# hassony2/homan

Measured on AMD Instinct MI355X. Metric: optimisation iters/sec (30-frame 256^2 clip), higher is better.
Workload: dtype f32

## Files before the change

homan_amd/csrc/adam.hip:

```cpp
#include "hm_common.h"

struct AdamSlot {
    float* p; float* g; float* m; float* v;
    long n;
    float lr;
    int pad;
};

__device__ __forceinline__ void log_total_clip(float* __restrict__ vals, const float* __restrict__ w, int n, int s,
                                               int max_steps, float* __restrict__ log, int c, int nc)
{
    float* v = vals + (long)c * (n + 1);
    float t = 0.f;
    for (int i = 0; i < n; ++i)
        if (w[i] != 0.f) t += w[i] * v[i];
    v[n] = t;
    if (s < max_steps)
        for (int i = 0; i <= n; ++i) log[((long)s * nc + c) * (n + 1) + i] = v[i];
}
__device__ __forceinline__ double adam_pow(double b, int t)
{
    double r = 1.0;
    for (; t > 0; t >>= 1) {
        if (t & 1) r = r * b;
        b = b * b;
    }
    return r;
}
__global__ __launch_bounds__(256) void k_adam(const AdamSlot* __restrict__ slots, int n_tensors, int* __restrict__ step,
                                               float beta1, float beta2, float eps, int zero_grad, float* __restrict__ vals,
                                               const float* __restrict__ log_w, int log_n, int max_steps,
                                               float* __restrict__ log, int nclips)
{
    HM_LATENCY_KERNEL();
    HM_STAMP_START(0);
    const int step_now = __builtin_nontemporal_load(step);
    if ((int)blockIdx.y == n_tensors) {
        if (threadIdx.x == 0) {
            for (int c = blockIdx.x; c < nclips; c += gridDim.x) log_total_clip(vals, log_w, log_n, step_now, max_steps, log, c, nclips);
            const unsigned nblk = gridDim.x * gridDim.y;
            if (atomicAdd(reinterpret_cast<unsigned int*>(step) + 1, 1u) == nblk - 1u) {
                atomicExch(reinterpret_cast<unsigned int*>(step) + 1, 0u);
                atomicExch(step, step_now + 1);
            }
        }
        return;
    }
    const AdamSlot s = slots[blockIdx.y];
    const double bc1 = 1.0 - adam_pow((double)beta1, step_now + 1);
    const double bc2 = 1.0 - adam_pow((double)beta2, step_now + 1);
    const float neg_step = (float)(-((double)s.lr / bc1));
    const float bc2_sqrt = (float)sqrt(bc2);
    const float w1 = (float)(1.0 - (double)beta1), w2 = (float)(1.0 - (double)beta2);
    for (long i = (long)blockIdx.x * blockDim.x + threadIdx.x; i < s.n; i += (long)gridDim.x * blockDim.x) {
        const float g = s.g[i];
        float m = s.m[i], v = s.v[i];
        m = m + w1 * (g - m);
        v = v * beta2;
        v = v + (w2 * g) * g;
        const float denom = sqrtf(v) / bc2_sqrt + eps;
        s.p[i] = s.p[i] + (neg_step * m) / denom;
        s.m[i] = m;
        s.v[i] = v;
        if (zero_grad) s.g[i] = 0.f;
    }
    __syncthreads();
    if (threadIdx.x == 0) {
        const unsigned nblk = gridDim.x * gridDim.y;
        if (atomicAdd(reinterpret_cast<unsigned int*>(step) + 1, 1u) == nblk - 1u) {
            atomicExch(reinterpret_cast<unsigned int*>(step) + 1, 0u);
            atomicExch(step, step_now + 1);
        }
    }
    HM_STAMP_END(0);
}

__global__ void k_log(const float* __restrict__ src, int n, const int* __restrict__ step, int max_steps,
                      float* __restrict__ log)
{
    const int i = blockIdx.x * blockDim.x + threadIdx.x;
    const int t = step[0];
    if (i < n && t < max_steps) log[(long)t * n + i] = src[i];
}

__global__ void k_log_total(float* __restrict__ vals, const float* __restrict__ w, int n, const int* __restrict__ step,
                            int max_steps, float* __restrict__ log)
{
    HM_LATENCY_KERNEL();
    if (threadIdx.x == 0) log_total_clip(vals, w, n, step[0], max_steps, log, blockIdx.x, gridDim.x);
}

extern "C" {
int hm_log_total_clips(float* vals, const float* weights, int n, const int* step, int max_steps, float* log, int nclips,
                       hipStream_t stream)
{
    HM_CHECK_ARG(vals && weights && step && log && n > 0 && nclips > 0);
    hipLaunchKernelGGL(k_log_total, dim3(nclips), dim3(64), 0, stream, vals, weights, n, step, max_steps, log);
    return hm_launch_status();
}
size_t hm_adam_slot_bytes(void) { return sizeof(AdamSlot); }

int hm_adam_step(const void* slots, int n_tensors, int* step, float beta1, float beta2, float eps, int zero_grad,
                 int blocks_per_tensor, hipStream_t stream)
{
    HM_CHECK_ARG(slots && step && n_tensors > 0 && blocks_per_tensor > 0);
    hipLaunchKernelGGL(k_adam, dim3(blocks_per_tensor, n_tensors), dim3(256), 0, stream, (const AdamSlot*)slots, n_tensors,
                       step, beta1, beta2, eps, zero_grad, (float*)nullptr, (const float*)nullptr, 0, 0, (float*)nullptr, 0);
    return hm_launch_status();
}
int hm_adam_step_log(const void* slots, int n_tensors, int* step, float beta1, float beta2, float eps, int zero_grad,
                     int blocks_per_tensor, float* vals, const float* weights, int n, int max_steps, float* log, int nclips,
                     hipStream_t stream)
{
    HM_CHECK_ARG(slots && step && n_tensors > 0 && blocks_per_tensor > 0);
    HM_CHECK_ARG(vals && weights && log && n > 0 && nclips > 0);
    hipLaunchKernelGGL(k_adam, dim3(blocks_per_tensor, n_tensors + 1), dim3(256), 0, stream, (const AdamSlot*)slots, n_tensors,
                       step, beta1, beta2, eps, zero_grad, vals, weights, n, max_steps, log, nclips);
    return hm_launch_status();
}
int hm_log_scalars(const float* src, int n, const int* step, int max_steps, float* log, hipStream_t stream)
{
    HM_CHECK_ARG(src && step && log && n > 0);
    hipLaunchKernelGGL(k_log, dim3(hm_cdiv(n, 64)), dim3(64), 0, stream, src, n, step, max_steps, log);
    return hm_launch_status();
}
#ifdef HM_CHAIN_STAMPS
int hm_debug_chain_adam(unsigned long long* out, int reset)
{
    unsigned long long z[8] = {~0ull, 0, ~0ull, 0, ~0ull, 0, ~0ull, 0};
    (void)hipDeviceSynchronize();
    if (out) (void)hipMemcpyFromSymbol(out, HIP_SYMBOL(g_chain_ts), sizeof(z));
    if (reset) (void)hipMemcpyToSymbol(HIP_SYMBOL(g_chain_ts), z, sizeof(z));
    return HM_OK;
}
#endif
}
```

homan_amd/csrc/geometry.hip:

```cpp
#include "hm_common.h"

__global__ __launch_bounds__(256) void k_rigid_fwd(const float* __restrict__ mesh, const float* __restrict__ rot6d,
                                                   const float* __restrict__ trans, const float* __restrict__ scale,
                                                   int abs_scale, int N, int V, float* __restrict__ rotmat,
                                                   float* __restrict__ verts, int clip_len)
{
    __shared__ float R[9];
    const int n = blockIdx.y;
    if (threadIdx.x == 0) {
        float r[9];
        rot6d_to_mat(rot6d + n * 6, r);
#pragma unroll
        for (int k = 0; k < 9; ++k) R[k] = r[k];
        if (blockIdx.x == 0 && rotmat)
#pragma unroll
            for (int k = 0; k < 9; ++k) rotmat[n * 9 + k] = r[k];
    }
    __syncthreads();
    const int v = blockIdx.x * blockDim.x + threadIdx.x;
    if (v >= V) return;
    float s = scale[n / clip_len];
    if (abs_scale) s = fabsf(s);
    const float* m = mesh + ((long)n * V + v) * 3;
    const float x = s * m[0], y = s * m[1], z = s * m[2];
    float* o = verts + ((long)n * V + v) * 3;
    const float* t = trans + n * 3;
    o[0] = x * R[0] + y * R[3] + z * R[6] + t[0];
    o[1] = x * R[1] + y * R[4] + z * R[7] + t[1];
    o[2] = x * R[2] + y * R[5] + z * R[8] + t[2];
}

struct SilGather {
    const double* parts;
    const int* adj_off;
    const int* adj_items;
    const float* cam_verts;
    const float* K;
    float orig_size;
    int F;
};
template <bool EXACT>
__global__ __launch_bounds__(1024) void k_rigid_bwd(const float* __restrict__ mesh, const float* __restrict__ rot6d,
                                                   const float* __restrict__ scale, int abs_scale, RigidTerms terms,
                                                   SilGather sil,
                                                   const float* __restrict__ g_rigid, const float* __restrict__ g_frame,
                                                   int frame_stride, float frame_scale, int N, int V,
                                                   float* __restrict__ g_mesh,
                                                   float* __restrict__ g_rot6d, float* __restrict__ g_trans,
                                                   float* __restrict__ g_scale_part, float* __restrict__ partials,
                                                   unsigned int* __restrict__ frame_cnt, int clip_len, double magic)
{
    HM_LATENCY_KERNEL();
    HM_STAMP_START(sil.parts ? 1 : 0);
    __shared__ float red13[16 * 13];
    __shared__ double red13d[EXACT ? 16 * 13 : 1];
    __shared__ int s_flag;
    const int n = blockIdx.x;
    float R[9];
    rot6d_to_mat(rot6d + n * 6, R);
    const float sraw = scale[n / clip_len];
    const float s = abs_scale ? fabsf(sraw) : sraw;
    float gfr[3] = {0.f, 0.f, 0.f};
    if (g_frame) {
#pragma unroll
        for (int c = 0; c < 3; ++c) gfr[c] = frame_scale * g_frame[(long)n * frame_stride + c];
    }
    float acc[13];
    double accd[13];
#pragma unroll
    for (int k = 0; k < 13; ++k) { acc[k] = 0.f; accd[k] = 0.0; }
    for (int v = blockIdx.y * blockDim.x + threadIdx.x; v < V; v += gridDim.y * blockDim.x) {
        const long o = ((long)n * V + v) * 3;
        const float m[3] = {mesh[o], mesh[o + 1], mesh[o + 2]};
        float gf[3] = {0.f, 0.f, 0.f}, gt[3];
#pragma unroll
        for (int k = 0; k < 5; ++k)
            if (terms.p[k]) {
                gf[0] += terms.w[k] * terms.p[k][o]; gf[1] += terms.w[k] * terms.p[k][o + 1]; gf[2] += terms.w[k] * terms.p[k][o + 2];
            }
        if (sil.parts) {
            double su = 0.0, sv = 0.0;
            const double2* pf = reinterpret_cast<const double2*>(sil.parts + (long)n * sil.F * 6);
            const int a1 = sil.adj_off[v + 1];
            for (int a = sil.adj_off[v]; a < a1; a += 8) {
                int item[8];
#pragma unroll
                for (int k = 0; k < 8; ++k) item[k] = a + k < a1 ? sil.adj_items[a + k] : -1;
                double2 g2[8];
#pragma unroll
                for (int k = 0; k < 8; ++k) g2[k] = item[k] >= 0 ? pf[item[k]] : make_double2(0.0, 0.0);
#pragma unroll
                for (int k = 0; k < 8; ++k) { su += g2[k].x; sv += g2[k].y; }
            }
            const float gu = (float)su, gv = (float)sv;
            const float* k = sil.K + n * 9;
            const float x = sil.cam_verts[o], y = sil.cam_verts[o + 1], z = sil.cam_verts[o + 2];
            const float zz = z + 1e-9f;
            const float du0 = gu * (2.0f / sil.orig_size), dv0 = -gv * (2.0f / sil.orig_size);
            const float dxn = k[0] * du0 + k[3] * dv0;
            const float dyn = k[1] * du0 + k[4] * dv0;
            gf[0] += dxn / zz;
            gf[1] += dyn / zz;
            gf[2] += -(dxn * x + dyn * y) / (zz * zz);
        }
        gt[0] = gf[0] + gfr[0]; gt[1] = gf[1] + gfr[1]; gt[2] = gf[2] + gfr[2];
        if (g_rigid) { gt[0] += g_rigid[o]; gt[1] += g_rigid[o + 1]; gt[2] += g_rigid[o + 2]; }
        const float dm[3] = {R[0] * gf[0] + R[1] * gf[1] + R[2] * gf[2], R[3] * gf[0] + R[4] * gf[1] + R[5] * gf[2],
                             R[6] * gf[0] + R[7] * gf[1] + R[8] * gf[2]};
        if (EXACT) {
#pragma unroll
            for (int i = 0; i < 3; ++i)
#pragma unroll
                for (int j = 0; j < 3; ++j) accd[3 * i + j] += hm_quant((s * m[i]) * gt[j], magic);
#pragma unroll
            for (int j = 0; j < 3; ++j) accd[9 + j] += hm_quant(gt[j], magic);
            accd[12] += hm_quant(m[0] * dm[0] + m[1] * dm[1] + m[2] * dm[2], magic);
        } else {
#pragma unroll
            for (int i = 0; i < 3; ++i)
#pragma unroll
                for (int j = 0; j < 3; ++j) acc[3 * i + j] += (s * m[i]) * gt[j];
#pragma unroll
            for (int j = 0; j < 3; ++j) acc[9 + j] += gt[j];
            acc[12] += m[0] * dm[0] + m[1] * dm[1] + m[2] * dm[2];
        }
        if (g_mesh) { g_mesh[o] = s * dm[0]; g_mesh[o + 1] = s * dm[1]; g_mesh[o + 2] = s * dm[2]; }
    }
    float tot[13];
    if (EXACT) {
        hm_block_sum_n_f64<13>(accd, red13d);
        if (gridDim.y > 1) {
            double* rec = reinterpret_cast<double*>(partials + ((long)n * gridDim.y + blockIdx.y) * 32);
            if (threadIdx.x == 0) {
#pragma unroll
                for (int k = 0; k < 13; ++k) __hip_atomic_store(rec + k, accd[k], __ATOMIC_RELAXED, __HIP_MEMORY_SCOPE_AGENT);
            }
            if (!hm_last_block(frame_cnt + n, gridDim.y, &s_flag)) return;
            if (threadIdx.x < 13 * gridDim.y)
                red13d[threadIdx.x] = __hip_atomic_load(reinterpret_cast<const double*>(partials + ((long)n * gridDim.y + threadIdx.x / 13) * 32) + threadIdx.x % 13,
                                                        __ATOMIC_RELAXED, __HIP_MEMORY_SCOPE_AGENT);
            __syncthreads();
            if (threadIdx.x == 0) {
#pragma unroll
                for (int k = 0; k < 13; ++k) accd[k] = 0.0;
                for (unsigned c = 0; c < gridDim.y; ++c)
#pragma unroll
                    for (int k = 0; k < 13; ++k) accd[k] += red13d[c * 13 + k];
            }
        }
#pragma unroll
        for (int k = 0; k < 13; ++k) tot[k] = (float)accd[k];
    } else {
#pragma unroll
    for (int k = 0; k < 13; ++k) tot[k] = acc[k];
    hm_block_sum_n<13>(tot, red13);
    if (gridDim.y > 1) {
        float* rec = partials + ((long)n * gridDim.y + blockIdx.y) * 32;
        if (threadIdx.x == 0) {
#pragma unroll
            for (int k = 0; k < 13; ++k) hm_partial_store(rec + k, tot[k]);
        }
        if (!hm_last_block(frame_cnt + n, gridDim.y, &s_flag)) return;
        if (threadIdx.x < 13 * gridDim.y)
            red13[threadIdx.x] = hm_partial_load(partials + ((long)n * gridDim.y + threadIdx.x / 13) * 32 + threadIdx.x % 13);
        __syncthreads();
        if (threadIdx.x == 0) {
#pragma unroll
            for (int k = 0; k < 13; ++k) tot[k] = 0.f;
            for (unsigned c = 0; c < gridDim.y; ++c)
#pragma unroll
                for (int k = 0; k < 13; ++k) tot[k] += red13[c * 13 + k];
        }
    }
    }
    if (threadIdx.x == 0) {
        float dr6[6];
        rot6d_backward(rot6d + n * 6, tot, dr6);
#pragma unroll
        for (int k = 0; k < 6; ++k) g_rot6d[n * 6 + k] = dr6[k];
#pragma unroll
        for (int k = 0; k < 3; ++k) g_trans[n * 3 + k] = tot[9 + k];
        if (g_scale_part) g_scale_part[n] = (abs_scale && sraw < 0.f) ? -tot[12] : tot[12];
    }
    HM_STAMP_END(sil.parts ? 1 : 0);
}

struct SmoothIn { const float* verts; float w; };
template <int NV, int MAXT>
__global__ __launch_bounds__(MAXT) void k_rigid_bwd_x(const float* __restrict__ mesh, const float* __restrict__ rot6d,
                                                     const float* __restrict__ scale, int abs_scale, RigidTerms terms,
                                                     SilGather sil, SmoothIn sm, int N, int V, float* __restrict__ g_rot6d,
                                                     float* __restrict__ g_trans, float* __restrict__ g_scale_part,
                                                     float* __restrict__ partials, unsigned int* __restrict__ frame_cnt,
                                                     int clip_len, double magic)
{
    HM_LATENCY_KERNEL();
    HM_STAMP_START(1);
    __shared__ double red13d[16 * 13];
    __shared__ int s_flag;
    const int n = blockIdx.x;
    float R[9];
    rot6d_to_mat(rot6d + n * 6, R);
    const float sraw = scale[n / clip_len];
    const float s = abs_scale ? fabsf(sraw) : sraw;
    const int fl = n % clip_len;
    const long row = (long)V * 3;
    const long scnt = (long)(clip_len - 1) * row;
    const float inv_cnt = scnt > 0 ? 1.0f / (float)scnt : 0.f;
    int vv[NV];
    bool ok[NV];
    int a0[NV], a1[NV];
    float m[NV][3], cv[NV][3], tv[NV][5][3], nb[NV][2][3];
#pragma unroll
    for (int j = 0; j < NV; ++j) {
        vv[j] = ((int)blockIdx.y * NV + j) * (int)blockDim.x + (int)threadIdx.x;
        ok[j] = vv[j] < V;
        const int v = ok[j] ? vv[j] : 0;
        const long o = ((long)n * V + v) * 3;
        a0[j] = sil.parts ? sil.adj_off[v] : 0;
        a1[j] = sil.parts ? sil.adj_off[v + 1] : 0;
#pragma unroll
        for (int c = 0; c < 3; ++c) {
            m[j][c] = mesh[o + c];
            cv[j][c] = sil.parts ? sil.cam_verts[o + c] : 0.f;
        }
#pragma unroll
        for (int k = 0; k < 5; ++k)
#pragma unroll
            for (int c = 0; c < 3; ++c) tv[j][k][c] = terms.p[k] ? terms.p[k][o + c] : 0.f;
#pragma unroll
        for (int c = 0; c < 3; ++c) {
            nb[j][0][c] = (sm.verts && fl + 1 < clip_len) ? sm.verts[o + row + c] : 0.f;
            nb[j][1][c] = (sm.verts && fl >= 1) ? sm.verts[o - row + c] : 0.f;
        }
    }
    float sv[NV][3];
#pragma unroll
    for (int j = 0; j < NV; ++j)
#pragma unroll
        for (int c = 0; c < 3; ++c) sv[j][c] = sm.verts ? sm.verts[((long)n * V + (ok[j] ? vv[j] : 0)) * 3 + c] : 0.f;
    int item[NV][8];
#pragma unroll
    for (int j = 0; j < NV; ++j)
#pragma unroll
        for (int k = 0; k < 8; ++k) item[j][k] = (ok[j] && a0[j] + k < a1[j]) ? sil.adj_items[a0[j] + k] : -1;
    double su[NV], sw[NV];
    {
        const double2* pf = reinterpret_cast<const double2*>(sil.parts + (long)n * sil.F * 6);
        double2 g2[NV][8];
#pragma unroll
        for (int j = 0; j < NV; ++j)
#pragma unroll
            for (int k = 0; k < 8; ++k) g2[j][k] = item[j][k] >= 0 ? pf[item[j][k]] : make_double2(0.0, 0.0);
#pragma unroll
        for (int j = 0; j < NV; ++j) {
            su[j] = 0.0; sw[j] = 0.0;
#pragma unroll
            for (int k = 0; k < 8; ++k) { su[j] += g2[j][k].x; sw[j] += g2[j][k].y; }
            for (int a = a0[j] + 8; ok[j] && a < a1[j]; ++a) {
                const double2 g = pf[sil.adj_items[a]];
                su[j] += g.x; sw[j] += g.y;
            }
        }
    }
    double accd[13];
#pragma unroll
    for (int k = 0; k < 13; ++k) accd[k] = 0.0;
#pragma unroll
    for (int j = 0; j < NV; ++j) {
        if (!ok[j]) continue;
        float gf[3] = {0.f, 0.f, 0.f}, gt[3];
        if (sm.verts) {
#pragma unroll
            for (int c = 0; c < 3; ++c) {
                float g = 0.f;
                if (fl + 1 < clip_len) { const float d = nb[j][0][c] - sv[j][c]; g -= d; }
                if (fl >= 1) g += sv[j][c] - nb[j][1][c];
                gf[c] += sm.w * (2.0f * g * inv_cnt);
            }
        }
#pragma unroll
        for (int k = 0; k < 5; ++k)
            if (terms.p[k]) {
                gf[0] += terms.w[k] * tv[j][k][0]; gf[1] += terms.w[k] * tv[j][k][1]; gf[2] += terms.w[k] * tv[j][k][2];
            }
        if (sil.parts) {
            const float gu = (float)su[j], gv = (float)sw[j];
            const float* k = sil.K + n * 9;
            const float x = cv[j][0], y = cv[j][1], z = cv[j][2];
            const float zz = z + 1e-9f;
            const float du0 = gu * (2.0f / sil.orig_size), dv0 = -gv * (2.0f / sil.orig_size);
            const float dxn = k[0] * du0 + k[3] * dv0;
            const float dyn = k[1] * du0 + k[4] * dv0;
            gf[0] += dxn / zz;
            gf[1] += dyn / zz;
            gf[2] += -(dxn * x + dyn * y) / (zz * zz);
        }
        gt[0] = gf[0] + 0.f; gt[1] = gf[1] + 0.f; gt[2] = gf[2] + 0.f;
        const float dm[3] = {R[0] * gf[0] + R[1] * gf[1] + R[2] * gf[2], R[3] * gf[0] + R[4] * gf[1] + R[5] * gf[2],
                             R[6] * gf[0] + R[7] * gf[1] + R[8] * gf[2]};
#pragma unroll
        for (int i = 0; i < 3; ++i)
#pragma unroll
            for (int q = 0; q < 3; ++q) accd[3 * i + q] += hm_quant((s * m[j][i]) * gt[q], magic);
#pragma unroll
        for (int q = 0; q < 3; ++q) accd[9 + q] += hm_quant(gt[q], magic);
        accd[12] += hm_quant(m[j][0] * dm[0] + m[j][1] * dm[1] + m[j][2] * dm[2], magic);
    }
    hm_block_sum_n_f64<13>(accd, red13d);
    if (gridDim.y > 1) {
        double* rec = reinterpret_cast<double*>(partials + ((long)n * gridDim.y + blockIdx.y) * 32);
        if (threadIdx.x == 0) {
#pragma unroll
            for (int k = 0; k < 13; ++k) __hip_atomic_store(rec + k, accd[k], __ATOMIC_RELAXED, __HIP_MEMORY_SCOPE_AGENT);
        }
        if (!hm_last_block(frame_cnt + n, gridDim.y, &s_flag)) return;
        if (threadIdx.x < 13 * gridDim.y)
            red13d[threadIdx.x] = __hip_atomic_load(reinterpret_cast<const double*>(partials + ((long)n * gridDim.y + threadIdx.x / 13) * 32) + threadIdx.x % 13,
                                                    __ATOMIC_RELAXED, __HIP_MEMORY_SCOPE_AGENT);
        __syncthreads();
        if (threadIdx.x == 0) {
#pragma unroll
            for (int k = 0; k < 13; ++k) accd[k] = 0.0;
            for (unsigned c = 0; c < gridDim.y; ++c)
#pragma unroll
                for (int k = 0; k < 13; ++k) accd[k] += red13d[c * 13 + k];
        }
    }
    if (threadIdx.x == 0) {
        float tot[13], dr6[6];
#pragma unroll
        for (int k = 0; k < 13; ++k) tot[k] = (float)accd[k];
        rot6d_backward(rot6d + n * 6, tot, dr6);
#pragma unroll
        for (int k = 0; k < 6; ++k) g_rot6d[n * 6 + k] = dr6[k];
#pragma unroll
        for (int k = 0; k < 3; ++k) g_trans[n * 3 + k] = tot[9 + k];
        if (g_scale_part) g_scale_part[n] = (abs_scale && sraw < 0.f) ? -tot[12] : tot[12];
    }
    HM_STAMP_END(1);
}

__global__ void k_scale_by(const float* __restrict__ in, const float* __restrict__ s, long n, float* __restrict__ out)
{
    const long i = (long)blockIdx.x * blockDim.x + threadIdx.x;
    if (i < n) out[i] = s[0] * in[i];
}
__global__ void k_sum_small(const float* __restrict__ parts, int n, float w0, const float* __restrict__ extra, float w1,
                            float* __restrict__ out)
{
    __shared__ float red[16];
    const int c = blockIdx.x;
    float a = 0.f;
    for (int i = threadIdx.x; i < n; i += blockDim.x) a += parts[(long)c * n + i];
    a = hm_block_sum(a, red);
    if (threadIdx.x == 0) out[c] = w0 * a + (extra ? w1 * extra[c] : 0.f);
}

extern "C" {
int hm_sum_small_clips(const float* parts, int n, float w0, const float* extra, float w1, float* out, int nclips,
                       hipStream_t stream)
{
    HM_CHECK_ARG(parts && out && n > 0 && nclips > 0);
    hipLaunchKernelGGL(k_sum_small, dim3(nclips), dim3(64), 0, stream, parts, n, w0, extra, w1, out);
    return hm_launch_status();
}
int hm_rigid_fwd_clips(const float* mesh, const float* rot6d, const float* trans, const float* scale, int abs_scale, int N,
                       int V, float* rotmat, float* verts, int clip_len, hipStream_t stream)
{
    HM_CHECK_ARG(mesh && rot6d && trans && scale && verts && N > 0 && V > 0 && HM_CLIP_LEN_OK(N, clip_len));
    hipLaunchKernelGGL(k_rigid_fwd, dim3(hm_cdiv(V, 256), N), dim3(256), 0, stream, mesh, rot6d, trans, scale,
                       abs_scale, N, V, rotmat, verts, clip_len ? clip_len : N);
    return hm_launch_status();
}
int hm_rigid_fwd(const float* mesh, const float* rot6d, const float* trans, const float* scale, int abs_scale, int N,
                 int V, float* rotmat, float* verts, hipStream_t stream)
{
    return hm_rigid_fwd_clips(mesh, rot6d, trans, scale, abs_scale, N, V, rotmat, verts, 0, stream);
}
#define RIGID_MAX_CHUNKS 16
size_t hm_rigid_workspace_bytes(int N) { return (((size_t)N * 4 + 255) & ~(size_t)255) + (size_t)N * RIGID_MAX_CHUNKS * 32 * 4; }
static int rigid_bwd_launch(const float* mesh, const float* rot6d, const float* scale, int abs_scale,
                            const float* const* g_terms, const float* weights, int n_terms, SilGather sil,
                            const float* g_rigid, const float* g_frame, int frame_stride, float frame_scale, int N, int V,
                            float* g_mesh, float* g_rot6d, float* g_trans, float* g_scale_part, void* workspace,
                            int clip_len, int exact, int sum_log2q, SmoothIn smooth, hipStream_t stream)
{
    HM_CHECK_ARG(sum_log2q <= 0 && sum_log2q >= -60);
    HM_CHECK_ARG(mesh && rot6d && scale && g_rot6d && g_trans && N > 0 && V > 0 && HM_CLIP_LEN_OK(N, clip_len));
    HM_CHECK_ARG(n_terms >= 0 && n_terms <= 5 && (n_terms == 0 || (g_terms && weights)));
    HM_CHECK_ARG(!g_frame || frame_stride >= 3);
    RigidTerms t;
    for (int k = 0; k < 5; ++k) { t.p[k] = k < n_terms ? g_terms[k] : nullptr; t.w[k] = k < n_terms ? weights[k] : 0.f; }
    const int threads = exact ? 256 : (V > 512 ? 1024 : 256);
    const int chunks = workspace ? min(RIGID_MAX_CHUNKS, hm_cdiv(V, exact ? threads : 4 * threads)) : 1;
    unsigned int* cnt = (unsigned int*)workspace;
    float* partials = workspace ? (float*)((char*)workspace + (((size_t)N * 4 + 255) & ~(size_t)255)) : nullptr;
    const bool small = V <= RIGID_MAX_CHUNKS * 256;
    const int nv = small ? 1 : 2;
    const int thr = small ? 256 : 768;
    if (exact && !g_rigid && !g_frame && !g_mesh && (workspace ? V <= RIGID_MAX_CHUNKS * thr * nv : V <= thr * nv)) {
        const int ch = hm_cdiv(V, thr * nv);
        const double magic = hm_sum_magic(sum_log2q);
        if (nv == 2)
            hipLaunchKernelGGL((k_rigid_bwd_x<2, 768>), dim3(N, ch), dim3(thr), 0, stream, mesh, rot6d, scale,
                               abs_scale, t, sil, smooth, N, V, g_rot6d, g_trans, g_scale_part, partials, cnt, clip_len ? clip_len : N, magic);
        else
            hipLaunchKernelGGL((k_rigid_bwd_x<1, 1024>), dim3(N, ch), dim3(thr), 0, stream, mesh, rot6d, scale,
                               abs_scale, t, sil, smooth, N, V, g_rot6d, g_trans, g_scale_part, partials, cnt, clip_len ? clip_len : N, magic);
        return hm_launch_status();
    }
    HM_CHECK_ARG(!smooth.verts);
    if (exact)
        hipLaunchKernelGGL(k_rigid_bwd<true>, dim3(N, chunks), dim3(threads), 0, stream, mesh, rot6d, scale,
                           abs_scale, t, sil, g_rigid, g_frame, frame_stride, frame_scale, N, V, g_mesh, g_rot6d, g_trans,
                           g_scale_part, partials, cnt, clip_len ? clip_len : N, hm_sum_magic(sum_log2q));
    else
        hipLaunchKernelGGL(k_rigid_bwd<false>, dim3(N, chunks), dim3(threads), 0, stream, mesh, rot6d, scale,
                           abs_scale, t, sil, g_rigid, g_frame, frame_stride, frame_scale, N, V, g_mesh, g_rot6d, g_trans,
                           g_scale_part, partials, cnt, clip_len ? clip_len : N, 0.0);
    return hm_launch_status();
}
int hm_rigid_bwd_clips(const float* mesh, const float* rot6d, const float* scale, int abs_scale,
                       const float* const* g_terms, const float* weights, int n_terms, const float* g_rigid,
                       const float* g_frame, int frame_stride, float frame_scale, int N, int V, float* g_mesh,
                       float* g_rot6d, float* g_trans, float* g_scale_part, void* workspace, int clip_len,
                       hipStream_t stream)
{
    SilGather none = {nullptr, nullptr, nullptr, nullptr, nullptr, 1.0f, 0};
    return rigid_bwd_launch(mesh, rot6d, scale, abs_scale, g_terms, weights, n_terms, none, g_rigid, g_frame, frame_stride,
                            frame_scale, N, V, g_mesh, g_rot6d, g_trans, g_scale_part, workspace, clip_len, 0, 0,
                            SmoothIn{nullptr, 0.f}, stream);
}
int hm_rigid_bwd(const float* mesh, const float* rot6d, const float* scale, int abs_scale, const float* const* g_terms,
                 const float* weights, int n_terms, const float* g_rigid, const float* g_frame, int frame_stride,
                 float frame_scale, int N, int V, float* g_mesh, float* g_rot6d, float* g_trans, float* g_scale_part,
                 void* workspace, hipStream_t stream)
{
    return hm_rigid_bwd_clips(mesh, rot6d, scale, abs_scale, g_terms, weights, n_terms, g_rigid, g_frame, frame_stride,
                              frame_scale, N, V, g_mesh, g_rot6d, g_trans, g_scale_part, workspace, 0, stream);
}
int hm_rigid_bwd_sil_clips(const float* mesh, const float* rot6d, const float* scale, int abs_scale,
                           const float* const* g_terms, const float* weights, int n_terms, const double* sil_parts,
                           const int* adj_off, const int* adj_items, const float* cam_verts, const float* K,
                           float orig_size, int F, int N, int V, float* g_rot6d, float* g_trans, float* g_scale_part,
                           void* workspace, int clip_len, int sum_log2q, const float* smooth_verts, float smooth_weight,
                           hipStream_t stream)
{
    HM_CHECK_ARG(sil_parts && adj_off && adj_items && cam_verts && K && F > 0);
    SilGather sil = {sil_parts, adj_off, adj_items, cam_verts, K, orig_size, F};
    return rigid_bwd_launch(mesh, rot6d, scale, abs_scale, g_terms, weights, n_terms, sil, nullptr, nullptr, 0, 0.f, N, V,
                            nullptr, g_rot6d, g_trans, g_scale_part, workspace, clip_len, 1, sum_log2q,
                            SmoothIn{smooth_verts, smooth_weight}, stream);
}
int hm_rigid_bwd_sil(const float* mesh, const float* rot6d, const float* scale, int abs_scale, const float* const* g_terms,
                     const float* weights, int n_terms, const double* sil_parts, const int* adj_off, const int* adj_items,
                     const float* cam_verts, const float* K, float orig_size, int F, int N, int V, float* g_rot6d,
                     float* g_trans, float* g_scale_part, void* workspace, int sum_log2q, hipStream_t stream)
{
    return hm_rigid_bwd_sil_clips(mesh, rot6d, scale, abs_scale, g_terms, weights, n_terms, sil_parts, adj_off, adj_items,
                                  cam_verts, K, orig_size, F, N, V, g_rot6d, g_trans, g_scale_part, workspace, 0, sum_log2q,
                                  nullptr, 0.f, stream);
}
int hm_scale_by(const float* in, const float* s, long n, float* out, hipStream_t stream)
{
    HM_CHECK_ARG(in && s && out && n > 0);
    hipLaunchKernelGGL(k_scale_by, dim3(hm_cdiv(n, 256)), dim3(256), 0, stream, in, s, n, out);
    return hm_launch_status();
}
#ifdef HM_CHAIN_STAMPS
int hm_debug_chain_geometry(unsigned long long* out, int reset)
{
    unsigned long long z[8] = {~0ull, 0, ~0ull, 0, ~0ull, 0, ~0ull, 0};
    (void)hipDeviceSynchronize();
    if (out) (void)hipMemcpyFromSymbol(out, HIP_SYMBOL(g_chain_ts), sizeof(z));
    if (reset) (void)hipMemcpyToSymbol(HIP_SYMBOL(g_chain_ts), z, sizeof(z));
    return HM_OK;
}
#endif
}
```

homan_amd/csrc/hm_common.h:

```cpp
#pragma once
#include <hip/hip_runtime.h>
#include <stdint.h>
#include "homan_amd.h"

#define HM_WAVE 64

#ifndef HM_PRIO
#define HM_PRIO 3
#endif
#define HM_LATENCY_KERNEL() __builtin_amdgcn_s_setprio(HM_PRIO)
#ifdef HM_CHAIN_STAMPS
static __device__ unsigned long long g_chain_ts[8];
#define HM_STAMP_START(k) do { if (threadIdx.x == 0) atomicMin(&g_chain_ts[2 * (k)], (unsigned long long)wall_clock64()); } while (0)
#define HM_STAMP_END(k) do { if (threadIdx.x == 0) atomicMax(&g_chain_ts[2 * (k) + 1], (unsigned long long)wall_clock64()); } while (0)
#else
#define HM_STAMP_START(k)
#define HM_STAMP_END(k)
#endif
#ifndef HM_HAND_PRIO
#define HM_HAND_PRIO HM_PRIO
#endif
#define HM_HAND_KERNEL() __builtin_amdgcn_s_setprio(HM_HAND_PRIO)
#ifdef HM_CHAIN_PRIO
#define HM_CHAIN_KERNEL() __builtin_amdgcn_s_setprio(HM_CHAIN_PRIO)
#else
#define HM_CHAIN_KERNEL()
#endif

#define HM_CHECK_ARG(cond) \
    do {                   \
        if (!(cond)) return HM_ERR_BAD_ARG; \
    } while (0)

#define HM_CLIP_LEN_OK(N, clip_len) ((clip_len) == 0 || ((clip_len) > 0 && (N) % (clip_len) == 0))
#define HM_RED_WS_FLOATS 576

static inline int hm_launch_status()
{
    hipError_t e = hipGetLastError();
    return e == hipSuccess ? HM_OK : HM_ERR_LAUNCH;
}

static inline int hm_cdiv(long a, long b) { return (int)((a + b - 1) / b); }

template <int CTRL, int ROW_MASK>
__device__ __forceinline__ float hm_dpp(float old, float v)
{
    return __builtin_bit_cast(float, __builtin_amdgcn_update_dpp(__builtin_bit_cast(int, old), __builtin_bit_cast(int, v),
                                                                CTRL, ROW_MASK, 0xf, false));
}
__device__ __forceinline__ float hm_wave_sum(float v)
{
    v += hm_dpp<0xb1, 0xf>(0.f, v);
    v += hm_dpp<0x4e, 0xf>(0.f, v);
    v += hm_dpp<0x114, 0xf>(0.f, v);
    v += hm_dpp<0x118, 0xf>(0.f, v);
    v += hm_dpp<0x142, 0xa>(0.f, v);
    v += hm_dpp<0x143, 0xc>(0.f, v);
    return __builtin_bit_cast(float, __builtin_amdgcn_readlane(__builtin_bit_cast(int, v), 63));
}
__device__ __forceinline__ float hm_wave_min(float v)
{
    v = fminf(v, hm_dpp<0xb1, 0xf>(v, v));
    v = fminf(v, hm_dpp<0x4e, 0xf>(v, v));
    v = fminf(v, hm_dpp<0x114, 0xf>(v, v));
    v = fminf(v, hm_dpp<0x118, 0xf>(v, v));
    v = fminf(v, hm_dpp<0x142, 0xa>(v, v));
    v = fminf(v, hm_dpp<0x143, 0xc>(v, v));
    return __builtin_bit_cast(float, __builtin_amdgcn_readlane(__builtin_bit_cast(int, v), 63));
}
__device__ __forceinline__ float hm_wave_max(float v)
{
    v = fmaxf(v, hm_dpp<0xb1, 0xf>(v, v));
    v = fmaxf(v, hm_dpp<0x4e, 0xf>(v, v));
    v = fmaxf(v, hm_dpp<0x114, 0xf>(v, v));
    v = fmaxf(v, hm_dpp<0x118, 0xf>(v, v));
    v = fmaxf(v, hm_dpp<0x142, 0xa>(v, v));
    v = fmaxf(v, hm_dpp<0x143, 0xc>(v, v));
    return __builtin_bit_cast(float, __builtin_amdgcn_readlane(__builtin_bit_cast(int, v), 63));
}

__device__ __forceinline__ float hm_block_sum(float v, float* red)
{
    const int lane = threadIdx.x & 63, w = threadIdx.x >> 6, nw = (blockDim.x + 63) >> 6;
    v = hm_wave_sum(v);
    __syncthreads();
    if (lane == 0) red[w] = v;
    __syncthreads();
    float t = 0.f;
    for (int i = 0; i < nw; ++i) t += red[i];
    return t;
}
template <int N>
__device__ __forceinline__ void hm_block_sum_n(float (&v)[N], float* red)
{
    const int lane = threadIdx.x & 63, w = threadIdx.x >> 6, nw = (blockDim.x + 63) >> 6;
#pragma unroll
    for (int k = 0; k < N; ++k) v[k] = hm_wave_sum(v[k]);
    __syncthreads();
    if (lane == 0) {
#pragma unroll
        for (int k = 0; k < N; ++k) red[k * 16 + w] = v[k];
    }
    __syncthreads();
#pragma unroll
    for (int k = 0; k < N; ++k) {
        float t = 0.f;
        for (int i = 0; i < nw; ++i) t += red[k * 16 + i];
        v[k] = t;
    }
}
__device__ __forceinline__ float hm_block_min(float v, float* red)
{
    const int lane = threadIdx.x & 63, w = threadIdx.x >> 6, nw = (blockDim.x + 63) >> 6;
    v = hm_wave_min(v);
    __syncthreads();
    if (lane == 0) red[w] = v;
    __syncthreads();
    float t = red[0];
    for (int i = 1; i < nw; ++i) t = fminf(t, red[i]);
    return t;
}
__device__ __forceinline__ float hm_block_max(float v, float* red)
{
    const int lane = threadIdx.x & 63, w = threadIdx.x >> 6, nw = (blockDim.x + 63) >> 6;
    v = hm_wave_max(v);
    __syncthreads();
    if (lane == 0) red[w] = v;
    __syncthreads();
    float t = red[0];
    for (int i = 1; i < nw; ++i) t = fmaxf(t, red[i]);
    return t;
}

__device__ __forceinline__ void hm_partial_store(float* p, float v)
{
    __hip_atomic_store(p, v, __ATOMIC_RELAXED, __HIP_MEMORY_SCOPE_AGENT);
}
__device__ __forceinline__ float hm_partial_load(const float* p)
{
    return __hip_atomic_load(p, __ATOMIC_RELAXED, __HIP_MEMORY_SCOPE_AGENT);
}
__device__ __forceinline__ bool hm_last_block(unsigned int* counter, unsigned int nblocks, int* s_flag)
{
    __syncthreads();
    if (threadIdx.x == 0) {
        asm volatile("s_waitcnt vmcnt(0)" ::: "memory");
        const unsigned int ticket = atomicAdd(counter, 1u);
        const int last = (ticket == nblocks - 1u);
        if (last) atomicExch(counter, 0u);
        *s_flag = last;
    }
    __syncthreads();
    return *s_flag != 0;
}


__device__ __forceinline__ float hm_last_block_sum(const float* partials, int n, int stride, float* red)
{
    float a = 0.f;
    for (int i = threadIdx.x; i < n; i += blockDim.x) a += hm_partial_load(partials + (long)i * stride);
    return hm_block_sum(a, red);
}

__host__ __device__ __forceinline__ void hm_sincos(float af, float* sn, float* cs)
{
    const double a = (double)af;
    const double k = __builtin_rint(a * 0.63661977236758138243);
    double r = a - k * 1.57079632673412561417e+00;
    r = r - k * 6.07710050650619224932e-11;
    const double z = r * r;
    double ps = 1.58969099521155010221e-10;
    ps = -2.50507602534068634195e-08 + z * ps;
    ps = 2.75573137070700676789e-06 + z * ps;
    ps = -1.98412698298579493134e-04 + z * ps;
    ps = 8.33333333332248946124e-03 + z * ps;
    ps = -1.66666666666666324348e-01 + z * ps;
    const double s = r + (r * z) * ps;
    double pc = -1.13596475577881948265e-11;
    pc = 2.08757232129817482790e-09 + z * pc;
    pc = -2.75573143513906633035e-07 + z * pc;
    pc = 2.48015872894767294178e-05 + z * pc;
    pc = -1.38888888888741095749e-03 + z * pc;
    pc = 4.16666666666666019037e-02 + z * pc;
    const double c = (1.0 - 0.5 * z) + (z * z) * pc;
    const int q = (int)((long long)k) & 3;
    const double sv = (q == 0) ? s : (q == 1) ? c : (q == 2) ? -s : -c;
    const double cv = (q == 0) ? c : (q == 1) ? -s : (q == 2) ? -c : s;
    *sn = (float)sv;
    *cs = (float)cv;
}

__host__ __device__ __forceinline__ float hm_tanh(float xf)
{
    const double ax = xf < 0.f ? -(double)xf : (double)xf;
    if (ax > 20.0) return xf < 0.f ? -1.0f : 1.0f;
    if (ax < 0.01) {
        const double q = ax * ax;
        const double sm = ax * (1.0 + q * (-3.33333333333333314830e-01 + q * (1.33333333333333331483e-01 + q * -5.39682539682539708542e-02)));
        return (float)(xf < 0.f ? -sm : sm);
    }
    const double t = -2.0 * ax;
    const double k = __builtin_rint(t * 1.44269504088896338700e+00);
    const double r = (t - k * 6.93147180369123816490e-01) - k * 1.90821492927058770002e-10;
    const double z = r * r;
    double p = 4.13813679705723846039e-08;
    p = -1.65339022054652515390e-06 + z * p;
    p = 6.61375632143793436117e-05 + z * p;
    p = -2.77777777770155933842e-03 + z * p;
    p = 1.66666666666666019037e-01 + z * p;
    const double c = r - z * p;
    const double er = 1.0 - ((r * c) / (c - 2.0) - r);
    const double e = __builtin_ldexp(er, (int)k);
    const double th = (1.0 - e) / (1.0 + e);
    return (float)(xf < 0.f ? -th : th);
}

__host__ __device__ __forceinline__ float hm_sigmoid(float xf)
{
    const double t = -(double)xf;
    const double k = __builtin_rint(t * 1.44269504088896338700e+00);
    const double r = (t - k * 6.93147180369123816490e-01) - k * 1.90821492927058770002e-10;
    const double z = r * r;
    double p = 4.13813679705723846039e-08;
    p = -1.65339022054652515390e-06 + z * p;
    p = 6.61375632143793436117e-05 + z * p;
    p = -2.77777777770155933842e-03 + z * p;
    p = 1.66666666666666019037e-01 + z * p;
    const double c = r - z * p;
    const double er = 1.0 - ((r * c) / (c - 2.0) - r);
    const double e = __builtin_ldexp(er, (int)k);
    return (float)(1.0 / (1.0 + e));
}

__device__ __forceinline__ void rot6d_to_mat(const float* r6 , float* R )
{
    const float a1[3] = {r6[0], r6[2], r6[4]}, a2[3] = {r6[1], r6[3], r6[5]};
    const float n1 = fmaxf(sqrtf(a1[0] * a1[0] + a1[1] * a1[1] + a1[2] * a1[2]), 1e-12f);
    const float b1[3] = {a1[0] / n1, a1[1] / n1, a1[2] / n1};
    const float d = b1[0] * a2[0] + b1[1] * a2[1] + b1[2] * a2[2];
    const float u[3] = {a2[0] - d * b1[0], a2[1] - d * b1[1], a2[2] - d * b1[2]};
    const float nu = fmaxf(sqrtf(u[0] * u[0] + u[1] * u[1] + u[2] * u[2]), 1e-12f);
    const float b2[3] = {u[0] / nu, u[1] / nu, u[2] / nu};
    const float b3[3] = {b1[1] * b2[2] - b1[2] * b2[1], b1[2] * b2[0] - b1[0] * b2[2], b1[0] * b2[1] - b1[1] * b2[0]};
#pragma unroll
    for (int i = 0; i < 3; ++i) { R[3 * i] = b1[i]; R[3 * i + 1] = b2[i]; R[3 * i + 2] = b3[i]; }
}

__device__ __forceinline__ void rot6d_backward(const float* r6, const float* dR, float* dr6)
{
    const float a1[3] = {r6[0], r6[2], r6[4]}, a2[3] = {r6[1], r6[3], r6[5]};
    const float n1r = sqrtf(a1[0] * a1[0] + a1[1] * a1[1] + a1[2] * a1[2]);
    const float n1 = fmaxf(n1r, 1e-12f);
    const float b1[3] = {a1[0] / n1, a1[1] / n1, a1[2] / n1};
    const float d = b1[0] * a2[0] + b1[1] * a2[1] + b1[2] * a2[2];
    const float u[3] = {a2[0] - d * b1[0], a2[1] - d * b1[1], a2[2] - d * b1[2]};
    const float nur = sqrtf(u[0] * u[0] + u[1] * u[1] + u[2] * u[2]);
    const float nu = fmaxf(nur, 1e-12f);
    const float b2[3] = {u[0] / nu, u[1] / nu, u[2] / nu};
    float db1[3] = {dR[0], dR[3], dR[6]}, db2[3] = {dR[1], dR[4], dR[7]};
    const float db3[3] = {dR[2], dR[5], dR[8]};
    db1[0] += b2[1] * db3[2] - b2[2] * db3[1];
    db1[1] += b2[2] * db3[0] - b2[0] * db3[2];
    db1[2] += b2[0] * db3[1] - b2[1] * db3[0];
    db2[0] += db3[1] * b1[2] - db3[2] * b1[1];
    db2[1] += db3[2] * b1[0] - db3[0] * b1[2];
    db2[2] += db3[0] * b1[1] - db3[1] * b1[0];
    float du[3];
    if (nur > 1e-12f) {
        const float s = b2[0] * db2[0] + b2[1] * db2[1] + b2[2] * db2[2];
#pragma unroll
        for (int i = 0; i < 3; ++i) du[i] = (db2[i] - b2[i] * s) / nu;
    } else {
#pragma unroll
        for (int i = 0; i < 3; ++i) du[i] = db2[i] / nu;
    }
    float da2[3] = {du[0], du[1], du[2]};
    const float dd = -(du[0] * b1[0] + du[1] * b1[1] + du[2] * b1[2]);
#pragma unroll
    for (int i = 0; i < 3; ++i) { db1[i] += -d * du[i] + dd * a2[i]; da2[i] += dd * b1[i]; }
    float da1[3];
    if (n1r > 1e-12f) {
        const float s = b1[0] * db1[0] + b1[1] * db1[1] + b1[2] * db1[2];
#pragma unroll
        for (int i = 0; i < 3; ++i) da1[i] = (db1[i] - b1[i] * s) / n1;
    } else {
#pragma unroll
        for (int i = 0; i < 3; ++i) da1[i] = db1[i] / n1;
    }
#pragma unroll
    for (int i = 0; i < 3; ++i) { dr6[2 * i] = da1[i]; dr6[2 * i + 1] = da2[i]; }
}

#define HM_SUM_LOG2Q_DEFAULT (-44)
__host__ __device__ __forceinline__ double hm_sum_magic(int log2q)
{
    return 6755399441055744.0  * __builtin_ldexp(1.0, log2q ? log2q : HM_SUM_LOG2Q_DEFAULT);
}
__device__ __forceinline__ double hm_quant(float x, double magic) { return ((double)x + magic) - magic; }

template <int CTRL, int ROW_MASK>
__device__ __forceinline__ double hm_dpp_f64(double v)
{
    const int lo = __builtin_amdgcn_update_dpp(0, __double2loint(v), CTRL, ROW_MASK, 0xf, false);
    const int hi = __builtin_amdgcn_update_dpp(0, __double2hiint(v), CTRL, ROW_MASK, 0xf, false);
    return __hiloint2double(hi, lo);
}
__device__ __forceinline__ double hm_wave_sum_f64(double v)
{
    v += hm_dpp_f64<0xb1, 0xf>(v);
    v += hm_dpp_f64<0x4e, 0xf>(v);
    v += hm_dpp_f64<0x114, 0xf>(v);
    v += hm_dpp_f64<0x118, 0xf>(v);
    v += hm_dpp_f64<0x142, 0xa>(v);
    v += hm_dpp_f64<0x143, 0xc>(v);
    return __hiloint2double(__builtin_amdgcn_readlane(__double2hiint(v), 63), __builtin_amdgcn_readlane(__double2loint(v), 63));
}
template <int N>
__device__ __forceinline__ void hm_block_sum_n_f64(double (&v)[N], double* red)
{
    const int lane = threadIdx.x & 63, w = threadIdx.x >> 6, nw = (blockDim.x + 63) >> 6;
#pragma unroll
    for (int k = 0; k < N; ++k) v[k] = hm_wave_sum_f64(v[k]);
    if (nw == 1) return;
    __syncthreads();
    if (lane == 0) {
#pragma unroll
        for (int k = 0; k < N; ++k) red[k * 16 + w] = v[k];
    }
    __syncthreads();
#pragma unroll
    for (int k = 0; k < N; ++k) {
        double t = 0.0;
        for (int i = 0; i < nw; ++i) t += red[k * 16 + i];
        v[k] = t;
    }
}

struct RigidTerms { const float* p[5]; float w[5]; };
```

homan_amd/csrc/mano.hip:

```cpp
#include "hm_common.h"
#include <string.h>

#define MANO_V 778
#define MANO_J 16
#define MANO_NF 145
#define MANO_CHUNK 256
#define MANO_NCHUNK 4
#define MANO_PART 352
#define MANO_NCH64 13
#define MANO_STATE_SH 832
#define MANO_STATE_DW (MANO_STATE_SH + 3 * MANO_V + 2)

struct ManoModelDev {
    const float* v_template;
    const float* M;
    const float* J_template;
    const float* J_shapedirs;
    const float* weights;
    const float* comps;
    const float* hand_mean;
    const int* parents;
};

__device__ __forceinline__ void rodrigues(const float* r, float* R)
{
    const float e0 = r[0] + 1e-8f, e1 = r[1] + 1e-8f, e2 = r[2] + 1e-8f;
    const float a = sqrtf(e0 * e0 + e1 * e1 + e2 * e2);
    const float nx = r[0] / a, ny = r[1] / a, nz = r[2] / a;
    float s, cs_;
    hm_sincos(a, &s, &cs_);
    const float c1 = 1.0f - cs_;
    const float K[9] = {0.f, -nz, ny, nz, 0.f, -nx, -ny, nx, 0.f};
#pragma unroll
    for (int i = 0; i < 3; ++i)
#pragma unroll
        for (int j = 0; j < 3; ++j) {
            float kk = K[3 * i] * K[j] + K[3 * i + 1] * K[3 + j] + K[3 * i + 2] * K[6 + j];
            R[3 * i + j] = (i == j ? 1.0f : 0.0f) + s * K[3 * i + j] + c1 * kk;
        }
}

__device__ __forceinline__ void rodrigues_backward(const float* r, const float* dR, float* dr)
{
    const float e[3] = {r[0] + 1e-8f, r[1] + 1e-8f, r[2] + 1e-8f};
    const float a = sqrtf(e[0] * e[0] + e[1] * e[1] + e[2] * e[2]);
    const float n[3] = {r[0] / a, r[1] / a, r[2] / a};
    float s, c;
    hm_sincos(a, &s, &c);
    const float c1 = 1.0f - c;
    const float K[9] = {0.f, -n[2], n[1], n[2], 0.f, -n[0], -n[1], n[0], 0.f};
    float KK[9];
#pragma unroll
    for (int i = 0; i < 3; ++i)
#pragma unroll
        for (int j = 0; j < 3; ++j) KK[3 * i + j] = K[3 * i] * K[j] + K[3 * i + 1] * K[3 + j] + K[3 * i + 2] * K[6 + j];
    float dRK = 0.f, dRKK = 0.f;
#pragma unroll
    for (int k = 0; k < 9; ++k) { dRK += dR[k] * K[k]; dRKK += dR[k] * KK[k]; }
    float da = c * dRK + s * dRKK;
    float dK[9];
#pragma unroll
    for (int i = 0; i < 3; ++i)
#pragma unroll
        for (int j = 0; j < 3; ++j) {
            float t1 = dR[3 * i] * K[3 * j] + dR[3 * i + 1] * K[3 * j + 1] + dR[3 * i + 2] * K[3 * j + 2];
            float t2 = K[i] * dR[j] + K[3 + i] * dR[3 + j] + K[6 + i] * dR[6 + j];
            dK[3 * i + j] = s * dR[3 * i + j] + c1 * (t1 + t2);
        }
    const float dn[3] = {dK[7] - dK[5], dK[2] - dK[6], dK[3] - dK[1]};
    da += -(dn[0] * r[0] + dn[1] * r[1] + dn[2] * r[2]) / (a * a);
#pragma unroll
    for (int i = 0; i < 3; ++i) dr[i] = dn[i] / a + da * e[i] / a;
}

struct ManoShared {
    float pose[48];
    float Rl[MANO_J][9];
    float J[MANO_J][3];
    float Rw[MANO_J][9];
    float tw[MANO_J][3];
    float A[MANO_J][12];
    float feat[MANO_NF];
    int parents[MANO_J];
    int depth[MANO_J];
};

__device__ __forceinline__ void mano_prepare(const ManoModelDev& m, const float* pca, int pca_stride, const float* rot,
                                             const float* betas, int b, ManoShared& sh, int t)
{
    if (t < 48) {
        float v;
        if (t < 3) v = rot[b * 3 + t];
        else {
            const int k = t - 3;
            v = 0.f;
            for (int i = 0; i < 16; ++i) v += pca[(long)b * pca_stride + i] * m.comps[i * 45 + k];
            v += m.hand_mean[k];
        }
        sh.pose[t] = v;
    }
    if (t < 10) sh.feat[135 + t] = betas[b * 10 + t];
    if (t < MANO_J) sh.parents[t] = m.parents[t];
    __syncthreads();
    if (t < MANO_J) {
        int d = 0;
        for (int q = sh.parents[t]; q >= 0; q = sh.parents[q]) ++d;
        sh.depth[t] = d;
        float R[9];
        rodrigues(&sh.pose[3 * t], R);
#pragma unroll
        for (int k = 0; k < 9; ++k) sh.Rl[t][k] = R[k];
        if (t >= 1)
#pragma unroll
            for (int k = 0; k < 9; ++k) sh.feat[9 * (t - 1) + k] = R[k] - ((k % 4 == 0) ? 1.0f : 0.0f);
#pragma unroll
        for (int c = 0; c < 3; ++c) {
            float v = m.J_template[t * 3 + c];
            for (int l = 0; l < 10; ++l) v += betas[b * 10 + l] * m.J_shapedirs[(t * 3 + c) * 10 + l];
            sh.J[t][c] = v;
        }
    }
    __syncthreads();
    int depth = 0, par = -1, maxd = 0;
    if (t < MANO_J) { par = sh.parents[t]; depth = sh.depth[t]; }
#pragma unroll
    for (int j = 0; j < MANO_J; ++j) maxd = max(maxd, sh.depth[j]);
    for (int level = 0; level < MANO_J; ++level) {
        if (t < MANO_J && depth == level) {
            const int j = t, p = par;
            if (p < 0) {
#pragma unroll
                for (int k = 0; k < 9; ++k) sh.Rw[j][k] = sh.Rl[j][k];
#pragma unroll
                for (int c = 0; c < 3; ++c) sh.tw[j][c] = sh.J[j][c];
            } else {
                const float rel[3] = {sh.J[j][0] - sh.J[p][0], sh.J[j][1] - sh.J[p][1], sh.J[j][2] - sh.J[p][2]};
#pragma unroll
                for (int i = 0; i < 3; ++i) {
#pragma unroll
                    for (int k = 0; k < 3; ++k)
                        sh.Rw[j][3 * i + k] = sh.Rw[p][3 * i] * sh.Rl[j][k] + sh.Rw[p][3 * i + 1] * sh.Rl[j][3 + k] +
                                              sh.Rw[p][3 * i + 2] * sh.Rl[j][6 + k];
                    sh.tw[j][i] = sh.Rw[p][3 * i] * rel[0] + sh.Rw[p][3 * i + 1] * rel[1] + sh.Rw[p][3 * i + 2] * rel[2] +
                                  sh.tw[p][i];
                }
            }
        }
        __syncthreads();
        if (level >= maxd) break;
    }
    if (t < MANO_J) {
        const int j = t;
#pragma unroll
        for (int i = 0; i < 3; ++i) {
            sh.A[j][4 * i] = sh.Rw[j][3 * i];
            sh.A[j][4 * i + 1] = sh.Rw[j][3 * i + 1];
            sh.A[j][4 * i + 2] = sh.Rw[j][3 * i + 2];
            sh.A[j][4 * i + 3] = sh.tw[j][i] - (sh.Rw[j][3 * i] * sh.J[j][0] + sh.Rw[j][3 * i + 1] * sh.J[j][1] +
                                                sh.Rw[j][3 * i + 2] * sh.J[j][2]);
        }
    }
    __syncthreads();
}

#define MANO_VCH 64
#define MANO_ROWS_PER_WAVE 37
__device__ __forceinline__ void mano_posed_chunk(const ManoModelDev& m, const ManoShared& sh, int v0, float (*s_part)[MANO_VCH][3],
                                                 float (*s_vp)[3])
{
    const int lane = threadIdx.x & 63, wv = threadIdx.x >> 6;
    const int v = min(v0 + lane, MANO_V - 1);
    float a0 = 0.f, a1 = 0.f, a2 = 0.f;
    const int k0 = wv * MANO_ROWS_PER_WAVE, k1 = min(MANO_NF, k0 + MANO_ROWS_PER_WAVE);
    const float* base = m.M + 3 * v;
#pragma unroll 4
    for (int k = k0; k < k1; ++k) {
        const float f = sh.feat[k];
        const float* row = base + (long)k * (3 * MANO_V);
        a0 += f * row[0];
        a1 += f * row[1];
        a2 += f * row[2];
    }
    s_part[wv][lane][0] = a0; s_part[wv][lane][1] = a1; s_part[wv][lane][2] = a2;
    __syncthreads();
    if (wv == 0) {
#pragma unroll
        for (int c = 0; c < 3; ++c)
            s_vp[lane][c] = m.v_template[3 * v + c] + ((s_part[0][lane][c] + s_part[1][lane][c]) + (s_part[2][lane][c] + s_part[3][lane][c]));
    }
    __syncthreads();
}

__device__ __forceinline__ void mano_skin_transform(const ManoModelDev& m, const ManoShared& sh, int v, float* T)
{
#pragma unroll
    for (int k = 0; k < 12; ++k) T[k] = 0.f;
    const float4* wrow = reinterpret_cast<const float4*>(m.weights + v * MANO_J);
#pragma unroll
    for (int q = 0; q < 4; ++q) {
        const float4 w4 = wrow[q];
        const float ws[4] = {w4.x, w4.y, w4.z, w4.w};
#pragma unroll
        for (int u = 0; u < 4; ++u) {
            const int j = 4 * q + u;
#pragma unroll
            for (int k = 0; k < 12; ++k) T[k] += ws[u] * sh.A[j][k];
        }
    }
}

#define MANO_FPW 4
__global__ __launch_bounds__(256) void k_mano_fwd(ManoModelDev m, const float* __restrict__ pca, int pca_stride,
                                                   const float* __restrict__ rot, const float* __restrict__ betas,
                                                   const float* __restrict__ trans, int B, float* __restrict__ verts,
                                                   float* __restrict__ joints, const float* __restrict__ rigid_rot6d,
                                                   const float* __restrict__ rigid_trans,
                                                   const float* __restrict__ rigid_scale, float* __restrict__ verts_world,
                                                   float* __restrict__ state, int clip_len, int row0, int row_stride)
{
    __shared__ ManoShared shs[MANO_FPW];
    __shared__ float s_part[4][MANO_FPW][MANO_VCH][3];
    __shared__ float s_vp[MANO_FPW][MANO_VCH][3];
    __shared__ float s_R[MANO_FPW][9];
    const int lane = threadIdx.x & 63, wv = threadIdx.x >> 6;
    const int b_raw = blockIdx.y * MANO_FPW + wv;
    const bool live = b_raw < B;
    const int b = (min(b_raw, B - 1)) * row_stride + row0;
    ManoShared& sh = shs[wv];
    if (verts_world && lane == 48) rot6d_to_mat(rigid_rot6d + b * 6, s_R[wv]);
    mano_prepare(m, pca, pca_stride, rot, betas, b, sh, lane);
    const float tr[3] = {trans ? trans[b * 3] : 0.f, trans ? trans[b * 3 + 1] : 0.f, trans ? trans[b * 3 + 2] : 0.f};
    if (joints && live && blockIdx.x == 0 && lane < MANO_J * 3)
        joints[b * MANO_J * 3 + lane] = sh.tw[lane / 3][lane % 3] + tr[lane % 3];
    const int v0 = blockIdx.x * MANO_VCH;
    const int v = min(v0 + lane, MANO_V - 1);
    {
        float a[MANO_FPW][3];
#pragma unroll
        for (int f = 0; f < MANO_FPW; ++f) a[f][0] = a[f][1] = a[f][2] = 0.f;
        const int k0 = wv * MANO_ROWS_PER_WAVE, k1 = min(MANO_NF, k0 + MANO_ROWS_PER_WAVE);
        const float* base = m.M + 3 * v;
#pragma unroll 4
        for (int k = k0; k < k1; ++k) {
            const float* row = base + (long)k * (3 * MANO_V);
            const float r0 = row[0], r1 = row[1], r2 = row[2];
#pragma unroll
            for (int f = 0; f < MANO_FPW; ++f) {
                const float ft = shs[f].feat[k];
                a[f][0] += ft * r0;
                a[f][1] += ft * r1;
                a[f][2] += ft * r2;
            }
        }
#pragma unroll
        for (int f = 0; f < MANO_FPW; ++f) {
            s_part[wv][f][lane][0] = a[f][0]; s_part[wv][f][lane][1] = a[f][1]; s_part[wv][f][lane][2] = a[f][2];
        }
    }
    __syncthreads();
#pragma unroll
    for (int c = 0; c < 3; ++c)
        s_vp[wv][lane][c] = m.v_template[3 * v + c] + ((s_part[0][wv][lane][c] + s_part[1][wv][lane][c]) +
                                                       (s_part[2][wv][lane][c] + s_part[3][wv][lane][c]));
    __builtin_amdgcn_wave_barrier();
    if (!live) return;
    if (state) {
        float* st = state + (long)b * MANO_STATE_DW;
        if (blockIdx.x == 0)
            for (int i = lane; i < (int)(sizeof(ManoShared) / 4); i += 64) st[i] = reinterpret_cast<const float*>(&sh)[i];
        const int nv3 = 3 * min(MANO_VCH, MANO_V - v0);
        for (int i = lane; i < nv3; i += 64) st[MANO_STATE_SH + 3 * v0 + i] = (&s_vp[wv][0][0])[i];
    }
    if (v0 + lane >= MANO_V) return;
    float T[12];
    mano_skin_transform(m, sh, v, T);
    const float* vp = s_vp[wv][lane];
    float* o = verts + ((long)b * MANO_V + v) * 3;
    float p[3];
#pragma unroll
    for (int i = 0; i < 3; ++i) { p[i] = T[4 * i] * vp[0] + T[4 * i + 1] * vp[1] + T[4 * i + 2] * vp[2] + T[4 * i + 3] + tr[i]; o[i] = p[i]; }
    if (verts_world) {
        const float s = rigid_scale[b / clip_len];
        const float x = s * p[0], y = s * p[1], z = s * p[2];
        const float* t = rigid_trans + b * 3;
        const float* R = s_R[wv];
        float* ow = verts_world + ((long)b * MANO_V + v) * 3;
        ow[0] = x * R[0] + y * R[3] + z * R[6] + t[0];
        ow[1] = x * R[1] + y * R[4] + z * R[7] + t[1];
        ow[2] = x * R[2] + y * R[5] + z * R[8] + t[2];
    }
}

static_assert(sizeof(ManoShared) / 4 <= MANO_STATE_SH, "MANO_STATE_SH too small");

struct ManoBwd2Shared {
    float tot[MANO_PART];
    float dRw[MANO_J][9], dtw[MANO_J][3], dJ[MANO_J][3], dRl[MANO_J][9], dpose[48];
    float cR[MANO_J][9], ct[MANO_J][3], cJ[MANO_J][3];
};
__device__ __forceinline__ void mano_bwd2_body(const ManoModelDev& m, const ManoShared& sh, ManoBwd2Shared& w,
                                               const float* __restrict__ partials, int nchunk, int lb, int b, int pca_dim,
                                               const float* __restrict__ g_pca_extra, float w_extra,
                                               float* __restrict__ g_pca, float* __restrict__ g_rot,
                                               float* __restrict__ g_betas, float* __restrict__ g_trans)
{
    const int t = threadIdx.x, nt = blockDim.x;
    for (int k = t; k < MANO_PART; k += nt) {
        float v[MANO_NCH64];
#pragma unroll
        for (int c = 0; c < MANO_NCH64; ++c)
            v[c] = c < nchunk ? hm_partial_load(partials + ((long)lb * nchunk + c) * MANO_PART + k) : 0.f;
        float a = 0.f;
#pragma unroll
        for (int c = 0; c < MANO_NCH64; ++c) a += v[c];
        w.tot[k] = a;
    }
    int depth = 0, par = -1, maxd = 0;
    if (t < MANO_J) { par = sh.parents[t]; depth = sh.depth[t]; }
#pragma unroll
    for (int j = 0; j < MANO_J; ++j) maxd = max(maxd, sh.depth[j]);
    __syncthreads();
    if (t < MANO_J) {
        const int j = t;
        const float* dA = &w.tot[j * 12];
#pragma unroll
        for (int i = 0; i < 3; ++i) {
#pragma unroll
            for (int k = 0; k < 3; ++k) w.dRw[j][3 * i + k] = dA[4 * i + k] - dA[4 * i + 3] * sh.J[j][k];
            w.dtw[j][i] = dA[4 * i + 3];
        }
#pragma unroll
        for (int k = 0; k < 3; ++k)
            w.dJ[j][k] = -(sh.Rw[j][k] * dA[3] + sh.Rw[j][3 + k] * dA[7] + sh.Rw[j][6 + k] * dA[11]);
    }
    __syncthreads();
    for (int level = maxd; level >= 1; --level) {
        if (t < MANO_J && depth == level) {
            const int j = t, p = par;
            const float rel[3] = {sh.J[j][0] - sh.J[p][0], sh.J[j][1] - sh.J[p][1], sh.J[j][2] - sh.J[p][2]};
#pragma unroll
            for (int i = 0; i < 3; ++i) {
#pragma unroll
                for (int k = 0; k < 3; ++k)
                    w.cR[j][3 * i + k] = w.dtw[j][i] * rel[k] + w.dRw[j][3 * i] * sh.Rl[j][3 * k] +
                                         w.dRw[j][3 * i + 1] * sh.Rl[j][3 * k + 1] + w.dRw[j][3 * i + 2] * sh.Rl[j][3 * k + 2];
                w.ct[j][i] = w.dtw[j][i];
            }
#pragma unroll
            for (int k = 0; k < 3; ++k) {
                const float d = sh.Rw[p][k] * w.dtw[j][0] + sh.Rw[p][3 + k] * w.dtw[j][1] + sh.Rw[p][6 + k] * w.dtw[j][2];
                w.dJ[j][k] += d;
                w.cJ[j][k] = -d;
            }
#pragma unroll
            for (int i = 0; i < 3; ++i)
#pragma unroll
                for (int k = 0; k < 3; ++k)
                    w.dRl[j][3 * i + k] = sh.Rw[p][i] * w.dRw[j][k] + sh.Rw[p][3 + i] * w.dRw[j][3 + k] + sh.Rw[p][6 + i] * w.dRw[j][6 + k];
        }
        __syncthreads();
        if (t < MANO_J && depth == level - 1) {
            for (int j = 0; j < MANO_J; ++j)
                if (sh.parents[j] == t) {
#pragma unroll
                    for (int k = 0; k < 9; ++k) w.dRw[t][k] += w.cR[j][k];
#pragma unroll
                    for (int k = 0; k < 3; ++k) { w.dtw[t][k] += w.ct[j][k]; w.dJ[t][k] += w.cJ[j][k]; }
                }
        }
        __syncthreads();
    }
    if (t < MANO_J && par < 0) {
#pragma unroll
        for (int k = 0; k < 9; ++k) w.dRl[t][k] = w.dRw[t][k];
#pragma unroll
        for (int c = 0; c < 3; ++c) w.dJ[t][c] += w.dtw[t][c];
    }
    __syncthreads();
    if (t < MANO_J) {
        float dR[9];
#pragma unroll
        for (int k = 0; k < 9; ++k) dR[k] = w.dRl[t][k] + (t >= 1 ? w.tot[192 + 9 * (t - 1) + k] : 0.f);
        float dr[3];
        rodrigues_backward(&sh.pose[3 * t], dR, dr);
#pragma unroll
        for (int c = 0; c < 3; ++c) w.dpose[3 * t + c] = dr[c];
    }
    __syncthreads();
    if (t < 3) {
        g_rot[b * 3 + t] = w.dpose[t];
        g_trans[b * 3 + t] = w.tot[337 + t];
    }
    for (int i = t; i < pca_dim; i += nt) {
        float a = 0.f;
        if (i < 16) {
            float cv[45];
#pragma unroll
            for (int k = 0; k < 45; ++k) cv[k] = m.comps[i * 45 + k];
#pragma unroll
            for (int k = 0; k < 45; ++k) a += cv[k] * w.dpose[3 + k];
        }
        if (g_pca_extra) a += w_extra * g_pca_extra[(long)b * pca_dim + i];
        g_pca[(long)b * pca_dim + i] = a;
    }
    if (t < 10) {
        float a = w.tot[192 + 135 + t];
        float jv[MANO_J * 3];
#pragma unroll
        for (int q = 0; q < MANO_J * 3; ++q) jv[q] = m.J_shapedirs[q * 10 + t];
#pragma unroll
        for (int q = 0; q < MANO_J * 3; ++q) a += jv[q] * w.dJ[q / 3][q % 3];
        g_betas[b * 10 + t] = a;
    }
}

#ifdef MANO_PHASES
static __device__ unsigned long long g_mano_ph[16];
#define MPH_MARK(k) do { if (threadIdx.x == 0) { const unsigned long long t_ = wall_clock64(); atomicAdd(&g_mano_ph[k], t_ - mph_t); mph_t = t_; } } while (0)
#else
#define MPH_MARK(k)
#endif
struct ManoRigid {
    const float* mesh;
    const float* rot6d;
    const float* scale;
    int clip_len;
    RigidTerms terms;
    const float* g_rigid;
    const float* g_frame;
    int frame_stride;
    float frame_scale;
    float* g_rot6d; float* g_trans;
};
template <bool RIGID>
__global__ __launch_bounds__(256) void k_mano_bwd(ManoModelDev m, const float* __restrict__ pca, int pca_stride,
                                                   const float* __restrict__ rot, const float* __restrict__ betas,
                                                   const float* __restrict__ gout, int B, const float* __restrict__ state,
                                                   float* __restrict__ partials, unsigned int* __restrict__ frame_cnt,
                                                   int pca_dim, const float* __restrict__ g_pca_extra, float w_extra,
                                                   float* __restrict__ g_pca, float* __restrict__ g_rot,
                                                   float* __restrict__ g_betas, float* __restrict__ g_trans, int row0,
                                                   int row_stride, ManoRigid mr)
{
    HM_HAND_KERNEL();
    __shared__ ManoShared sh;
    __shared__ float s_part[4][MANO_VCH][3];
    __shared__ float s_vp[MANO_VCH][3];
    __shared__ float s_g[MANO_VCH][3];
    __shared__ float s_dvp[MANO_VCH * 3];
    __shared__ float s_w[MANO_VCH][MANO_J + 1];
    __shared__ float red[16];
    __shared__ ManoBwd2Shared w2;
    __shared__ int s_flag;
    const int lb = blockIdx.y, b = lb * row_stride + row0, t = threadIdx.x;
    const int v0 = blockIdx.x * MANO_VCH;
    const int nv = min(MANO_VCH, MANO_V - v0);
#ifdef MANO_PHASES
    unsigned long long mph_t = wall_clock64();
    if (t == 0) atomicAdd(&g_mano_ph[15], 1ull);
#endif
    if (state) {
        const float* st = state + (long)b * MANO_STATE_DW;
        for (int i = t; i < (int)(sizeof(ManoShared) / 4); i += blockDim.x) reinterpret_cast<float*>(&sh)[i] = st[i];
        if (t < 3 * nv) (&s_vp[0][0])[t] = st[MANO_STATE_SH + 3 * v0 + t];
        __syncthreads();
    } else {
        mano_prepare(m, pca, pca_stride, rot, betas, b, sh, threadIdx.x);
        mano_posed_chunk(m, sh, v0, s_part, s_vp);
    }
    MPH_MARK(0);
    float g[3] = {0.f, 0.f, 0.f};
    float racc[12];
#pragma unroll
    for (int k = 0; k < 12; ++k) racc[k] = 0.f;
    if (t < nv) {
        const int v = v0 + t;
        if (RIGID) {
            const long o = ((long)b * MANO_V + v) * 3;
            float R[9];
            rot6d_to_mat(mr.rot6d + (long)b * 6, R);
            const float s = mr.scale[b / mr.clip_len];
            const float mv[3] = {mr.mesh[o], mr.mesh[o + 1], mr.mesh[o + 2]};
            float gf[3] = {0.f, 0.f, 0.f}, gt[3];
#pragma unroll
            for (int k = 0; k < 5; ++k)
                if (mr.terms.p[k]) {
                    gf[0] += mr.terms.w[k] * mr.terms.p[k][o]; gf[1] += mr.terms.w[k] * mr.terms.p[k][o + 1];
                    gf[2] += mr.terms.w[k] * mr.terms.p[k][o + 2];
                }
#pragma unroll
            for (int c = 0; c < 3; ++c)
                gt[c] = gf[c] + (mr.g_frame ? mr.frame_scale * mr.g_frame[(long)b * mr.frame_stride + c] : 0.f);
            if (mr.g_rigid) { gt[0] += mr.g_rigid[o]; gt[1] += mr.g_rigid[o + 1]; gt[2] += mr.g_rigid[o + 2]; }
#pragma unroll
            for (int i = 0; i < 3; ++i)
#pragma unroll
                for (int j = 0; j < 3; ++j) racc[3 * i + j] = (s * mv[i]) * gt[j];
#pragma unroll
            for (int j = 0; j < 3; ++j) racc[9 + j] = gt[j];
            g[0] = s * (R[0] * gf[0] + R[1] * gf[1] + R[2] * gf[2]);
            g[1] = s * (R[3] * gf[0] + R[4] * gf[1] + R[5] * gf[2]);
            g[2] = s * (R[6] * gf[0] + R[7] * gf[1] + R[8] * gf[2]);
        } else {
            const float* gp = gout + ((long)b * MANO_V + v) * 3;
            g[0] = gp[0]; g[1] = gp[1]; g[2] = gp[2];
        }
    }
    float* out = partials + ((long)lb * gridDim.x + blockIdx.x) * MANO_PART;
    if (RIGID) {
        float* red12 = &s_part[0][0][0];
        hm_block_sum_n<12>(racc, red12);
        if (t < 12) hm_partial_store(out + 340 + t, racc[t]);
        __syncthreads();
    }
    if (t < nv) {
        const int v = v0 + t;
        float T[12];
        mano_skin_transform(m, sh, v, T);
#pragma unroll
        for (int c = 0; c < 3; ++c) {
            s_g[t][c] = g[c];
            s_dvp[3 * t + c] = T[c] * g[0] + T[4 + c] * g[1] + T[8 + c] * g[2];
        }
        for (int j = 0; j < MANO_J; ++j) s_w[t][j] = m.weights[v * MANO_J + j];
    }
    MPH_MARK(1);
    const float tg0 = hm_block_sum(g[0], red), tg1 = hm_block_sum(g[1], red), tg2 = hm_block_sum(g[2], red);
    if (t == 0) { hm_partial_store(out + 337, tg0); hm_partial_store(out + 338, tg1); hm_partial_store(out + 339, tg2); }
    __syncthreads();
    MPH_MARK(2);
    if (t < 192) {
        const int j = t / 12, r = (t % 12) / 4, c = t % 4;
        float acc = 0.f;
        for (int i = 0; i < nv; ++i) acc += s_w[i][j] * s_g[i][r] * (c < 3 ? s_vp[i][c] : 1.0f);
        hm_partial_store(out + t, acc);
    }
    __syncthreads();
    MPH_MARK(3);
    const int wv = t >> 6, lane = t & 63;
    const int ne = 3 * nv;
    float d0 = 0.f, d1 = 0.f, d2 = 0.f;
    if (lane < ne) d0 = s_dvp[lane];
    if (lane + 64 < ne) d1 = s_dvp[lane + 64];
    if (lane + 128 < ne) d2 = s_dvp[lane + 128];
    constexpr int ROWS = (MANO_NF + 3) / 4;
    float r0[ROWS], r1[ROWS], r2[ROWS];
#pragma unroll
    for (int q = 0; q < ROWS; ++q) {
        const int k = wv + 4 * q;
        const float* row = m.M + (long)min(k, MANO_NF - 1) * (3 * MANO_V) + 3 * v0;
        r0[q] = lane < ne ? row[lane] : 0.f;
        r1[q] = lane + 64 < ne ? row[lane + 64] : 0.f;
        r2[q] = lane + 128 < ne ? row[lane + 128] : 0.f;
    }
#pragma unroll
    for (int q = 0; q < ROWS; ++q) {
        const int k = wv + 4 * q;
        float acc = r0[q] * d0;
        acc += r1[q] * d1;
        acc += r2[q] * d2;
        acc = hm_wave_sum(acc);
        if (lane == 0 && k < MANO_NF) hm_partial_store(out + 192 + k, acc);
    }
    asm volatile("s_waitcnt vmcnt(0)" ::: "memory");
    __syncthreads();
    MPH_MARK(4);
    if (t == 0) {
        const unsigned int ticket = atomicAdd(frame_cnt + lb, 1u);
        const int last = ticket == gridDim.x - 1u;
        if (last) atomicExch(frame_cnt + lb, 0u);
        s_flag = last;
    }
    __syncthreads();
    MPH_MARK(5);
    if (s_flag) {
        mano_bwd2_body(m, sh, w2, partials, gridDim.x, lb, b, pca_dim, g_pca_extra, w_extra, g_pca, g_rot, g_betas, g_trans);
        if (RIGID) {
            __syncthreads();
            if (t == 0) {
                float dr6[6];
                rot6d_backward(mr.rot6d + (long)b * 6, &w2.tot[340], dr6);
#pragma unroll
                for (int k = 0; k < 6; ++k) mr.g_rot6d[(long)b * 6 + k] = dr6[k];
#pragma unroll
                for (int k = 0; k < 3; ++k) mr.g_trans[(long)b * 3 + k] = w2.tot[349 + k];
            }
        }
#ifdef MANO_PHASES
        __syncthreads();
        MPH_MARK(6);
        if (t == 0) atomicAdd(&g_mano_ph[14], 1ull);
#endif
    }
}

extern "C" {
int hm_mano_fwd_rows(const void* const* model, const float* pca, int pca_dim, const float* rot, const float* betas,
                     const float* trans, int B, float* verts, float* joints, const float* rigid_rot6d,
                     const float* rigid_trans, const float* rigid_scale, float* verts_world, float* state, int clip_len,
                     int row0, int row_stride, hipStream_t stream)
{
    HM_CHECK_ARG(model && pca && rot && betas && verts && B > 0 && pca_dim >= 16 && row_stride >= 1 && row0 >= 0 && row0 < row_stride);
    HM_CHECK_ARG(clip_len >= 0 && (clip_len == 0 || (B * row_stride) % clip_len == 0));
    HM_CHECK_ARG(!verts_world || (rigid_rot6d && rigid_trans && rigid_scale));
    ManoModelDev m = {(const float*)model[0], (const float*)model[1], (const float*)model[2], (const float*)model[3],
                      (const float*)model[4], (const float*)model[5], (const float*)model[6], (const int*)model[7]};
    hipLaunchKernelGGL(k_mano_fwd, dim3(MANO_NCH64, (B + MANO_FPW - 1) / MANO_FPW), dim3(256), 0, stream, m, pca, pca_dim, rot, betas, trans, B, verts,
                       joints, rigid_rot6d, rigid_trans, rigid_scale, verts_world, state, clip_len ? clip_len : B * row_stride,
                       row0, row_stride);
    return hm_launch_status();
}
int hm_mano_fwd_clips(const void* const* model, const float* pca, int pca_dim, const float* rot, const float* betas,
                      const float* trans, int B, float* verts, float* joints, const float* rigid_rot6d,
                      const float* rigid_trans, const float* rigid_scale, float* verts_world, float* state, int clip_len,
                      hipStream_t stream)
{
    HM_CHECK_ARG(model && pca && rot && betas && verts && B > 0 && pca_dim >= 16 && HM_CLIP_LEN_OK(B, clip_len));
    HM_CHECK_ARG(!verts_world || (rigid_rot6d && rigid_trans && rigid_scale));
    ManoModelDev m = {(const float*)model[0], (const float*)model[1], (const float*)model[2], (const float*)model[3],
                      (const float*)model[4], (const float*)model[5], (const float*)model[6], (const int*)model[7]};
    hipLaunchKernelGGL(k_mano_fwd, dim3(MANO_NCH64, (B + MANO_FPW - 1) / MANO_FPW), dim3(256), 0, stream, m, pca, pca_dim, rot, betas, trans, B, verts,
                       joints, rigid_rot6d, rigid_trans, rigid_scale, verts_world, state, clip_len ? clip_len : B, 0, 1);
    return hm_launch_status();
}
int hm_mano_fwd(const void* const* model, const float* pca, int pca_dim, const float* rot, const float* betas,
                const float* trans, int B, float* verts, float* joints, const float* rigid_rot6d, const float* rigid_trans,
                const float* rigid_scale, float* verts_world, float* state, hipStream_t stream)
{
    return hm_mano_fwd_clips(model, pca, pca_dim, rot, betas, trans, B, verts, joints, rigid_rot6d, rigid_trans,
                             rigid_scale, verts_world, state, 0, stream);
}
size_t hm_mano_workspace_bytes(int B) { return 512 + (size_t)B * 4 + (size_t)B * MANO_NCH64 * MANO_PART * sizeof(float); }
size_t hm_mano_state_bytes(int B) { return (size_t)B * MANO_STATE_DW * sizeof(float); }
static int mano_bwd_launch(const void* const* model, const float* pca, int pca_dim, const float* rot, const float* betas, int B,
                           const float* g_verts, const float* g_pca_extra, float w_extra, float* g_pca, float* g_rot,
                           float* g_betas, float* g_trans, const float* state, void* workspace, int row0, int row_stride,
                           const ManoRigid& mr, hipStream_t stream)
{
    HM_CHECK_ARG(model && pca && rot && betas && (g_verts || mr.mesh) && g_pca && g_rot && g_betas && g_trans && workspace);
    HM_CHECK_ARG(B > 0 && pca_dim >= 16 && row_stride >= 1 && row0 >= 0 && row0 < row_stride);
    ManoModelDev m = {(const float*)model[0], (const float*)model[1], (const float*)model[2], (const float*)model[3],
                      (const float*)model[4], (const float*)model[5], (const float*)model[6], (const int*)model[7]};
    unsigned int* cnt = (unsigned int*)workspace;
    float* partials = (float*)((char*)workspace + 256 + (((size_t)B * 4 + 255) & ~(size_t)255));
    if (mr.mesh)
        hipLaunchKernelGGL(k_mano_bwd<true>, dim3(MANO_NCH64, B), dim3(256), 0, stream, m, pca, pca_dim, rot, betas,
                           g_verts, B, state, partials, cnt, pca_dim, g_pca_extra, w_extra, g_pca, g_rot, g_betas, g_trans, row0,
                           row_stride, mr);
    else
        hipLaunchKernelGGL(k_mano_bwd<false>, dim3(MANO_NCH64, B), dim3(256), 0, stream, m, pca, pca_dim, rot, betas,
                           g_verts, B, state, partials, cnt, pca_dim, g_pca_extra, w_extra, g_pca, g_rot, g_betas, g_trans, row0,
                           row_stride, mr);
    return hm_launch_status();
}
int hm_mano_bwd_rows(const void* const* model, const float* pca, int pca_dim, const float* rot, const float* betas, int B,
                     const float* g_verts, const float* g_pca_extra, float w_extra, float* g_pca, float* g_rot, float* g_betas,
                     float* g_trans, const float* state, void* workspace, int row0, int row_stride, hipStream_t stream)
{
    ManoRigid none;
    memset(&none, 0, sizeof(none));
    return mano_bwd_launch(model, pca, pca_dim, rot, betas, B, g_verts, g_pca_extra, w_extra, g_pca, g_rot, g_betas, g_trans,
                           state, workspace, row0, row_stride, none, stream);
}
int hm_mano_bwd_rigid_clips(const void* const* model, const float* pca, int pca_dim, const float* rot, const float* betas, int B,
                            const float* g_pca_extra, float w_extra, float* g_pca, float* g_rot, float* g_betas,
                            float* g_trans, const float* state, void* workspace, const float* mesh, const float* rigid_rot6d,
                            const float* rigid_scale, const float* const* g_terms, const float* weights, int n_terms,
                            const float* g_rigid, const float* g_frame, int frame_stride, float frame_scale,
                            float* g_rigid_rot6d, float* g_rigid_trans, int clip_len, hipStream_t stream)
{
    HM_CHECK_ARG(mesh && rigid_rot6d && rigid_scale && g_rigid_rot6d && g_rigid_trans && HM_CLIP_LEN_OK(B, clip_len));
    HM_CHECK_ARG(n_terms >= 0 && n_terms <= 5 && (n_terms == 0 || (g_terms && weights)));
    HM_CHECK_ARG(!g_frame || frame_stride >= 3);
    ManoRigid mr;
    memset(&mr, 0, sizeof(mr));
    mr.mesh = mesh; mr.rot6d = rigid_rot6d; mr.scale = rigid_scale; mr.clip_len = clip_len ? clip_len : B;
    for (int k = 0; k < 5; ++k) { mr.terms.p[k] = k < n_terms ? g_terms[k] : nullptr; mr.terms.w[k] = k < n_terms ? weights[k] : 0.f; }
    mr.g_rigid = g_rigid; mr.g_frame = g_frame; mr.frame_stride = frame_stride; mr.frame_scale = frame_scale;
    mr.g_rot6d = g_rigid_rot6d; mr.g_trans = g_rigid_trans;
    return mano_bwd_launch(model, pca, pca_dim, rot, betas, B, nullptr, g_pca_extra, w_extra, g_pca, g_rot, g_betas, g_trans,
                           state, workspace, 0, 1, mr, stream);
}
int hm_mano_bwd(const void* const* model, const float* pca, int pca_dim, const float* rot, const float* betas, int B,
                const float* g_verts, const float* g_pca_extra, float w_extra, float* g_pca, float* g_rot, float* g_betas,
                float* g_trans, const float* state, void* workspace, hipStream_t stream)
{
    return hm_mano_bwd_rows(model, pca, pca_dim, rot, betas, B, g_verts, g_pca_extra, w_extra, g_pca, g_rot, g_betas, g_trans,
                            state, workspace, 0, 1, stream);
}
#ifdef MANO_PHASES
int hm_debug_mano_phases(unsigned long long* out)
{
    unsigned long long z[16] = {0};
    (void)hipDeviceSynchronize();
    (void)hipMemcpyFromSymbol(out, HIP_SYMBOL(g_mano_ph), sizeof(z));
    (void)hipMemcpyToSymbol(HIP_SYMBOL(g_mano_ph), z, sizeof(z));
    return HM_OK;
}
#endif
}
```

homan_amd/fused.py:

```python
from collections import OrderedDict, defaultdict

import numpy as np
import torch

from . import lib as _lib
from .homan import HOMan
from .loopcommon import HmAdam, parameter_groups


def _morton_order(verts):
    v = verts.detach().float().cpu().numpy()
    lo, hi = v.min(0), v.max(0)
    q = np.clip(((v - lo) / np.maximum(hi - lo, 1e-12) * 1023.0).astype(np.int64), 0, 1023)
    code = np.zeros(len(v), np.int64)
    for bit in range(10):
        for ax in range(3):
            code |= ((q[:, ax] >> bit) & 1) << (3 * bit + ax)
    return torch.from_numpy(np.argsort(code, kind="stable").astype(np.int32))


_LOOP_STREAMS = {}


def _loop_streams(device):
    key = torch.device(device).index if torch.device(device).index is not None else torch.cuda.current_device()
    if key not in _LOOP_STREAMS:
        got, seen = [], {torch.cuda.current_stream(key).cuda_stream, torch.cuda.default_stream(key).cuda_stream}
        for _ in range(256):
            st = torch.cuda.Stream(device=key)
            if st.cuda_stream not in seen:
                seen.add(st.cuda_stream)
                got.append(st)
            if len(got) == 4:
                break
        assert len(got) == 4, "could not obtain four distinct HIP streams"
        _LOOP_STREAMS[key] = tuple(got)
    return _LOOP_STREAMS[key]


class FusedStepper:

    SLOTS = ["loss_pca", "loss_scale_obj", "loss_scale_hand", "loss_smooth_obj", "loss_smooth_hand", "loss_collision",
             "loss_contact", "loss_v2d_hand", "v2d_hand", "loss_sil_obj", "iou_object", "loss_inter",
             "handobj_maxdist", "loss_depth"]
    raster_reorder = 1

    def __init__(self, model, loss_weights, lr, max_steps, capture=True, shared_scale=False, group=None, collectives=True):
        from . import constants, ops
        from .clipbatch import ClipBatch, ClipReduceWorkspace
        for one in (model.models if isinstance(model, ClipBatch) else model if isinstance(model, (list, tuple)) else [model]):
            if len(one.hand_sides) not in (1, 2):
                raise NotImplementedError("one or two hands per frame")
            if getattr(one, "sil_mode", "nmr") != "nmr":
                raise NotImplementedError("sil_mode='soft': the fused loop renders hard silhouettes only (mode='graph' or 'eager')")
        m = self.model = model if isinstance(model, ClipBatch) else ClipBatch(model if isinstance(model, (list, tuple))
                                                                             else [model])
        if len({tuple(one.hand_sides) for one in m.models}) != 1:
            raise NotImplementedError("the clips of a batch share the hand side (one MANO model per launch)")
        if m.int_scales_hand.requires_grad or m.hand_proj_mode != "persp":
            raise NotImplementedError("FusedStepper covers optimize_mano_beta=True (the hand scale a buffer) and persp")
        self.h = h = len(m.models[0].hand_sides)
        kinds = {one.losses.inter_type for one in m.models}
        self.inter_min = kinds == {"min"}
        if len(kinds) != 1 or (self.inter_min and (h > 1 or m.C > 1)):
            raise NotImplementedError("inter_type='min' in the fused loop: one hand, one clip (else mode='graph' or 'eager')")
        if h > 1 and (m.C > 1 or shared_scale):
            raise NotImplementedError("two hands per frame: the fused loop takes one clip at a time (a batch of two-hand "
                                      "clips: one stepper per clip, or mode='graph')")
        lw = self.lw = {k: float(v) for k, v in loss_weights.items()}
        if lw.get("lw_depth", 0) > 0:
            if not getattr(m, "ordinal_depth", False):
                raise TypeError("compute_ordinal_depth_loss() missing 3 required positional arguments: "
                                "'masks', 'silhouettes', and 'depths'")
        self.shared_scale, self.group = bool(shared_scale), group
        self.collectives = bool(collectives)
        if self.shared_scale and not m.optimize_object_scale:
            raise ValueError("shared_scale needs models built with optimize_object_scale=True")
        self.L, self.c, self.ops = _lib.lib(), constants, ops
        dev = m.translations_object.device
        B, Vo, Vh = m.B, m.verts_object_og.shape[1], 778
        C, NS = m.C, len(self.SLOTS) + 1
        self.B, self.C, self.clip_len, self.NS = B, C, m.clip_len, NS
        self.use_aux = C > 1 and not lw.get("lw_depth", 0) > 0
        self.log_in_adam = not self.use_aux and not self.shared_scale
        self.side_own_vo = (self.h == 1 and C == 1 and not lw.get("lw_depth", 0) > 0 and not lw.get("lw_collision", 0) > 0 and
                            not lw.get("lw_contact", 0) > 0)
        self.merge_renders = self.h == 1 and lw.get("lw_depth", 0) > 0 and lw.get("lw_sil_obj", 0) > 0
        self.sil_reduce_in_bwd = not self.use_aux
        self.Vo, self.Vh, self.P = Vo, Vh, m.mano_pca_pose.shape[1]
        f = lambda *shape: torch.zeros(*shape, device=dev)
        N = self.N = B * h
        self.vo, self.vm, self.vh = f(B, Vo, 3), f(N, Vh, 3), f(N, Vh, 3)
        self.vo_b = torch.zeros_like(self.vo) if self.side_own_vo else self.vo
        self.vals = f(C, NS)
        on = lambda k: lw.get(k, 0.0) > 0
        self.on = dict(pca=on("lw_pca"), so=on("lw_scale_obj"), sh=on("lw_scale_hand"),
                       smooth=on("lw_smooth_hand") or on("lw_smooth_obj"), col=on("lw_collision"),
                       con=on("lw_contact"), v2d=on("lw_v2d_hand"), sil=on("lw_sil_obj"), inter=on("lw_inter"),
                       depth=on("lw_depth"))
        w = {"loss_pca": lw["lw_pca"] if self.on["pca"] else 0, "loss_scale_obj": lw["lw_scale_obj"] if self.on["so"] else 0,
             "loss_scale_hand": lw["lw_scale_hand"] if self.on["sh"] else 0,
             "loss_smooth_obj": lw["lw_smooth_obj"] if self.on["smooth"] else 0,
             "loss_smooth_hand": lw["lw_smooth_hand"] if self.on["smooth"] else 0,
             "loss_collision": lw["lw_collision"] if self.on["col"] else 0,
             "loss_contact": lw["lw_contact"] if self.on["con"] else 0,
             "loss_v2d_hand": lw["lw_v2d_hand"] if self.on["v2d"] else 0,
             "loss_sil_obj": lw["lw_sil_obj"] if self.on["sil"] else 0,
             "loss_inter": lw["lw_inter"] if self.on["inter"] else 0,
             "loss_depth": lw["lw_depth"] if self.on["depth"] else 0}
        self.w = w
        self.weights = torch.tensor([w.get(k, 0.0) for k in self.SLOTS], device=dev)
        self.keys = [k for k in self.SLOTS if self._reported(k)]
        self.U_pca, self.U_so, self.U_sh = f(N, self.P), f(C), f(C)
        self.U_smo, self.U_smh, self.U_v2d = f(B, Vo, 3), f(N, Vh, 3), f(N, Vh, 3)
        self.U_colh, self.U_colo, self.U_conh, self.U_cono = f(N, Vh, 3), f(B, Vo, 3), f(N, Vh, 3), f(B, Vo, 3)
        self.G_sil, self.G_int_h, self.G_int_o = f(B, Vo, 3), f(N, Vh, 3), f(B, Vo, 3)
        self.G_o, self.G_h, self.G_mesh = f(B, Vo, 3), f(N, Vh, 3), f(N, Vh, 3)
        self.g_pca_mano, self.g_so_part = f(N, self.P), f(B)
        self.rec = f(N, 8)
        if self.inter_min:
            self.G_min_h, self.tmp_inter, self.rows = f(N, Vh, 3), f(2), torch.arange(B, device=dev)
        if h > 1:
            self.vh_d = [f(B, Vh, 3) for _ in range(h)]
            self.nn_idx_d = [torch.zeros(B, Vh, dtype=torch.int32, device=dev) for _ in range(h)]
            self.nn_d2_d = [f(B, Vh) for _ in range(h)]
            self.U_conh_d, self.U_cono_d = [f(B, Vh, 3) for _ in range(h)], [f(B, Vo, 3) for _ in range(h)]
            self.U_colh2, self.U_col_d = f(N, Vh, 3), [f(B, Vh, 3) for _ in range(4)]
            self.U_colo_d = f(B, Vo, 3)
            self.rec_d, self.G_int_o_d = [f(B, 8) for _ in range(h)], [f(B, Vo, 3) for _ in range(h)]
            self.tmp_h, self.tmp_col = f(h, 4), f(3)
            self.rws_h = [ClipReduceWorkspace(dev, 1) for _ in range(h)]
            self.hand_ctx = [m.mano_model.ctx_mean if sd == "right" else m.mano_model._left_ctx(False)
                             for sd in m.models[0].hand_sides]
        self.nn_idx = torch.zeros(B, Vh, dtype=torch.int32, device=dev)
        self.nn_seed = torch.zeros((2 + (Vh + 127) // 128) * B, dtype=torch.int32, device=dev)
        self.nn_d2 = f(B, Vh)
        self.obj_order = _morton_order(m.verts_object_og[0]).to(dev)
        side = m.models[0].hand_sides[0]
        self.mctx = m.mano_model.ctx_mean if side == "right" else m.mano_model._left_ctx(False)
        self.hand_order = _morton_order(self.mctx.tensors[0]).to(dev)
        self.Vo, self.B = Vo, B
        with torch.no_grad():
            self.obj_spheres = self._group_spheres()
        self.pooled = f(B, m.sil_ctx.S, m.sil_ctx.S)
        sx = m.sil_ctx
        self.sil_K = sx.K_eff(m.camintr_rois_object).contiguous()
        self.sil_keep, self.sil_ref = sx.pad(m.keep_mask_object), sx.pad(m.ref_mask_object)
        self.up_sil, self.up_inter = torch.tensor([w["loss_sil_obj"]], device=dev), torch.tensor([w["loss_inter"]], device=dev)
        if self.on["depth"] and h > 1:
            ctx_o, ctx_hs, m_o, m_hs = m.models[0]._depth_contexts_hands()
            if ctx_o.padded:
                raise NotImplementedError("the fused loop renders the depth images at image_size % 32 == 0; other sizes: "
                                          "mode='graph' or 'eager'")
            self.dlayers = [(ctx_o, Vo, m_o)] + [(ctx_hs[i], Vh, m_hs[i]) for i in range(h)]
            self.dpairs = [(a, b) for a in range(h + 1) for b in range(a + 1, h + 1)]
            Sd = ctx_o.S
            self.dl_sil, self.dl_dep = [f(B, Sd, Sd) for _ in self.dlayers], [f(B, Sd, Sd) for _ in self.dlayers]
            self.dl_g = [f(B, Sd, Sd) for _ in self.dlayers]
            self.dp_part, self.dp_rec = [f(B * 8) for _ in self.dpairs], [f(8) for _ in self.dpairs]
            self.dp_out, self.dp_up = [f(1) for _ in self.dpairs], [f(1) for _ in self.dpairs]
            self.dp_g = [(f(B, Sd, Sd), f(B, Sd, Sd)) for _ in self.dpairs]
            self.rws_dp = [ClipReduceWorkspace(dev, 1) for _ in self.dpairs]
            self.G_dep_o, self.G_dep_h_d, self.G_dep_h = f(B, Vo, 3), [f(B, Vh, 3) for _ in range(h)], f(N, Vh, 3)
        elif self.on["depth"]:
            if C == 1:
                self.dctx = m.models[0].depth_contexts()
            else:
                m0_, size = m.models[0], int(m.image_size)
                for one in m.models:
                    if tuple(one.masks_object.shape[1:]) != (size, size) or tuple(one.masks_human.shape[1:]) != (size, size):
                        raise NotImplementedError("ordinal depth: instance masks must be (B, image_size, image_size)")
                self.dctx = (ops.SilhouetteContext(m0_.faces_object[:1].expand(B, -1, -1), Vo, B, size, dev),
                             ops.SilhouetteContext(m0_.faces_hand[:1].expand(B, -1, -1), 778, B, size, dev),
                             torch.cat([(one.masks_object != 0).to(torch.uint8) for one in m.models]).contiguous(),
                             torch.cat([(one.masks_human != 0).to(torch.uint8) for one in m.models]).contiguous())
            ctx_o, ctx_h = self.dctx[0], self.dctx[1]
            if ctx_o.padded:
                raise NotImplementedError("the fused loop renders the depth images at image_size % 32 == 0; other sizes: "
                                          "mode='graph' or 'eager'")
            Sd = ctx_o.S
            self.d_sil_o, self.d_dep_o, self.d_sil_h, self.d_dep_h = f(B, Sd, Sd), f(B, Sd, Sd), f(B, Sd, Sd), f(B, Sd, Sd)
            self.d_go, self.d_gh, self.d_part, self.d_rec = f(B, Sd, Sd), f(B, Sd, Sd), f(B * 8), f(C, 8)
            self.d_flags = torch.ones(2, B * Sd * (Sd // 64), dtype=torch.uint8, device=dev) if Sd % 64 == 0 else None
            self.rws_depth = ClipReduceWorkspace(dev, C)
            self.G_dep_o, self.G_dep_h = f(B, Vo, 3), f(B, Vh, 3)
            self.up_depth = torch.tensor([w["loss_depth"]], device=dev)
        for p in m.parameters():
            p.grad = None
        gp = [m.translations_object, m.rotations_object, m.translations_hand, m.rotations_hand]
        if m.optimize_mano:
            gp += [m.mano_pca_pose, m.mano_rot, m.mano_trans, m.mano_betas]
        if m.optimize_object_scale:
            gp.append(m.int_scales_object)
        for p in gp:
            p.grad = torch.zeros_like(p)
        self._build_optimizers(lr)
        self.log_buf = torch.zeros(max_steps, C, NS, device=dev)
        self.max_steps = max_steps
        self.rigid_ws_h, self.rigid_ws_o = (torch.zeros(self.L.hm_rigid_workspace_bytes(n), dtype=torch.uint8, device=dev)
                                            for n in (N, B))
        self.mano_state = torch.empty(self.L.hm_mano_state_bytes(N), dtype=torch.uint8, device=dev)
        self.graph = self.graph_b = self.graph_k = None
        self.graph_iters = 4 if C == 1 else 1
        self.cap_stream, self.side, self.aux, side = _loop_streams(dev)
        self.ev_vo, self.ev_pair, self.ev_sil, self.ev_fwd, self.ev_ras = (torch.cuda.Event() for _ in range(5))
        self.ev_dep, self.ev_dgrad, self.ev_lines = (torch.cuda.Event() for _ in range(3))
        self.reduce_ws_b = ClipReduceWorkspace(dev, C)
        self.reduce_ws_c, self.reduce_ws_d, self.reduce_ws_e = (ClipReduceWorkspace(dev, C) for _ in range(3))
        self.pairs_after_lines = C > 1 and self.on["sil"]
        self.mano_bwd_rigid = C == 1 or not (self.on["col"] or self.on["con"])
        self.pair_fused = C == 1
        if self.shared_scale:
            self._sync_shared_scale_start()
        side.wait_stream(torch.cuda.current_stream())
        with torch.cuda.stream(side):
            self.forward_backward()
        torch.cuda.current_stream().wait_stream(side)
        torch.cuda.synchronize()
        if self.on["sil"]:
            m.sil_ctx.calibrate()
        if self.on["depth"] and self.h == 1:
            self.dctx[1].calibrate()
        if capture:
            sb = 768 if (self.on["col"] or self.on["con"]) and C == 1 else 1024 if self.pairs_after_lines else 1280
            pad = 4096 if (self.on["col"] or self.on["con"]) and C == 1 else 0
            nn_pad = 34816 if C > 1 and not self.on["con"] else 0
            tune = _lib.lib()
            prev = tune.hm_tune_sweep_blocks(sb)
            prev_pad = tune.hm_tune_raster_lds_pad(pad)
            prev_reorder = tune.hm_tune_raster_reorder(self.raster_reorder)
            prev_nn_pad = tune.hm_tune_nn_lds_pad(nn_pad)
            try:
                self.graph = _lib.new_graph()
                with torch.cuda.graph(self.graph, stream=self.cap_stream):
                    self.forward_backward(log=not self.log_in_adam)
                    if not self.shared_scale:
                        self._capture_step()
                if self.shared_scale:
                    self.graph_b = _lib.new_graph()
                    with torch.cuda.graph(self.graph_b, stream=self.cap_stream):
                        self._spread_shared_scale_grad()
                        self.opt.step(zero_grad=False)
                elif self.graph_iters > 1:
                    self.graph_k = _lib.new_graph()
                    with torch.cuda.graph(self.graph_k, stream=self.cap_stream):
                        self._capture_iterations(self.graph_iters)
            finally:
                tune.hm_tune_sweep_blocks(prev)
                tune.hm_tune_raster_lds_pad(prev_pad)
                tune.hm_tune_raster_reorder(prev_reorder)
                tune.hm_tune_nn_lds_pad(prev_nn_pad)

    def reload(self, clip_inputs):
        m = self.model
        if len(clip_inputs) != m.C:
            raise ValueError(f"reload: {len(clip_inputs)} clips for a stepper of {m.C}")
        from .clipbatch import _PER_CLIP, _PER_FRAME
        with torch.no_grad():
            for c, (one, kw) in enumerate(zip(m.models, clip_inputs)):
                one.load_clip(**kw)
                if m.C > 1:
                    for k in _PER_FRAME + _PER_CLIP:
                        if hasattr(m, k) and not isinstance(getattr(m, k), torch.nn.Parameter):
                            m.clip_slice(getattr(m, k), c).copy_(getattr(one, k))
                    m.keep_sum[c:c + 1].copy_(one.losses.keep_sum)
            if m.C > 1:
                m.sil_ctx.invalidate_outputs()
            sx = m.sil_ctx
            if sx.padded:
                self.sil_K.copy_(sx.K_eff(m.camintr_rois_object))
                self.sil_keep.copy_(sx.pad(m.keep_mask_object))
                self.sil_ref.copy_(sx.pad(m.ref_mask_object))
            self.obj_spheres.copy_(self._group_spheres())
            if self.on["depth"] and self.h == 1 and m.C == 1:
                self.dctx = m.models[0].depth_contexts()
            elif self.on["depth"] and self.h == 1:
                CL = m.clip_len
                for c, one in enumerate(m.models):
                    self.dctx[2][c * CL:(c + 1) * CL].copy_((one.masks_object != 0).to(torch.uint8))
                    self.dctx[3][c * CL:(c + 1) * CL].copy_((one.masks_human != 0).to(torch.uint8))
            for st_m, st_v in self.opt.state:
                st_m.zero_()
                st_v.zero_()
            self.opt.step_t.zero_()
            self.vals.zero_()
            for p in m.parameters():
                if p.grad is not None:
                    p.grad.zero_()
            if self.shared_scale:
                self._sync_shared_scale_start()

    def _group_spheres(self):
        m, Vo, B = self.model, self.Vo, self.B
        ng = (Vo + 63) // 64
        vs = m.verts_object_og.detach()[:, self.obj_order.long()]
        pad = ng * 64 - Vo
        valid = torch.ones(Vo + pad, dtype=torch.bool, device=vs.device)
        if pad:
            vs = torch.cat([vs, vs[:, -1:].expand(-1, pad, -1)], 1)
            valid[Vo:] = False
        grp = vs.reshape(B, ng, 64, 3)
        wgt = valid.reshape(1, ng, 64, 1).float()
        ctr = (grp * wgt).sum(2) / wgt.sum(2)
        rad = ((grp - ctr[:, :, None]) ** 2).sum(-1).sqrt().amax(2)
        return torch.cat([ctr, rad[..., None]], -1).contiguous()

    def _dist_on(self):
        import torch.distributed as dist
        return (self.collectives and dist.is_available() and dist.is_initialized() and
                dist.get_world_size(self.group) > 1)

    def _sync_shared_scale_start(self):
        import torch.distributed as dist
        s = self.model.int_scales_object
        with torch.no_grad():
            s0 = s.data[:1].clone()
            if self._dist_on():
                from .dist import broadcast_shared_scalar, group_src
                broadcast_shared_scalar(s0, group_src(self.group), self.group)
            s.copy_(s0.expand_as(s))
        self.g_shared = torch.zeros(1, device=s.device)

    def _reduce_shared_scale_grad(self):
        if self._dist_on():
            from .dist import sync_shared_scalar_grad
            sync_shared_scalar_grad(self.g_shared, self.group)

    def _spread_shared_scale_grad(self):
        g = self.model.int_scales_object.grad
        g.copy_(self.g_shared.expand_as(g))

    def _reported(self, k):
        o = self.on
        return {"loss_pca": o["pca"], "loss_scale_obj": o["so"], "loss_scale_hand": o["sh"], "loss_smooth_obj": o["smooth"],
                "loss_smooth_hand": o["smooth"], "loss_collision": o["col"], "loss_contact": o["con"],
                "loss_v2d_hand": o["v2d"], "v2d_hand": o["v2d"], "loss_sil_obj": o["sil"], "iou_object": o["sil"],
                "loss_inter": o["inter"], "handobj_maxdist": o["inter"], "loss_depth": o["depth"]}[k]

    def _slot(self, name):
        i = self.SLOTS.index(name)
        return self.vals.data_ptr() + 4 * i

    def forward_backward(self, log=False):
        if self.h > 1:
            return self._forward_backward_hands(log)
        it = self._iteration_namespace(log)
        main = it.main
        self.side.wait_stream(main)
        self._issue_silhouette_chain(it)
        with torch.cuda.stream(self.side):
            self._issue_hand_forward(it)
            self._issue_pair_terms(it)
            if self.on["depth"]:
                self._issue_depth_terms(it)
            self._issue_hand_backward(it)
        self._issue_object_backward(it)
        self._issue_join(it)

    def _build_optimizers(self, lr):
        self.opt = HmAdam(parameter_groups(self.model, lr))

    def _capture_step(self):
        self.opt.step(zero_grad=False, log=self._adam_log())

    def _capture_iterations(self, K):
        for _ in range(K):
            self.forward_backward(log=not self.log_in_adam)
            self._capture_step()

    def _iteration_namespace(self, log=False):
        from types import SimpleNamespace
        m, P = self.model, _lib.ptr
        main = torch.cuda.current_stream()
        return SimpleNamespace(m=m, L=self.L, P=P, ck=_lib.check, B=self.B, Vo=self.Vo, Vh=self.Vh, c=self.c, on=self.on, w=self.w,
                               CL=self.clip_len, NS=self.NS, C=self.C, main=main, side=self.side, sa=main.cuda_stream,
                               sb=self.side.cuda_stream, rws_b=P(self.reduce_ws_b.buf), sctx=m.sil_ctx,
                               cctx=m.collision_ctx, pca=m.mano_pca_pose, rot=m.mano_rot, betas=m.mano_betas,
                               mtr=m.mano_trans if m.optimize_mano else None, npca=self.P * self.clip_len,
                               use_aux=self.use_aux, log=log)

    def _aux_block(self, it):
        (m, L, P, ck, on, CL, NS, C, sctx, use_aux, log) = \
            (it.m, it.L, it.P, it.ck, it.on, it.CL, it.NS, it.C, it.sctx, it.use_aux, it.log)
        if not use_aux:
            return
        with torch.cuda.stream(self.aux):
            self.aux.wait_event(self.ev_fwd)
            if on["sil"]:
                self.aux.wait_event(self.ev_ras)
                ck(sctx.reduce(keep_sum=m.keep_sum, loss_out=self._slot("loss_sil_obj"), clip_len=CL, out_stride=NS,
                               stream=self.aux.cuda_stream), "sil_reduce")
            if log:
                ck(L.hm_log_total_clips(P(self.vals), P(self.weights), len(self.SLOTS), P(self.opt.step_t),
                                        self.max_steps, P(self.log_buf), C, self.aux.cuda_stream), "log")

    def _issue_silhouette_chain(self, it):
        (m, L, ck, on, CL, NS, main, sa, sctx, use_aux) = \
            (it.m, it.L, it.ck, it.on, it.CL, it.NS, it.main, it.sa, it.sctx, it.use_aux)
        if on["sil"]:
            render = dict(verts=m.verts_object_og, K=self.sil_K, keep=self.sil_keep, ref=self.sil_ref, pooled=self.pooled,
                          rigid_rot6d=m.rotations_object, rigid_trans=m.translations_object, rigid_scale=m.int_scales_object,
                          rigid_abs=1, persistent_outputs=1, clip_len=CL, cam_verts_out=self.vo)
            fwd_args = dict(render, out_stride=NS, stream=sa)
            if self.merge_renders:
                arr = _lib.sil_renders([
                    self.dctx[0].render_fields(verts=m.verts_object_og, K=m.camintr, pooled=self.d_sil_o, pooled_depth=self.d_dep_o,
                                               rigid_rot6d=m.rotations_object, rigid_trans=m.translations_object,
                                               rigid_scale=m.int_scales_object, rigid_abs=1, persistent_outputs=1, clip_len=CL),
                    sctx.render_fields(**render)])
                ck(L.hm_sil_fwd_multi(arr, 2, 1, sa), "sil_fwd_multi(setup)")
                self.ev_sil.record(main)
                ck(L.hm_sil_fwd_multi(arr, 2, 2, sa), "sil_fwd_multi(raster)")
                self.ev_dep.record(main)
            elif self.side_own_vo:
                ck(sctx.forward(**fwd_args), "sil_fwd")
            else:
                ck(sctx.forward(phases=1, **fwd_args), "sil_fwd(setup)")
                self.ev_sil.record(main)
                ck(sctx.forward(phases=2, **fwd_args), "sil_fwd(raster)")
                if use_aux:
                    self.ev_ras.record(main)
            if on["depth"] and not self.merge_renders:
                self._depth_render(self.vo, self.dctx[0], self.d_sil_o, self.d_dep_o, sa)
                self.ev_dep.record(main)
            bwd_args = dict(upstream=self.up_sil, keep_sum=m.keep_sum, clip_len=CL,
                            loss_out=self._slot("loss_sil_obj") if self.sil_reduce_in_bwd else None, out_stride=NS, stream=sa)
            mode = 2 if self.lw["lw_sil_obj"] > 0 else 1
            if self.pairs_after_lines:
                ck(sctx.backward(self.vo, self.sil_K, mode, phases=1, **bwd_args), "sil_bwd(lines)")
                self.ev_lines.record(main)
                ck(sctx.backward(self.vo, self.sil_K, mode, phases=2, **bwd_args), "sil_bwd(sweeps)")
            else:
                ck(sctx.backward(self.vo, self.sil_K, mode, **bwd_args), "sil_bwd")

    def _issue_hand_forward(self, it):
        (m, L, P, ck, B, Vo, Vh, on, CL, NS, C, side, sb, rws_b, pca, rot, betas, mtr, npca) = \
            (it.m, it.L, it.P, it.ck, it.B, it.Vo, it.Vh, it.on, it.CL, it.NS, it.C, it.side, it.sb, it.rws_b, it.pca, it.rot, it.betas, it.mtr, it.npca)
        if not on["sil"]:
            ck(L.hm_rigid_fwd_clips(P(m.verts_object_og), P(m.rotations_object), P(m.translations_object),
                                    P(m.int_scales_object), 1, B, Vo, None, P(self.vo), CL, sb), "rigid_fwd(obj)")
        elif self.side_own_vo:
            ck(L.hm_rigid_fwd_clips(P(m.verts_object_og), P(m.rotations_object), P(m.translations_object),
                                    P(m.int_scales_object), 1, B, Vo, None, P(self.vo_b), CL, sb), "rigid_fwd(obj, side copy)")
        if m.optimize_mano:
            ck(L.hm_mano_fwd_clips(self.mctx.ptrs, P(pca), self.P, P(rot), P(betas), P(mtr), B, P(self.vm), None,
                                   P(m.rotations_hand), P(m.translations_hand), P(m.int_scales_hand), P(self.vh),
                                   P(self.mano_state), CL, sb),
               "mano_fwd + rigid(hand)")
        else:
            ck(L.hm_rigid_fwd_clips(P(m.verts_hand_og), P(m.rotations_hand), P(m.translations_hand),
                                    P(m.int_scales_hand), 0, B, Vh, None, P(self.vh), CL, sb), "rigid_fwd(hand)")
        pri = on["pca"] or on["so"] or on["sh"]
        fuse = self.pair_fused and on["inter"] and Vo <= 4096 and not self.inter_min
        nn_fused = fuse and not on["con"]
        nn_full_fused = fuse and on["con"]
        ht_fused = fuse and on["smooth"] and on["v2d"]
        ht_args = (P(m.ref_verts2d_hand), float(m.image_size), P(self.U_v2d), self._slot("loss_v2d_hand"), P(self.U_smh),
                   self._slot("loss_smooth_hand"), P(pca) if pri else None, npca,
                   P(m.int_scales_object), P(m.int_scale_object_mean), P(m.int_scales_hand),
                   P(m.int_scale_hand_mean), P(self.U_pca), P(self.U_so), P(self.U_sh), self._slot("loss_pca"))
        if ht_fused:
            pass
        elif on["smooth"] and on["v2d"]:
            ck(L.hm_hand_terms_fwd_clips(P(self.vh), P(m.camintr), 1, ht_args[0], ht_args[1], B, Vh, *ht_args[2:], rws_b, CL,
                                         NS, sb), "hand terms")
        else:
            if pri:
                ck(L.hm_priors_fwd_clips(P(pca), npca, P(m.int_scales_object), P(m.int_scale_object_mean),
                                         P(m.int_scales_hand), P(m.int_scale_hand_mean), P(self.U_pca), P(self.U_so),
                                         P(self.U_sh), self._slot("loss_pca"), C, NS, sb), "priors")
            if on["smooth"]:
                ck(L.hm_smooth_fwd_clips(P(self.vh), B, Vh, 1, P(self.U_smh), self._slot("loss_smooth_hand"), rws_b,
                                         CL, NS, sb), "smooth(hand)")
            if on["v2d"]:
                ck(L.hm_v2d_fwd_clips(P(self.vh), P(m.camintr), 1, P(m.ref_verts2d_hand), float(m.image_size), B, Vh,
                                      P(self.U_v2d), self._slot("loss_v2d_hand"), rws_b, CL, NS, sb), "v2d")
        if on["sil"]:
            if not self.side_own_vo:
                side.wait_event(self.ev_sil)
            if self.pairs_after_lines:
                side.wait_event(self.ev_lines)
        it.fuse = fuse
        it.ht_args = ht_args
        it.ht_fused = ht_fused
        it.nn_full_fused = nn_full_fused
        it.nn_fused = nn_fused

    def _issue_pair_terms(self, it):
        (m, L, P, ck, B, Vo, Vh, c, on, w, CL, NS, side, sb, rws_b, cctx, fuse, ht_args, ht_fused, nn_full_fused, nn_fused) = \
            (it.m, it.L, it.P, it.ck, it.B, it.Vo, it.Vh, it.c, it.on, it.w, it.CL, it.NS, it.side, it.sb, it.rws_b, it.cctx, it.fuse, it.ht_args, it.ht_fused, it.nn_full_fused, it.nn_fused)
        if on["col"]:
            ck(L.hm_collision_fwd_clips(P(self.vh), P(cctx.f0), Vh, cctx.f0.shape[0], P(self.vo_b), P(cctx.f1), Vo,
                                        cctx.f1.shape[0], B, c.SDF_SCALE_FACTOR, P(self.U_colh), P(self.U_colo),
                                        self._slot("loss_collision"), P(cctx.ws), CL, NS, sb), "collision")
        if on["smooth"] and not fuse:
            ck(L.hm_smooth_fwd_clips(P(self.vo_b), B, Vo, 1, P(self.U_smo), self._slot("loss_smooth_obj"), rws_b, CL, NS,
                                     sb), "smooth(obj)")
        def search_and_contact():
            if (on["con"] or on["inter"]) and not nn_fused and not nn_full_fused:
                full = on["con"] or Vo > 4096 or self.inter_min
                ck(L.hm_nn_fwd_rigid_clips(P(self.vh), P(self.vo_b), B, Vh, Vo, P(self.nn_idx) if full else None,
                                           P(self.nn_d2) if full else None, self._slot("handobj_maxdist"), rws_b, CL, NS,
                                           P(self.obj_order), P(self.obj_spheres), P(m.rotations_object),
                                           P(m.translations_object), P(m.int_scales_object), P(self.hand_order),
                                           None if full else P(self.nn_seed), sb), "nn")
            if on["con"]:
                ck(L.hm_contact_fwd_clips(P(self.vh), P(self.vo_b), P(self.nn_idx), B, Vh, Vo, c.COLLISION_THRESH,
                                          P(self.U_conh), P(self.U_cono), self._slot("loss_contact"), rws_b, CL, NS, sb),
                   "contact")
        if not nn_full_fused:
            search_and_contact()
        if fuse:
            ck(L.hm_pair_terms_fwd_clips(P(self.vh), P(self.vo_b), P(m.camintr), B, Vh, Vo,
                                         self._slot("handobj_maxdist") if (nn_fused or nn_full_fused) else None,
                                         P(self.obj_order), rws_b,
                                         c.INTERACTION_BBOX_EXPANSION, float(c.INTERACTION_Z_THRESH), P(self.rec),
                                         self._slot("loss_inter"), P(self.reduce_ws_c.buf),
                                         P(self.U_smo) if on["smooth"] else None,
                                         self._slot("loss_smooth_obj") if on["smooth"] else None, P(self.reduce_ws_d.buf),
                                         *(ht_args if ht_fused else (None, 0.0, None, None, None, None, None, 0, None, None,
                                                                     None, None, None, None, None, None)),
                                         P(self.reduce_ws_e.buf), P(self.obj_spheres), P(m.rotations_object),
                                         P(m.translations_object), P(m.int_scales_object), P(self.hand_order),
                                         P(self.nn_idx) if nn_full_fused else None, P(self.nn_d2) if nn_full_fused else None,
                                         P(self.nn_seed), CL, NS, sb),
               "pair terms")
            if nn_full_fused:
                search_and_contact()
        elif on["inter"]:
            ck(L.hm_inter_fwd_clips(P(self.vh), P(self.vo_b), P(m.camintr), B, Vh, Vo, c.INTERACTION_BBOX_EXPANSION,
                                    float(c.INTERACTION_Z_THRESH), P(self.rec),
                                    P(self.tmp_inter) if self.inter_min else self._slot("loss_inter"), rws_b, CL,
                                    NS, sb), "inter")
        if on["inter"] and self.inter_min:
            with torch.cuda.stream(side):
                flags = (self.rec[:, 0] != 0).float()
                i_star = self.nn_d2.argmin(1)
                j_star = self.nn_idx.gather(1, i_star[:, None]).long()[:, 0]
                diff = self.vh[self.rows, i_star] - self.vo_b[self.rows, j_star]
                self.vals[0, self.SLOTS.index("loss_inter")] = ((diff * diff).sum(1) * flags).sum()
                pull = (2.0 * w["loss_inter"]) * diff * flags[:, None]
                self.G_min_h.zero_()
                self.G_min_h[self.rows, i_star] = pull
                if m.optimize_object_scale:
                    self.G_int_o.zero_()
                    self.G_int_o[self.rows, j_star] = -pull
        elif on["inter"] and m.optimize_object_scale:
            ck(L.hm_inter_bwd(P(self.rec), P(self.up_inter), B, Vh, Vo, None, P(self.G_int_o), sb), "inter_bwd")

    def _issue_depth_terms(self, it):
        (m, L, P, ck, B, Vo, Vh, on, CL, NS, C, side, sb) = \
            (it.m, it.L, it.P, it.ck, it.B, it.Vo, it.Vh, it.on, it.CL, it.NS, it.C, it.side, it.sb)
        if on["depth"]:
            ctx_o, ctx_h, m_o, m_h = self.dctx
            Sd, K = ctx_o.S, P(m.camintr)
            self._depth_render(self.vh, ctx_h, self.d_sil_h, self.d_dep_h, sb)
            if on["sil"]:
                side.wait_event(self.ev_dep)
            else:
                self._depth_render(self.vo, ctx_o, self.d_sil_o, self.d_dep_o, sb)
            rw_bytes = L.hm_reduce_workspace_bytes()
            for ci in range(C):
                fr = slice(ci * CL, (ci + 1) * CL)
                args = (P(self.d_dep_o[fr]), P(self.d_dep_h[fr]), P(self.d_sil_o[fr]), P(self.d_sil_h[fr]), P(m_o[fr]),
                        P(m_h[fr]), CL, Sd)
                ck(L.hm_ordinal_depth_fwd(*args, P(self.d_part[8 * ci * CL:]), P(self.d_rec[ci]),
                                          self._slot("loss_depth") + 4 * NS * ci,
                                          self.rws_depth.buf.data_ptr() + rw_bytes * ci, sb), "ordinal depth")
                if self.d_flags is not None:
                    fo = ci * CL * Sd * (Sd // 64)
                    ck(L.hm_ordinal_depth_bwd_flags(*args, P(self.d_rec[ci]), P(self.up_depth), P(self.d_go[fr]), P(self.d_gh[fr]),
                                                    self.d_flags[0].data_ptr() + fo, self.d_flags[1].data_ptr() + fo, sb),
                       "ordinal depth bwd")
                else:
                    ck(L.hm_ordinal_depth_bwd(*args, P(self.d_rec[ci]), P(self.up_depth), P(self.d_go[fr]), P(self.d_gh[fr]),
                                              sb), "ordinal depth bwd")
            self.ev_dgrad.record(side)
            for verts, ctx, V_, g, G, li in (((self.vh, ctx_h, Vh, self.d_gh, self.G_dep_h, 1),) if on["sil"] else
                                             ((self.vo, ctx_o, Vo, self.d_go, self.G_dep_o, 0),
                                              (self.vh, ctx_h, Vh, self.d_gh, self.G_dep_h, 1))):
                ck(L.hm_depth_bwd_sparse(P(verts), K, B, V_, ctx.F, Sd, 1.0, P(g), P(ctx.adj_off), P(ctx.adj_items), P(G),
                                         P(self.d_flags[li]) if self.d_flags is not None else None, P(ctx.workspace), sb),
                   "depth bwd")

    def _issue_hand_backward(self, it):
        (m, L, P, ck, B, Vh, on, w, CL, pca, rot, betas, mtr, side, sb) = \
            (it.m, it.L, it.P, it.ck, it.B, it.Vh, it.on, it.w, it.CL, it.pca, it.rot, it.betas, it.mtr, it.side, it.sb)
        self.ev_fwd.record(side)
        self._aux_block(it)
        self.ev_pair.record(side)
        tp, tw, tn = _lib.terms([(self.U_smh if on["smooth"] else None, w["loss_smooth_hand"]),
                                 (self.U_v2d if on["v2d"] else None, w["loss_v2d_hand"]),
                                 (self.U_colh if on["col"] else None, w["loss_collision"]),
                                 (self.U_conh if on["con"] else None, w["loss_contact"]),
                                 (self.G_dep_h if on["depth"] else None, 1.0)])
        g_rig = P(self.G_min_h) if (on["inter"] and self.inter_min) else None
        g_frm = (self.rec.data_ptr() + 8) if (on["inter"] and not self.inter_min) else None
        if m.optimize_mano and self.mano_bwd_rigid:
            ck(L.hm_mano_bwd_rigid_clips(self.mctx.ptrs, P(pca), self.P, P(rot), P(betas), B,
                                         P(self.U_pca) if on["pca"] else None, w["loss_pca"], P(pca.grad), P(rot.grad),
                                         P(betas.grad), P(mtr.grad), P(self.mano_state), P(self.mctx.workspace(B)),
                                         P(self.vm), P(m.rotations_hand), P(m.int_scales_hand), tp, tw, tn, g_rig, g_frm, 8,
                                         w["loss_inter"] / Vh, P(m.rotations_hand.grad), P(m.translations_hand.grad), CL,
                                         sb), "mano_bwd + rigid_bwd(hand)")
        else:
            ck(L.hm_rigid_bwd_clips(P(self.vm if m.optimize_mano else m.verts_hand_og), P(m.rotations_hand),
                                    P(m.int_scales_hand), 0, tp, tw, tn, g_rig, g_frm, 8, w["loss_inter"] / Vh, B, Vh,
                                    P(self.G_mesh) if m.optimize_mano else None, P(m.rotations_hand.grad),
                                    P(m.translations_hand.grad), None, P(self.rigid_ws_h), CL, sb), "rigid_bwd(hand)")
            if m.optimize_mano:
                ck(L.hm_mano_bwd(self.mctx.ptrs, P(pca), self.P, P(rot), P(betas), B, P(self.G_mesh),
                                 P(self.U_pca) if on["pca"] else None, w["loss_pca"], P(pca.grad), P(rot.grad),
                                 P(betas.grad), P(mtr.grad), P(self.mano_state), P(self.mctx.workspace(B)), sb),
                   "mano_bwd")

    def _issue_object_backward(self, it):
        (m, L, P, ck, B, Vo, on, w, CL, main, sa, sctx) = \
            (it.m, it.L, it.P, it.ck, it.B, it.Vo, it.on, it.w, it.CL, it.main, it.sa, it.sctx)
        if on["depth"] and on["sil"]:
            main.wait_event(self.ev_dgrad)
            ctx_o = self.dctx[0]
            ck(L.hm_depth_bwd_sparse(P(self.vo), P(m.camintr), B, Vo, ctx_o.F, ctx_o.S, 1.0, P(self.d_go), P(ctx_o.adj_off),
                                     P(ctx_o.adj_items), P(self.G_dep_o),
                                     P(self.d_flags[0]) if self.d_flags is not None else None, P(ctx_o.workspace), sa),
               "depth bwd(obj)")
        sc_obj = m.optimize_object_scale
        sm_in = on["smooth"] and on["sil"] and Vo <= 24576
        side_terms = on["con"] or (on["inter"] and sc_obj) or (on["smooth"] and not sm_in) or not on["sil"]
        if side_terms:
            main.wait_event(self.ev_pair)
        tp, tw, tn = _lib.terms([(self.U_smo if (on["smooth"] and not sm_in) else None, w["loss_smooth_obj"]),
                                 (self.U_cono if on["con"] else None, w["loss_contact"]),
                                 (self.G_int_o if (on["inter"] and sc_obj) else None, 1.0),
                                 (self.G_dep_o if on["depth"] else None, 1.0)])
        if on["sil"]:
            ck(L.hm_rigid_bwd_sil_clips(P(m.verts_object_og), P(m.rotations_object), P(m.int_scales_object), 1, tp, tw, tn,
                                        sctx.parts_ptr(), P(sctx.adj_off),
                                        P(sctx.adj_items), P(self.vo), P(self.sil_K), 1.0, sctx.F, B, Vo,
                                        P(m.rotations_object.grad), P(m.translations_object.grad),
                                        P(self.g_so_part) if sc_obj else None, P(self.rigid_ws_o), CL, sctx.sum_log2q,
                                        P(self.vo) if sm_in else None, w["loss_smooth_obj"], sa),
               "rigid_bwd(obj) + silhouette gather")
        else:
            ck(L.hm_rigid_bwd_clips(P(m.verts_object_og), P(m.rotations_object), P(m.int_scales_object), 1, tp, tw, tn, None,
                                    None, 0, 0.0, B, Vo, None, P(m.rotations_object.grad), P(m.translations_object.grad),
                                    P(self.g_so_part) if sc_obj else None, P(self.rigid_ws_o), CL, sa), "rigid_bwd(obj)")
        it.sc_obj = sc_obj

    def _issue_join(self, it):
        (m, L, P, ck, on, w, CL, C, main, side, sa, use_aux, log, sc_obj) = \
            (it.m, it.L, it.P, it.ck, it.on, it.w, it.CL, it.C, it.main, it.side, it.sa, it.use_aux, it.log, it.sc_obj)
        main.wait_stream(side)
        if use_aux:
            main.wait_stream(self.aux)
        elif log:
            ck(L.hm_log_total_clips(P(self.vals), P(self.weights), len(self.SLOTS), P(self.opt.step_t),
                                    self.max_steps, P(self.log_buf), C, sa), "log")
        if sc_obj:
            ck(L.hm_sum_small_clips(P(self.g_so_part), CL, 1.0, P(self.U_so) if on["so"] else None, w["loss_scale_obj"],
                                    P(m.int_scales_object.grad), C, sa), "scale grad")
            if self.shared_scale:
                ck(L.hm_sum_small_clips(P(m.int_scales_object.grad), C, 1.0, None, 0.0, P(self.g_shared), 1, sa),
                   "shared scale grad")

    def _forward_backward_hands(self, log=False):
        from .fused_hands import forward_backward_hands
        return forward_backward_hands(self, log)

    def sil_chain_only(self):
        m, ck = self.model, _lib.check
        sctx, CL, NS = m.sil_ctx, self.clip_len, self.NS
        sa = torch.cuda.current_stream().cuda_stream
        ck(sctx.forward(verts=m.verts_object_og, K=self.sil_K, keep=self.sil_keep, ref=self.sil_ref, pooled=self.pooled,
                        rigid_rot6d=m.rotations_object, rigid_trans=m.translations_object, rigid_scale=m.int_scales_object,
                        rigid_abs=1, persistent_outputs=1, clip_len=CL, cam_verts_out=self.vo, out_stride=NS, stream=sa), "sil_fwd")
        ck(sctx.backward(self.vo, self.sil_K, 2, upstream=self.up_sil, keep_sum=m.keep_sum, clip_len=CL, out_stride=NS, stream=sa),
           "sil_bwd")

    def _depth_render(self, verts, ctx, sil, dep, stream_id):
        _lib.check(ctx.forward(verts=verts, K=self.model.camintr, pooled=sil, pooled_depth=dep, persistent_outputs=1,
                               stream=stream_id), "depth render")

    def _adam_log(self):
        if not self.log_in_adam:
            return None
        return (self.vals, self.weights, len(self.SLOTS), self.max_steps, self.log_buf, self.C)

    def _iteration(self):
        if self.graph is not None:
            self.graph.replay()
            if self.shared_scale:
                self._reduce_shared_scale_grad()
                self.graph_b.replay()
        else:
            self.forward_backward(log=not self.log_in_adam)
            if self.shared_scale:
                self._reduce_shared_scale_grad()
                self._spread_shared_scale_grad()
            self.opt.step(zero_grad=False, log=self._adam_log())

    def run(self, steps):
        if self.graph_k is not None:
            while steps >= self.graph_iters:
                self.graph_k.replay()
                steps -= self.graph_iters
        for _ in range(steps):
            self._iteration()

    def loss_evolution(self, steps, clip=None):
        torch.cuda.synchronize()
        host = self.log_buf[:steps].cpu().numpy()

        def one(ci):
            out = {k: host[:, ci, self.SLOTS.index(k)].astype(np.float64).tolist() for k in self.keys}
            out["loss"] = host[:, ci, len(self.SLOTS)].astype(np.float64).tolist()
            return out
        if clip is not None:
            return one(clip)
        return one(0) if self.C == 1 else [one(ci) for ci in range(self.C)]
```

homan_amd/loopcommon.py:

```python
import ctypes
import os
from collections import OrderedDict, defaultdict

import numpy as np
import torch

from . import lib as _lib
from .homan import HOMan


def _tensorify(x):
    if isinstance(x, torch.Tensor):
        return x
    a = np.asarray(x)
    return torch.from_numpy(a.astype(np.float32) if a.dtype.kind == "f" else a)


def collate_inputs(person_parameters, object_parameters, objvertices, objfaces):
    cat = torch.cat
    pp, op = person_parameters, object_parameters
    return dict(
        hand_sides=pp[0]["hand_side"],
        translations_object=cat([o["translations"] for o in op]),
        rotations_object=cat([o["rotations"] for o in op]),
        verts_object_og=_tensorify(objvertices),
        faces_object=_tensorify(objfaces),
        target_masks_object=cat([o["target_masks"] for o in op]),
        target_masks_hand=cat([p["target_masks"] for p in pp]),
        verts_hand_og=cat([p["verts"] for p in pp]),
        ref_verts2d_hand=cat([p["verts2d"] for p in pp]),
        mano_trans=cat([p["mano_trans"] for p in pp]),
        mano_rot=cat([p["mano_rot"] for p in pp]),
        mano_pca_pose=cat([p["mano_pca_pose"] for p in pp]),
        mano_betas=cat([p["mano_betas"] for p in pp]),
        translations_hand=cat([p["translations"] for p in pp]),
        rotations_hand=cat([p["rotations"] for p in pp]),
        faces_hand=pp[0]["faces"],
        masks_object=cat([o["full_mask"].unsqueeze(0) for o in op]),
        masks_hand=cat([p["masks"] for p in pp]),
        cams_hand=cat([p["cams"] for p in pp]),
        camintr_rois_object=cat([o["K_roi"][:, 0] for o in op]),
        camintr_rois_hand=cat([p["K_roi"] for p in pp]),
    )


def parameter_groups(model, lr):
    rigid = [v for k, v in model.named_parameters() if "mano" not in k and "rotation" not in k]
    rotation = [v for k, v in model.named_parameters() if ("rotation" in k) and ("mano" not in k)]
    return [{"params": rigid, "lr": lr},
            {"params": [model.mano_pca_pose, model.mano_betas], "lr": lr * 10},
            {"params": rotation, "lr": lr * 10}]


class HmAdam:

    def __init__(self, groups, betas=(0.9, 0.999), eps=1e-8):
        self.betas, self.eps = betas, eps
        self.items = []
        for g in groups:
            for p in g["params"]:
                if isinstance(p, torch.nn.Parameter) and p.requires_grad and p.grad is not None:
                    self.items.append((p, float(g["lr"])))
        assert self.items, "run one backward before building HmAdam (static gradient buffers)"
        dev = self.items[0][0].device
        self.state = [(torch.zeros_like(p), torch.zeros_like(p)) for p, _ in self.items]
        self.step_t = torch.zeros(2, dtype=torch.int32, device=dev)
        slot = np.zeros(len(self.items), dtype=[("p", "u8"), ("g", "u8"), ("m", "u8"), ("v", "u8"), ("n", "i8"),
                                                 ("lr", "f4"), ("pad", "i4")])
        assert slot.itemsize == _lib.lib().hm_adam_slot_bytes()
        for i, ((p, lr), (m, v)) in enumerate(zip(self.items, self.state)):
            assert p.is_contiguous() and p.grad.is_contiguous()
            slot[i] = (p.data_ptr(), p.grad.data_ptr(), m.data_ptr(), v.data_ptr(), p.numel(), lr, 0)
        self.slots = torch.from_numpy(slot.view(np.uint8).copy()).to(dev)
        self.grads = [p.grad for p, _ in self.items]
        self.blocks = max(1, min(64, (max(p.numel() for p, _ in self.items) + 255) // 256))

    def step(self, zero_grad=True, log=None):
        for (p, _), g in zip(self.items, self.grads):
            assert p.grad is g, "gradient buffers must stay static (do not call zero_grad(set_to_none=True))"
        if log is not None:
            vals, weights, n, max_steps, log_buf, nclips = log
            _lib.check(_lib.lib().hm_adam_step_log(_lib.ptr(self.slots), len(self.items), _lib.ptr(self.step_t),
                                                   self.betas[0], self.betas[1], self.eps, int(zero_grad), self.blocks,
                                                   _lib.ptr(vals), _lib.ptr(weights), n, max_steps, _lib.ptr(log_buf),
                                                   nclips, _lib.stream()), "hm_adam_step_log")
            return
        _lib.check(_lib.lib().hm_adam_step(_lib.ptr(self.slots), len(self.items), _lib.ptr(self.step_t),
                                           self.betas[0], self.betas[1], self.eps, int(zero_grad), self.blocks,
                                           _lib.stream()), "hm_adam_step")


class _DeviceLog:

    def __init__(self, keys, max_steps, step_t):
        self.keys = list(keys)
        self.buf = torch.zeros(max_steps, len(self.keys), device=step_t.device)
        self.max_steps, self.step_t = max_steps, step_t

    def record(self, scalars):
        packed = torch.cat([scalars[k].detach().reshape(1) for k in self.keys])
        _lib.check(_lib.lib().hm_log_scalars(_lib.ptr(packed), len(self.keys), _lib.ptr(self.step_t),
                                             self.max_steps, _lib.ptr(self.buf), _lib.stream()), "hm_log_scalars")


def _weighted_total(loss_dict, loss_weights):
    return sum(loss_dict[k] * loss_weights[k.replace("loss", "lw")] for k in loss_dict)


def build_model(person_parameters, object_parameters, class_name="default", objvertices=None, objfaces=None,
                camintr=None, hand_proj_mode="persp", optimize_mano=False, optimize_mano_beta=True,
                optimize_object_scale=False, state_dict=None, image_size=640, mano_model=None, rend_size=256,
                sync_metrics=True, ordinal_depth=False, sil_mode="nmr", sil_sigma=1e-4):
    kw = collate_inputs(person_parameters, object_parameters, objvertices, objfaces)
    model = HOMan(camintr=camintr, class_name=class_name, int_scale_init=1, hand_proj_mode=hand_proj_mode,
                  optimize_mano=optimize_mano, optimize_mano_beta=optimize_mano_beta,
                  optimize_object_scale=optimize_object_scale, image_size=image_size, mano_model=mano_model,
                  rend_size=rend_size, sync_metrics=sync_metrics, ordinal_depth=ordinal_depth, sil_mode=sil_mode,
                  sil_sigma=sil_sigma, **kw)
    if state_dict is not None:
        model.load_state_dict(state_dict, strict=False)
    return model
```

include/homan_amd.h:

```cpp
#ifndef HOMAN_AMD_H
#define HOMAN_AMD_H

#include <stddef.h>

#ifdef __cplusplus
extern "C" {
#endif

#ifndef HIP_INCLUDE_HIP_HIP_RUNTIME_API_H
typedef struct ihipStream_t* hipStream_t;
#endif

#define HM_OK 0
#define HM_ERR_BAD_ARG (-1)
#define HM_ERR_LAUNCH (-2)
#define HM_ERR_UNSUPPORTED (-3)

int hm_rigid_fwd(const float* mesh, const float* rot6d, const float* trans, const float* scale, int abs_scale, int N,
                 int V, float* rotmat, float* verts, hipStream_t stream);
int hm_rigid_bwd(const float* mesh, const float* rot6d, const float* scale, int abs_scale, const float* const* g_terms,
                 const float* weights, int n_terms, const float* g_rigid, const float* g_frame, int frame_stride,
                 float frame_scale, int N, int V, float* g_mesh, float* g_rot6d, float* g_trans, float* g_scale_part,
                 void* workspace, hipStream_t stream);
size_t hm_rigid_workspace_bytes(int N);
int hm_rigid_bwd_sil(const float* mesh, const float* rot6d, const float* scale, int abs_scale, const float* const* g_terms,
                     const float* weights, int n_terms, const double* sil_parts, const int* adj_off, const int* adj_items,
                     const float* cam_verts, const float* K, float orig_size, int F, int N, int V, float* g_rot6d,
                     float* g_trans, float* g_scale_part, void* workspace, int sum_log2q, hipStream_t stream);
int hm_offscreen_fwd(const float* verts, const float* K, int N, int V, float zfar, float weight, float* out, float* grad,
                     hipStream_t stream);
int hm_pose_keep_best(const float* sums, int stride, const float* extra, int n, const float* rot6d, const float* trans,
                      float* best_loss, float* best_rot6d, float* best_trans, float* losses_out, hipStream_t stream);
int hm_pose_keep_best_log(const float* sums, int stride, const float* extra, int n, const float* rot6d, const float* trans,
                          const int* step, int max_steps, float* log, float* losses_out, hipStream_t stream);
int hm_edge_edt(const float* ref, int size, int stride, int kernel_size, float power, float* edt, int* band_count,
                hipStream_t stream);
size_t hm_pose_edge_workspace_bytes(int N, int stride);
int hm_pose_edge_terms(const float* alpha, const float* keep, const float* ref, const float* edt, int N, int size, int stride,
                       int kernel_size, float lw_chamfer, float* terms, float* grad, void* workspace, hipStream_t stream);
int hm_scale_by(const float* in, const float* s, long n, float* out, hipStream_t stream);

int hm_mano_fwd(const void* const* model, const float* pca, int pca_dim, const float* rot, const float* betas,
                const float* trans, int B, float* verts, float* joints, const float* rigid_rot6d, const float* rigid_trans,
                const float* rigid_scale, float* verts_world, float* state, hipStream_t stream);
size_t hm_mano_workspace_bytes(int B);
size_t hm_mano_state_bytes(int B);
int hm_mano_bwd(const void* const* model, const float* pca, int pca_dim, const float* rot, const float* betas, int B,
                const float* g_verts, const float* g_pca_extra, float w_extra, float* g_pca, float* g_rot, float* g_betas,
                float* g_trans, const float* state, void* workspace, hipStream_t stream);
int hm_mano_bwd_rigid_clips(const void* const* model, const float* pca, int pca_dim, const float* rot, const float* betas, int B,
                            const float* g_pca_extra, float w_extra, float* g_pca, float* g_rot, float* g_betas,
                            float* g_trans, const float* state, void* workspace, const float* mesh, const float* rigid_rot6d,
                            const float* rigid_scale, const float* const* g_terms, const float* weights, int n_terms,
                            const float* g_rigid, const float* g_frame, int frame_stride, float frame_scale,
                            float* g_rigid_rot6d, float* g_rigid_trans, int clip_len, hipStream_t stream);

size_t hm_sil_workspace_bytes(int B, int V, int F, int S);
int hm_sil_fwd(const float* verts, const int* faces, int faces_bstride, const float* K, int B, int V, int F, int S,
               float orig_size, float znear, float zfar, const float* keep, const float* ref,
               const float* keep_sum, float* pooled, float* loss_out, const int* work_order, float* pooled_depth,
               float* alpha_full, int mask_shared, const float* rigid_rot6d, const float* rigid_trans,
               const float* rigid_scale, int rigid_abs, int persistent_outputs, void* workspace, hipStream_t stream);
int hm_sil_hint_near_winding(void* workspace, int winding, hipStream_t stream);
int hm_sil_reduce(int B, int V, int F, int S, const float* keep_sum, float* loss_out, float* frame_out, void* workspace,
                  hipStream_t stream);
int hm_sil_bwd(const float* verts, const float* K, int B, int V, int F, int S, float orig_size, float eps, int mode,
               const float* upstream, const float* grad_pooled, const float* keep_sum, const int* adj_off,
               const int* adj_items, float* grad_verts, float* grad_ndc, void* workspace,
               int sum_log2q, hipStream_t stream);
int hm_depth_bwd(const float* verts, const float* K, int B, int V, int F, int S, float orig_size,
                 const float* grad_pooled_depth, const int* adj_off, const int* adj_items, float* grad_verts,
                 void* workspace, hipStream_t stream);
int hm_depth_bwd_sparse(const float* verts, const float* K, int B, int V, int F, int S, float orig_size,
                        const float* grad_pooled_depth, const int* adj_off, const int* adj_items, float* grad_verts,
                        const unsigned char* gflags, void* workspace, hipStream_t stream);
int hm_ordinal_depth_fwd(const float* d0, const float* d1, const float* a0, const float* a1, const unsigned char* m0,
                         const unsigned char* m1, int B, int S, float* frame_part, float* rec, float* out1,
                         void* workspace, hipStream_t stream);
int hm_ordinal_depth_bwd(const float* d0, const float* d1, const float* a0, const float* a1, const unsigned char* m0,
                         const unsigned char* m1, int B, int S, const float* rec, const float* upstream, float* g0,
                         float* g1, hipStream_t stream);
int hm_ordinal_depth_bwd_flags(const float* d0, const float* d1, const float* a0, const float* a1, const unsigned char* m0,
                               const unsigned char* m1, int B, int S, const float* rec, const float* upstream, float* g0,
                               float* g1, unsigned char* flags0, unsigned char* flags1, hipStream_t stream);
int hm_tune_sweep_blocks(int blocks);
int hm_tune_raster_lds_pad(int bytes);
int hm_tune_raster_reorder(int enable);
int hm_tune_nn_lds_pad(int bytes);
int hm_debug_sweep_caps(int cap);
int hm_shade_rgb(const float* verts, const int* faces, int faces_bstride, const float* textures, int B, int V, int F, int S,
                 const float* light_dir, float intensity_ambient, float intensity_directional, const float* background,
                 float* rgb, void* workspace, hipStream_t stream);
const double* hm_sil_parts(const void* workspace, int B, int V, int F, int S);
int hm_sil_read_idx_map(const void* workspace, int B, int V, int F, int S, int* out, hipStream_t stream);
int hm_sil_read_faces9(const void* workspace, int B, int V, int F, int S, float* out, hipStream_t stream);
int hm_sil_invalidate_outputs(void* workspace, int B, int V, int F, int S, hipStream_t stream);
int hm_sil_read_parts(const void* workspace, int B, int V, int F, int S, double* out, hipStream_t stream);
int hm_sil_read_boxes(const void* workspace, int B, int V, int F, int S, void* out, hipStream_t stream);

size_t hm_softsil_workspace_bytes(int B, int V, int F, int S);
int hm_softsil_fwd(const float* verts, const int* faces, const float* K, int B, int V, int F, int S, float orig_size,
                   float znear, float zfar, const float* sigma, float* alpha, void* workspace, hipStream_t stream);
int hm_softsil_bwd(const float* verts, const int* faces, const float* K, int B, int V, int F, int S, float orig_size,
                   float znear, float zfar, const float* sigma, const float* alpha, const float* grad_alpha,
                   const int* adj_off, const int* adj_items, float* grad_verts, void* workspace, hipStream_t stream);

size_t hm_reduce_workspace_bytes(void);
int hm_v2d_fwd(const float* verts, const float* camintr, int hand_nb, const float* ref2d, float image_size, int N,
               int V, float* unit_grad, float* out2, void* workspace, hipStream_t stream);
int hm_smooth_fwd(const float* verts, int N, int V, int hand_nb, float* unit_grad, float* out1, void* workspace,
                  hipStream_t stream);
int hm_priors_fwd(const float* pca, long npca, const float* s_obj, const float* m_obj, const float* s_hand,
                  const float* m_hand, float* g_pca, float* g_sobj, float* g_shand, float* out3, hipStream_t stream);
int hm_inter_fwd(const float* verts_hand, const float* verts_obj, const float* camintr, int B, int Vh, int Vo,
                 float expansion, float zthresh, float* frame_rec, float* out1, void* workspace, hipStream_t stream);
int hm_inter_bwd(const float* frame_rec, const float* upstream, int B, int Vh, int Vo, float* g_hand, float* g_obj,
                 hipStream_t stream);

int hm_nn_fwd(const float* verts_hand, const float* verts_obj, int B, int Vh, int Vo, int* nn_idx, float* nn_d2,
              float* metric_out, void* workspace, hipStream_t stream);
int hm_contact_fwd(const float* verts_hand, const float* verts_obj, const int* nn_idx, int B, int Vh, int Vo,
                   float thresh, float* g_hand, float* g_obj, float* out1, void* workspace, hipStream_t stream);

size_t hm_cloud_metrics_workspace_bytes(int B, int N, int M);
int hm_cloud_metrics(const float* x, const float* y, int B, int N, int M, const float* aff_x, const float* aff_y, float* x_d2,
                     int* x_idx, float* y_d2, int* y_idx, double* out4, void* workspace, hipStream_t stream);
int hm_align_stats(const float* gt_hand, const float* pred_hand, int B, int hands, int V, int pred_centroid_from_gt,
                   float* aff_gt, float* aff_pred, double* hand_mean, hipStream_t stream);

int hm_keyframe_interp(const float* key_vals, const int* key_frames, int K, int N, int frame_nb, const int* gather, int M,
                       const float* signs, int out_f64, int* key_frames_dev, int* gather_dev, void* out, hipStream_t stream);

int hm_mask_crop_resize(const void* masks, int masks_f32, int N, int H, int W, const int* index, const float* boxes, int R,
                        int S, unsigned char* out, hipStream_t stream);
int hm_target_masks(int mode, const void* target, int target_f32, int Nt, const int* target_index, const void* occluders,
                    int occluders_f32, int No, const int* occluder_index, int K, int H, int W, const float* boxes, int R, int S,
                    float* out, hipStream_t stream);
int hm_instance_masks(const int* idx_map, int B, int S, int F, const int* face_start, int I, unsigned char* out,
                      hipStream_t stream);

size_t hm_collision_workspace_bytes(int B, int V0, int V1, int F0, int F1);
int hm_collision_fwd(const float* verts0, const int* faces0, int V0, int F0, const float* verts1, const int* faces1,
                     int V1, int F1, int B, float scale_factor, float* g0, float* g1, float* out1, void* workspace,
                     hipStream_t stream);
int hm_collision_dist_values(const float* verts0, int V0, const float* verts1, int V1, int F0, int F1, int B, float* dv0,
                             float* dv1, void* workspace, hipStream_t stream);
int hm_collision_read_grid(const int* faces, int V, int F, int B, int which, int V0, int V1, int F0, int F1, float* phi,
                           void* workspace, hipStream_t stream);
int hm_collision_read_needed(int B, int which, int V0, int V1, int F0, int F1, void* need_mask, int* need_len, float* phi,
                             void* workspace, hipStream_t stream);

size_t hm_adam_slot_bytes(void);
int hm_adam_step(const void* slots, int n_tensors, int* step, float beta1, float beta2, float eps, int zero_grad,
                 int blocks_per_tensor, hipStream_t stream);
int hm_adam_step_log(const void* slots, int n_tensors, int* step, float beta1, float beta2, float eps, int zero_grad,
                     int blocks_per_tensor, float* vals, const float* weights, int n, int max_steps, float* log, int nclips,
                     hipStream_t stream);
int hm_log_scalars(const float* src, int n, const int* step, int max_steps, float* log, hipStream_t stream);

int hm_rigid_fwd_clips(const float* mesh, const float* rot6d, const float* trans, const float* scale, int abs_scale, int N,
                       int V, float* rotmat, float* verts, int clip_len, hipStream_t stream);
int hm_rigid_bwd_clips(const float* mesh, const float* rot6d, const float* scale, int abs_scale,
                       const float* const* g_terms, const float* weights, int n_terms, const float* g_rigid,
                       const float* g_frame, int frame_stride, float frame_scale, int N, int V, float* g_mesh,
                       float* g_rot6d, float* g_trans, float* g_scale_part, void* workspace, int clip_len,
                       hipStream_t stream);
int hm_rigid_bwd_sil_clips(const float* mesh, const float* rot6d, const float* scale, int abs_scale,
                           const float* const* g_terms, const float* weights, int n_terms, const double* sil_parts,
                           const int* adj_off, const int* adj_items, const float* cam_verts, const float* K,
                           float orig_size, int F, int N, int V, float* g_rot6d, float* g_trans, float* g_scale_part,
                           void* workspace, int clip_len, int sum_log2q, const float* smooth_verts, float smooth_weight,
                           hipStream_t stream);
int hm_sum_small_clips(const float* parts, int n, float w0, const float* extra, float w1, float* out, int nclips,
                       hipStream_t stream);
int hm_mano_fwd_clips(const void* const* model, const float* pca, int pca_dim, const float* rot, const float* betas,
                      const float* trans, int B, float* verts, float* joints, const float* rigid_rot6d,
                      const float* rigid_trans, const float* rigid_scale, float* verts_world, float* state, int clip_len,
                      hipStream_t stream);
int hm_mano_fwd_rows(const void* const* model, const float* pca, int pca_dim, const float* rot, const float* betas,
                     const float* trans, int B, float* verts, float* joints, const float* rigid_rot6d,
                     const float* rigid_trans, const float* rigid_scale, float* verts_world, float* state, int clip_len,
                     int row0, int row_stride, hipStream_t stream);
int hm_mano_bwd_rows(const void* const* model, const float* pca, int pca_dim, const float* rot, const float* betas, int B,
                     const float* g_verts, const float* g_pca_extra, float w_extra, float* g_pca, float* g_rot, float* g_betas,
                     float* g_trans, const float* state, void* workspace, int row0, int row_stride, hipStream_t stream);
int hm_sil_fwd_clips(const float* verts, const int* faces, int faces_bstride, const float* K, int B, int V, int F, int S,
                     float orig_size, float znear, float zfar, const float* keep, const float* ref,
                     const float* keep_sum, float* pooled, float* loss_out, const int* work_order, float* pooled_depth,
                     float* alpha_full, int mask_shared, const float* rigid_rot6d, const float* rigid_trans,
                     const float* rigid_scale, int rigid_abs, int persistent_outputs, void* workspace, int clip_len,
                     int out_stride, float* cam_verts_out, hipStream_t stream);
int hm_sil_fwd_phase_clips(const float* verts, const int* faces, int faces_bstride, const float* K, int B, int V, int F, int S,
                           float orig_size, float znear, float zfar, const float* keep, const float* ref,
                           const float* keep_sum, float* pooled, float* loss_out, const int* work_order, float* pooled_depth,
                           float* alpha_full, int mask_shared, const float* rigid_rot6d, const float* rigid_trans,
                           const float* rigid_scale, int rigid_abs, int persistent_outputs, void* workspace, int clip_len,
                           int out_stride, float* cam_verts_out, int phases, hipStream_t stream);
typedef struct HmSilRender {
    const float* verts; const int* faces; const float* K; const float* keep; const float* ref; float* pooled;
    const int* work_order; float* pooled_depth; const float* rigid_rot6d; const float* rigid_trans; const float* rigid_scale;
    float* cam_verts_out; void* workspace;
    int faces_bstride, B, V, F, S, mask_shared, rigid_abs, persistent_outputs, clip_len;
    float orig_size, znear, zfar;
} HmSilRender;
int hm_sil_fwd_multi(const HmSilRender* renders, int n, int phases, hipStream_t stream);
size_t hm_sil_render_bytes(void);
int hm_sil_reduce_clips(int B, int V, int F, int S, const float* keep_sum, float* loss_out, float* frame_out,
                        void* workspace, int clip_len, int out_stride, hipStream_t stream);
int hm_sil_bwd_clips(const float* verts, const float* K, int B, int V, int F, int S, float orig_size, float eps, int mode,
                     const float* upstream, const float* grad_pooled, const float* keep_sum, const int* adj_off,
                     const int* adj_items, float* grad_verts, float* grad_ndc, void* workspace,
                     int clip_len, float* loss_out, int out_stride, int sum_log2q, hipStream_t stream);
int hm_sil_bwd_phase_clips(const float* verts, const float* K, int B, int V, int F, int S, float orig_size, float eps, int mode,
                     const float* upstream, const float* grad_pooled, const float* keep_sum, const int* adj_off,
                     const int* adj_items, float* grad_verts, float* grad_ndc, void* workspace,
                     int clip_len, float* loss_out, int out_stride, int phases, int sum_log2q, hipStream_t stream);
int hm_v2d_fwd_clips(const float* verts, const float* camintr, int hand_nb, const float* ref2d, float image_size, int N,
                     int V, float* unit_grad, float* out2, void* workspace, int clip_len, int out_stride,
                     hipStream_t stream);
int hm_smooth_fwd_clips(const float* verts, int N, int V, int hand_nb, float* unit_grad, float* out1, void* workspace,
                        int clip_len, int out_stride, hipStream_t stream);
int hm_priors_fwd_clips(const float* pca, long npca, const float* s_obj, const float* m_obj, const float* s_hand,
                        const float* m_hand, float* g_pca, float* g_sobj, float* g_shand, float* out3, int nclips,
                        int out_stride, hipStream_t stream);
int hm_hand_terms_fwd_clips(const float* verts, const float* camintr, int hand_nb, const float* ref2d, float image_size,
                            int N, int V, float* unit_v2d, float* out_v2d2, float* unit_smooth, float* out_smooth1,
                            const float* pca, long npca, const float* s_obj, const float* m_obj, const float* s_hand,
                            const float* m_hand, float* g_pca, float* g_sobj, float* g_shand, float* out_priors3,
                            void* workspace, int clip_len, int out_stride, hipStream_t stream);
int hm_inter_fwd_clips(const float* verts_hand, const float* verts_obj, const float* camintr, int B, int Vh, int Vo,
                       float expansion, float zthresh, float* frame_rec, float* out1, void* workspace, int clip_len,
                       int out_stride, hipStream_t stream);
int hm_pair_terms_fwd_clips(const float* verts_hand, const float* verts_obj, const float* camintr, int B, int Vh, int Vo,
                            float* metric_out, const int* obj_order, void* ws_nn, float expansion, float zthresh,
                            float* frame_rec, float* out_inter, void* ws_inter, float* unit_smooth, float* out_smooth,
                            void* ws_smooth,
                            const float* ht_ref2d, float ht_image_size, float* ht_unit_v2d, float* ht_out_v2d2,
                            float* ht_unit_smooth, float* ht_out_smooth1, const float* ht_pca, long ht_npca,
                            const float* ht_s_obj, const float* ht_m_obj, const float* ht_s_hand, const float* ht_m_hand,
                            float* ht_g_pca, float* ht_g_sobj, float* ht_g_shand, float* ht_out_priors3, void* ws_hand,
                            const float* obj_spheres, const float* obj_rot6d, const float* obj_trans, const float* obj_scale,
                            const int* hand_order, int* nn_idx, float* nn_d2, int* nn_seed,
                            int clip_len, int out_stride, hipStream_t stream);
int hm_nn_fwd_clips(const float* verts_hand, const float* verts_obj, int B, int Vh, int Vo, int* nn_idx, float* nn_d2,
                    float* metric_out, void* workspace, int clip_len, int out_stride, const int* obj_order,
                    hipStream_t stream);
int hm_nn_fwd_rigid_clips(const float* verts_hand, const float* verts_obj, int B, int Vh, int Vo, int* nn_idx, float* nn_d2,
                          float* metric_out, void* workspace, int clip_len, int out_stride, const int* obj_order,
                          const float* obj_spheres, const float* obj_rot6d, const float* obj_trans, const float* obj_scale,
                          const int* hand_order, int* nn_seed, hipStream_t stream);
int hm_contact_fwd_clips(const float* verts_hand, const float* verts_obj, const int* nn_idx, int B, int Vh, int Vo,
                         float thresh, float* g_hand, float* g_obj, float* out1, void* workspace, int clip_len,
                         int out_stride, hipStream_t stream);
int hm_collision_fwd_clips(const float* verts0, const int* faces0, int V0, int F0, const float* verts1, const int* faces1,
                           int V1, int F1, int B, float scale_factor, float* g0, float* g1, float* out1, void* workspace,
                           int clip_len, int out_stride, hipStream_t stream);
int hm_log_total_clips(float* vals, const float* weights, int n, const int* step, int max_steps, float* log, int nclips,
                       hipStream_t stream);

int hm_bench_sil_kernels(const float* verts, const int* faces, const float* K, int B, int V, int F, int S,
                         const float* keep, const float* ref, const float* keep_sum, float* pooled, float* loss_out,
                         const int* work_order, const int* adj_off, const int* adj_items,
                         const float* upstream, float* grad_verts, void* workspace, int reps, float* avg_ms,
                         hipStream_t stream);
size_t hm_sil_timestamps_bytes(int B, int V, int F, int S);
int hm_sil_timestamps(void* workspace, int B, int V, int F, int S, int enable, hipStream_t stream);
int hm_sil_timestamps_save(const void* workspace, int B, int V, int F, int S, void* dst, hipStream_t stream);
int hm_sil_timestamps_read(const void* workspace, int B, int V, int F, int S, const void* saved, float* us3, hipStream_t stream);

#ifdef __cplusplus
}
#endif
#endif
```

Measured before the change: 6605.

## Fuse Adam updates into the tails of the hand and object backward kernels

Adds an Adam 'tail' to the rigid object backward and the MANO+rigid hand backward kernels. Each block applies the Adam update to its per-frame parameters right after computing their gradients. The last arriving block does the loss logging and advances the step counter, so the separate Adam kernel launch is no longer needed in the captured step. This shortens the dependent kernel chain per iteration, at the cost of extra atomics, a serial logging loop in one thread, and more code paths. It also forces the object stream to wait on the pair event.

```diff
diff --git a/homan_amd/csrc/adam.hip b/homan_amd/csrc/adam.hip
--- a/homan_amd/csrc/adam.hip
+++ b/homan_amd/csrc/adam.hip
@@ -17,15 +17,6 @@
     v[n] = t;
     if (s < max_steps)
         for (int i = 0; i <= n; ++i) log[((long)s * nc + c) * (n + 1) + i] = v[i];
-}
-__device__ __forceinline__ double adam_pow(double b, int t)
-{
-    double r = 1.0;
-    for (; t > 0; t >>= 1) {
-        if (t & 1) r = r * b;
-        b = b * b;
-    }
-    return r;
 }
 __global__ __launch_bounds__(256) void k_adam(const AdamSlot* __restrict__ slots, int n_tensors, int* __restrict__ step,
                                                float beta1, float beta2, float eps, int zero_grad, float* __restrict__ vals,
@@ -47,19 +38,11 @@
         return;
     }
     const AdamSlot s = slots[blockIdx.y];
-    const double bc1 = 1.0 - adam_pow((double)beta1, step_now + 1);
-    const double bc2 = 1.0 - adam_pow((double)beta2, step_now + 1);
-    const float neg_step = (float)(-((double)s.lr / bc1));
-    const float bc2_sqrt = (float)sqrt(bc2);
-    const float w1 = (float)(1.0 - (double)beta1), w2 = (float)(1.0 - (double)beta2);
+    const HmAdamBias bias = hm_adam_bias(beta1, beta2, step_now);
     for (long i = (long)blockIdx.x * blockDim.x + threadIdx.x; i < s.n; i += (long)gridDim.x * blockDim.x) {
         const float g = s.g[i];
         float m = s.m[i], v = s.v[i];
-        m = m + w1 * (g - m);
-        v = v * beta2;
-        v = v + (w2 * g) * g;
-        const float denom = sqrtf(v) / bc2_sqrt + eps;
-        s.p[i] = s.p[i] + (neg_step * m) / denom;
+        s.p[i] = hm_adam_elem(s.p[i], g, m, v, s.lr, beta1, beta2, eps, bias);
         s.m[i] = m;
         s.v[i] = v;
         if (zero_grad) s.g[i] = 0.f;
@@ -99,6 +82,7 @@
     return hm_launch_status();
 }
 size_t hm_adam_slot_bytes(void) { return sizeof(AdamSlot); }
+size_t hm_adam_tail_bytes(void) { return sizeof(HmAdamTail); }
 
 int hm_adam_step(const void* slots, int n_tensors, int* step, float beta1, float beta2, float eps, int zero_grad,
                  int blocks_per_tensor, hipStream_t stream)
diff --git a/homan_amd/csrc/geometry.hip b/homan_amd/csrc/geometry.hip
--- a/homan_amd/csrc/geometry.hip
+++ b/homan_amd/csrc/geometry.hip
@@ -186,19 +186,21 @@
 }
 
 struct SmoothIn { const float* verts; float w; };
-template <int NV, int MAXT>
+template <int NV, int MAXT, bool ADAM>
 __global__ __launch_bounds__(MAXT) void k_rigid_bwd_x(const float* __restrict__ mesh, const float* __restrict__ rot6d,
                                                      const float* __restrict__ scale, int abs_scale, RigidTerms terms,
                                                      SilGather sil, SmoothIn sm, int N, int V, float* __restrict__ g_rot6d,
                                                      float* __restrict__ g_trans, float* __restrict__ g_scale_part,
                                                      float* __restrict__ partials, unsigned int* __restrict__ frame_cnt,
-                                                     int clip_len, double magic)
+                                                     int clip_len, double magic, const HmAdamTail* __restrict__ tail)
 {
     HM_LATENCY_KERNEL();
     HM_STAMP_START(1);
     __shared__ double red13d[16 * 13];
     __shared__ int s_flag;
     const int n = blockIdx.x;
+    HmTailEntry te;
+    if constexpr (ADAM) te = hm_tail_enter(tail);
     float R[9];
     rot6d_to_mat(rot6d + n * 6, R);
     const float sraw = scale[n / clip_len];
@@ -337,6 +339,21 @@
 #pragma unroll
         for (int k = 0; k < 3; ++k) g_trans[n * 3 + k] = tot[9 + k];
         if (g_scale_part) g_scale_part[n] = (abs_scale && sraw < 0.f) ? -tot[12] : tot[12];
+        if constexpr (ADAM) {
+            float* g9 = reinterpret_cast<float*>(red13d);
+#pragma unroll
+            for (int k = 0; k < 6; ++k) g9[k] = dr6[k];
+#pragma unroll
+            for (int k = 0; k < 3; ++k) g9[6 + k] = tot[9 + k];
+        }
+    }
+    if constexpr (ADAM) {
+        __syncthreads();
+        const float* g9 = reinterpret_cast<const float*>(red13d);
+        const int t = threadIdx.x;
+        if (t < 6) hm_tail_adam(tail, tail->t[0], n, t, g9[t], te);
+        else if (t < 9) hm_tail_adam(tail, tail->t[1], n, t - 6, g9[t], te);
+        else if (t == 64) hm_tail_arrive(tail, te.step_now);
     }
     HM_STAMP_END(1);
 }
@@ -384,7 +401,8 @@
                             const float* const* g_terms, const float* weights, int n_terms, SilGather sil,
                             const float* g_rigid, const float* g_frame, int frame_stride, float frame_scale, int N, int V,
                             float* g_mesh, float* g_rot6d, float* g_trans, float* g_scale_part, void* workspace,
-                            int clip_len, int exact, int sum_log2q, SmoothIn smooth, hipStream_t stream)
+                            int clip_len, int exact, int sum_log2q, SmoothIn smooth, hipStream_t stream,
+                            const HmAdamTail* tail = nullptr)
 {
     HM_CHECK_ARG(sum_log2q <= 0 && sum_log2q >= -60);
     HM_CHECK_ARG(mesh && rot6d && scale && g_rot6d && g_trans && N > 0 && V > 0 && HM_CLIP_LEN_OK(N, clip_len));
@@ -402,14 +420,17 @@
     if (exact && !g_rigid && !g_frame && !g_mesh && (workspace ? V <= RIGID_MAX_CHUNKS * thr * nv : V <= thr * nv)) {
         const int ch = hm_cdiv(V, thr * nv);
         const double magic = hm_sum_magic(sum_log2q);
-        if (nv == 2)
-            hipLaunchKernelGGL((k_rigid_bwd_x<2, 768>), dim3(N, ch), dim3(thr), 0, stream, mesh, rot6d, scale,
-                               abs_scale, t, sil, smooth, N, V, g_rot6d, g_trans, g_scale_part, partials, cnt, clip_len ? clip_len : N, magic);
-        else
-            hipLaunchKernelGGL((k_rigid_bwd_x<1, 1024>), dim3(N, ch), dim3(thr), 0, stream, mesh, rot6d, scale,
-                               abs_scale, t, sil, smooth, N, V, g_rot6d, g_trans, g_scale_part, partials, cnt, clip_len ? clip_len : N, magic);
+#define RIGID_X_LAUNCH(NV_, MAXT_, ADAM_) \
+        hipLaunchKernelGGL((k_rigid_bwd_x<NV_, MAXT_, ADAM_>), dim3(N, ch), dim3(thr), 0, stream, mesh, rot6d, scale, abs_scale, t, \
+                           sil, smooth, N, V, g_rot6d, g_trans, g_scale_part, partials, cnt, clip_len ? clip_len : N, magic, tail)
+        if (nv == 2 && tail) RIGID_X_LAUNCH(2, 768, true);
+        else if (nv == 2) RIGID_X_LAUNCH(2, 768, false);
+        else if (tail) RIGID_X_LAUNCH(1, 1024, true);
+        else RIGID_X_LAUNCH(1, 1024, false);
+#undef RIGID_X_LAUNCH
         return hm_launch_status();
     }
+    HM_CHECK_ARG(!tail);
     HM_CHECK_ARG(!smooth.verts);
     if (exact)
         hipLaunchKernelGGL(k_rigid_bwd<true>, dim3(N, chunks), dim3(threads), 0, stream, mesh, rot6d, scale,
@@ -453,6 +474,20 @@
                             nullptr, g_rot6d, g_trans, g_scale_part, workspace, clip_len, 1, sum_log2q,
                             SmoothIn{smooth_verts, smooth_weight}, stream);
 }
+int hm_rigid_bwd_sil_adam_clips(const float* mesh, const float* rot6d, const float* scale, int abs_scale,
+                                const float* const* g_terms, const float* weights, int n_terms, const double* sil_parts,
+                                const int* adj_off, const int* adj_items, const float* cam_verts, const float* K,
+                                float orig_size, int F, int N, int V, float* g_rot6d, float* g_trans, float* g_scale_part,
+                                void* workspace, int clip_len, int sum_log2q, const float* smooth_verts, float smooth_weight,
+                                const void* tail, hipStream_t stream)
+{
+    HM_CHECK_ARG(sil_parts && adj_off && adj_items && cam_verts && K && F > 0 && tail);
+    HM_CHECK_ARG(V > 0 && (workspace ? V <= RIGID_MAX_CHUNKS * 768 * 2 : V <= 256));
+    SilGather sil = {sil_parts, adj_off, adj_items, cam_verts, K, orig_size, F};
+    return rigid_bwd_launch(mesh, rot6d, scale, abs_scale, g_terms, weights, n_terms, sil, nullptr, nullptr, 0, 0.f, N, V,
+                            nullptr, g_rot6d, g_trans, g_scale_part, workspace, clip_len, 1, sum_log2q,
+                            SmoothIn{smooth_verts, smooth_weight}, stream, (const HmAdamTail*)tail);
+}
 int hm_rigid_bwd_sil(const float* mesh, const float* rot6d, const float* scale, int abs_scale, const float* const* g_terms,
                      const float* weights, int n_terms, const double* sil_parts, const int* adj_off, const int* adj_items,
                      const float* cam_verts, const float* K, float orig_size, int F, int N, int V, float* g_rot6d,
diff --git a/homan_amd/csrc/hm_common.h b/homan_amd/csrc/hm_common.h
--- a/homan_amd/csrc/hm_common.h
+++ b/homan_amd/csrc/hm_common.h
@@ -338,3 +338,94 @@
 }
 
 struct RigidTerms { const float* p[5]; float w[5]; };
+
+__device__ __forceinline__ double adam_pow(double b, int t)
+{
+    double r = 1.0;
+    for (; t > 0; t >>= 1) {
+        if (t & 1) r = r * b;
+        b = b * b;
+    }
+    return r;
+}
+struct HmAdamBias { double bc1; float bc2_sqrt; };
+__device__ __forceinline__ HmAdamBias hm_adam_bias(float beta1, float beta2, int step_now)
+{
+    HmAdamBias b;
+    b.bc1 = 1.0 - adam_pow((double)beta1, step_now + 1);
+    const double bc2 = 1.0 - adam_pow((double)beta2, step_now + 1);
+    b.bc2_sqrt = (float)sqrt(bc2);
+    return b;
+}
+__device__ __forceinline__ float hm_adam_elem(float p, float g, float& m, float& v, float lr, float beta1, float beta2,
+                                              float eps, const HmAdamBias& b)
+{
+    const float neg_step = (float)(-((double)lr / b.bc1));
+    const float w1 = (float)(1.0 - (double)beta1), w2 = (float)(1.0 - (double)beta2);
+    m = m + w1 * (g - m);
+    v = v * beta2;
+    v = v + (w2 * g) * g;
+    const float denom = sqrtf(v) / b.bc2_sqrt + eps;
+    return p + (neg_step * m) / denom;
+}
+
+#define HM_TAIL_TENSORS 4
+struct HmTailTensor { float* p; float* m; float* v; float lr; int per_frame; };
+struct HmAdamTail {
+    HmTailTensor t[HM_TAIL_TENSORS];
+    int* step;
+    float* vals; const float* weights; float* log;
+    float beta1, beta2, eps;
+    unsigned int target;
+    int log_n, max_steps, nclips, pad;
+};
+struct HmTailEntry { int step_now; HmAdamBias bias; };
+__device__ __forceinline__ HmTailEntry hm_tail_enter(const HmAdamTail* __restrict__ tl)
+{
+    HmTailEntry e;
+    e.step_now = __builtin_amdgcn_readfirstlane(__hip_atomic_load(tl->step, __ATOMIC_RELAXED, __HIP_MEMORY_SCOPE_AGENT));
+    e.bias = hm_adam_bias(tl->beta1, tl->beta2, e.step_now);
+    return e;
+}
+__device__ __forceinline__ void hm_tail_adam(const HmAdamTail* __restrict__ tl, const HmTailTensor& ts, long frame, int k, float g,
+                                             const HmTailEntry& e)
+{
+    const long i = frame * ts.per_frame + k;
+    float m = ts.m[i], v = ts.v[i];
+    ts.p[i] = hm_adam_elem(ts.p[i], g, m, v, ts.lr, tl->beta1, tl->beta2, tl->eps, e.bias);
+    ts.m[i] = m;
+    ts.v[i] = v;
+}
+__device__ __forceinline__ void hm_tail_log_clip(float* vals, const float* __restrict__ w, int n, int s, int max_steps,
+                                                 float* __restrict__ log, int c, int nc)
+{
+    float* v = vals + (long)c * (n + 1);
+    float* row = log + ((long)s * nc + c) * (n + 1);
+    float t = 0.f;
+    for (int i0 = 0; i0 < n; i0 += 16) {
+        float x[16], ww[16];
+#pragma unroll
+        for (int j = 0; j < 16; ++j) {
+            x[j] = i0 + j < n ? __hip_atomic_load(v + i0 + j, __ATOMIC_RELAXED, __HIP_MEMORY_SCOPE_AGENT) : 0.f;
+            ww[j] = i0 + j < n ? w[i0 + j] : 0.f;
+        }
+#pragma unroll
+        for (int j = 0; j < 16; ++j) {
+            if (i0 + j < n && ww[j] != 0.f) t += ww[j] * x[j];
+            if (i0 + j < n && s < max_steps) row[i0 + j] = x[j];
+        }
+    }
+    v[n] = t;
+    if (s < max_steps) row[n] = t;
+}
+__device__ __forceinline__ void hm_tail_arrive(const HmAdamTail* __restrict__ tl, int step_now)
+{
+    unsigned int* cnt = reinterpret_cast<unsigned int*>(tl->step) + 1;
+    if (atomicAdd(cnt, 1u) == tl->target - 1u) {
+        if (tl->vals)
+            for (int c = 0; c < tl->nclips; ++c)
+                hm_tail_log_clip(tl->vals, tl->weights, tl->log_n, step_now, tl->max_steps, tl->log, c, tl->nclips);
+        atomicExch(cnt, 0u);
+        atomicExch(tl->step, step_now + 1);
+    }
+}
diff --git a/homan_amd/csrc/mano.hip b/homan_amd/csrc/mano.hip
--- a/homan_amd/csrc/mano.hip
+++ b/homan_amd/csrc/mano.hip
@@ -298,11 +298,13 @@
     float dRw[MANO_J][9], dtw[MANO_J][3], dJ[MANO_J][3], dRl[MANO_J][9], dpose[48];
     float cR[MANO_J][9], ct[MANO_J][3], cJ[MANO_J][3];
 };
+template <bool KEEP = false>
 __device__ __forceinline__ void mano_bwd2_body(const ManoModelDev& m, const ManoShared& sh, ManoBwd2Shared& w,
                                                const float* __restrict__ partials, int nchunk, int lb, int b, int pca_dim,
                                                const float* __restrict__ g_pca_extra, float w_extra,
                                                float* __restrict__ g_pca, float* __restrict__ g_rot,
-                                               float* __restrict__ g_betas, float* __restrict__ g_trans)
+                                               float* __restrict__ g_betas, float* __restrict__ g_trans,
+                                               float* keep = nullptr)
 {
     const int t = threadIdx.x, nt = blockDim.x;
     for (int k = t; k < MANO_PART; k += nt) {
@@ -402,6 +404,7 @@
         }
         if (g_pca_extra) a += w_extra * g_pca_extra[(long)b * pca_dim + i];
         g_pca[(long)b * pca_dim + i] = a;
+        if constexpr (KEEP) { if (i == t) keep[0] = a; }
     }
     if (t < 10) {
         float a = w.tot[192 + 135 + t];
@@ -411,6 +414,7 @@
 #pragma unroll
         for (int q = 0; q < MANO_J * 3; ++q) a += jv[q] * w.dJ[q / 3][q % 3];
         g_betas[b * 10 + t] = a;
+        if constexpr (KEEP) keep[1] = a;
     }
 }
 
@@ -432,7 +436,7 @@
     float frame_scale;
     float* g_rot6d; float* g_trans;
 };
-template <bool RIGID>
+template <bool RIGID, bool ADAM = false>
 __global__ __launch_bounds__(256) void k_mano_bwd(ManoModelDev m, const float* __restrict__ pca, int pca_stride,
                                                    const float* __restrict__ rot, const float* __restrict__ betas,
                                                    const float* __restrict__ gout, int B, const float* __restrict__ state,
@@ -440,9 +444,11 @@
                                                    int pca_dim, const float* __restrict__ g_pca_extra, float w_extra,
                                                    float* __restrict__ g_pca, float* __restrict__ g_rot,
                                                    float* __restrict__ g_betas, float* __restrict__ g_trans, int row0,
-                                                   int row_stride, ManoRigid mr)
+                                                   int row_stride, ManoRigid mr, const HmAdamTail* __restrict__ tail)
 {
     HM_HAND_KERNEL();
+    HmTailEntry te;
+    if constexpr (ADAM) te = hm_tail_enter(tail);
     __shared__ ManoShared sh;
     __shared__ float s_part[4][MANO_VCH][3];
     __shared__ float s_vp[MANO_VCH][3];
@@ -574,7 +580,9 @@
     __syncthreads();
     MPH_MARK(5);
     if (s_flag) {
-        mano_bwd2_body(m, sh, w2, partials, gridDim.x, lb, b, pca_dim, g_pca_extra, w_extra, g_pca, g_rot, g_betas, g_trans);
+        float kept[2] = {0.f, 0.f};
+        mano_bwd2_body<ADAM>(m, sh, w2, partials, gridDim.x, lb, b, pca_dim, g_pca_extra, w_extra, g_pca, g_rot, g_betas, g_trans,
+                             kept);
         if (RIGID) {
             __syncthreads();
             if (t == 0) {
@@ -584,7 +592,20 @@
                 for (int k = 0; k < 6; ++k) mr.g_rot6d[(long)b * 6 + k] = dr6[k];
 #pragma unroll
                 for (int k = 0; k < 3; ++k) mr.g_trans[(long)b * 3 + k] = w2.tot[349 + k];
+                if constexpr (ADAM) {
+#pragma unroll
+                    for (int k = 0; k < 6; ++k) red[k] = dr6[k];
+                }
             }
+        }
+        if constexpr (ADAM) {
+            __syncthreads();
+            if (t < 64) {
+                if (t < pca_dim) hm_tail_adam(tail, tail->t[0], b, t, kept[0], te);
+                if (t < 10) hm_tail_adam(tail, tail->t[1], b, t, kept[1], te);
+            } else if (t >= 128 && t < 134) hm_tail_adam(tail, tail->t[2], b, t - 128, red[t - 128], te);
+            else if (t >= 134 && t < 137) hm_tail_adam(tail, tail->t[3], b, t - 134, w2.tot[349 + t - 134], te);
+            else if (t == 192) hm_tail_arrive(tail, te.step_now);
         }
 #ifdef MANO_PHASES
         __syncthreads();
@@ -635,7 +656,7 @@
 static int mano_bwd_launch(const void* const* model, const float* pca, int pca_dim, const float* rot, const float* betas, int B,
                            const float* g_verts, const float* g_pca_extra, float w_extra, float* g_pca, float* g_rot,
                            float* g_betas, float* g_trans, const float* state, void* workspace, int row0, int row_stride,
-                           const ManoRigid& mr, hipStream_t stream)
+                           const ManoRigid& mr, hipStream_t stream, const HmAdamTail* tail = nullptr)
 {
     HM_CHECK_ARG(model && pca && rot && betas && (g_verts || mr.mesh) && g_pca && g_rot && g_betas && g_trans && workspace);
     HM_CHECK_ARG(B > 0 && pca_dim >= 16 && row_stride >= 1 && row0 >= 0 && row0 < row_stride);
@@ -643,14 +664,19 @@
                       (const float*)model[4], (const float*)model[5], (const float*)model[6], (const int*)model[7]};
     unsigned int* cnt = (unsigned int*)workspace;
     float* partials = (float*)((char*)workspace + 256 + (((size_t)B * 4 + 255) & ~(size_t)255));
-    if (mr.mesh)
-        hipLaunchKernelGGL(k_mano_bwd<true>, dim3(MANO_NCH64, B), dim3(256), 0, stream, m, pca, pca_dim, rot, betas,
+    HM_CHECK_ARG(!tail || (mr.mesh && row0 == 0 && row_stride == 1 && pca_dim <= 64));
+    if (mr.mesh && tail)
+        hipLaunchKernelGGL((k_mano_bwd<true, true>), dim3(MANO_NCH64, B), dim3(256), 0, stream, m, pca, pca_dim, rot, betas,
                            g_verts, B, state, partials, cnt, pca_dim, g_pca_extra, w_extra, g_pca, g_rot, g_betas, g_trans, row0,
-                           row_stride, mr);
+                           row_stride, mr, tail);
+    else if (mr.mesh)
+        hipLaunchKernelGGL((k_mano_bwd<true>), dim3(MANO_NCH64, B), dim3(256), 0, stream, m, pca, pca_dim, rot, betas,
+                           g_verts, B, state, partials, cnt, pca_dim, g_pca_extra, w_extra, g_pca, g_rot, g_betas, g_trans, row0,
+                           row_stride, mr, tail);
     else
-        hipLaunchKernelGGL(k_mano_bwd<false>, dim3(MANO_NCH64, B), dim3(256), 0, stream, m, pca, pca_dim, rot, betas,
+        hipLaunchKernelGGL((k_mano_bwd<false>), dim3(MANO_NCH64, B), dim3(256), 0, stream, m, pca, pca_dim, rot, betas,
                            g_verts, B, state, partials, cnt, pca_dim, g_pca_extra, w_extra, g_pca, g_rot, g_betas, g_trans, row0,
-                           row_stride, mr);
+                           row_stride, mr, tail);
     return hm_launch_status();
 }
 int hm_mano_bwd_rows(const void* const* model, const float* pca, int pca_dim, const float* rot, const float* betas, int B,
@@ -681,6 +707,26 @@
     return mano_bwd_launch(model, pca, pca_dim, rot, betas, B, nullptr, g_pca_extra, w_extra, g_pca, g_rot, g_betas, g_trans,
                            state, workspace, 0, 1, mr, stream);
 }
+int hm_mano_bwd_rigid_adam_clips(const void* const* model, const float* pca, int pca_dim, const float* rot, const float* betas,
+                                 int B, const float* g_pca_extra, float w_extra, float* g_pca, float* g_rot, float* g_betas,
+                                 float* g_trans, const float* state, void* workspace, const float* mesh,
+                                 const float* rigid_rot6d, const float* rigid_scale, const float* const* g_terms,
+                                 const float* weights, int n_terms, const float* g_rigid, const float* g_frame, int frame_stride,
+                                 float frame_scale, float* g_rigid_rot6d, float* g_rigid_trans, int clip_len, const void* tail,
+                                 hipStream_t stream)
+{
+    HM_CHECK_ARG(mesh && rigid_rot6d && rigid_scale && g_rigid_rot6d && g_rigid_trans && HM_CLIP_LEN_OK(B, clip_len) && tail);
+    HM_CHECK_ARG(n_terms >= 0 && n_terms <= 5 && (n_terms == 0 || (g_terms && weights)));
+    HM_CHECK_ARG(!g_frame || frame_stride >= 3);
+    ManoRigid mr;
+    memset(&mr, 0, sizeof(mr));
+    mr.mesh = mesh; mr.rot6d = rigid_rot6d; mr.scale = rigid_scale; mr.clip_len = clip_len ? clip_len : B;
+    for (int k = 0; k < 5; ++k) { mr.terms.p[k] = k < n_terms ? g_terms[k] : nullptr; mr.terms.w[k] = k < n_terms ? weights[k] : 0.f; }
+    mr.g_rigid = g_rigid; mr.g_frame = g_frame; mr.frame_stride = frame_stride; mr.frame_scale = frame_scale;
+    mr.g_rot6d = g_rigid_rot6d; mr.g_trans = g_rigid_trans;
+    return mano_bwd_launch(model, pca, pca_dim, rot, betas, B, nullptr, g_pca_extra, w_extra, g_pca, g_rot, g_betas, g_trans,
+                           state, workspace, 0, 1, mr, stream, (const HmAdamTail*)tail);
+}
 int hm_mano_bwd(const void* const* model, const float* pca, int pca_dim, const float* rot, const float* betas, int B,
                 const float* g_verts, const float* g_pca_extra, float w_extra, float* g_pca, float* g_rot, float* g_betas,
                 float* g_trans, const float* state, void* workspace, hipStream_t stream)
diff --git a/homan_amd/fused.py b/homan_amd/fused.py
--- a/homan_amd/fused.py
+++ b/homan_amd/fused.py
@@ -45,7 +45,8 @@
              "handobj_maxdist", "loss_depth"]
     raster_reorder = 1
 
-    def __init__(self, model, loss_weights, lr, max_steps, capture=True, shared_scale=False, group=None, collectives=True):
+    def __init__(self, model, loss_weights, lr, max_steps, capture=True, shared_scale=False, group=None, collectives=True,
+                 adam_in_tails=None):
         from . import constants, ops
         from .clipbatch import ClipBatch, ClipReduceWorkspace
         for one in (model.models if isinstance(model, ClipBatch) else model if isinstance(model, (list, tuple)) else [model]):
@@ -197,6 +198,20 @@
         self._build_optimizers(lr)
         self.log_buf = torch.zeros(max_steps, C, NS, device=dev)
         self.max_steps = max_steps
+        self.tail_obj = [m.rotations_object, m.translations_object]
+        self.tail_hand = [m.mano_pca_pose, m.mano_betas, m.rotations_hand, m.translations_hand]
+        can = (C == 1 and h == 1 and self.on["sil"] and m.optimize_mano and not m.optimize_object_scale and
+               not self.shared_scale and not self.use_aux and self.log_in_adam and self.P <= 64 and Vo <= 24576 and
+               isinstance(getattr(self, "opt", None), HmAdam) and
+               sorted(id(p) for p, _ in self.opt.items) == sorted(id(p) for p in self.tail_obj + self.tail_hand) and
+               all(p.shape[0] == B for p in self.tail_obj + self.tail_hand))
+        if adam_in_tails and not can:
+            raise NotImplementedError("adam_in_tails: one clip, one hand, silhouette term, optimize_mano, no free or tied object "
+                                      "scale, and no trainable tensor besides the six per-frame ones")
+        self.adam_in_tails = bool(can if adam_in_tails is None else adam_in_tails)
+        if self.adam_in_tails:
+            self.tail_o = self.opt.tail_block(self.tail_obj, B, 2 * B, self._adam_log())
+            self.tail_h = self.opt.tail_block(self.tail_hand, B, 2 * B, self._adam_log())
         self.rigid_ws_h, self.rigid_ws_o = (torch.zeros(self.L.hm_rigid_workspace_bytes(n), dtype=torch.uint8, device=dev)
                                             for n in (N, B))
         self.mano_state = torch.empty(self.L.hm_mano_state_bytes(N), dtype=torch.uint8, device=dev)
@@ -361,7 +376,8 @@
         self.opt = HmAdam(parameter_groups(self.model, lr))
 
     def _capture_step(self):
-        self.opt.step(zero_grad=False, log=self._adam_log())
+        if not self.adam_in_tails:
+            self.opt.step(zero_grad=False, log=self._adam_log())
 
     def _capture_iterations(self, K):
         for _ in range(K):
@@ -597,12 +613,15 @@
         g_rig = P(self.G_min_h) if (on["inter"] and self.inter_min) else None
         g_frm = (self.rec.data_ptr() + 8) if (on["inter"] and not self.inter_min) else None
         if m.optimize_mano and self.mano_bwd_rigid:
-            ck(L.hm_mano_bwd_rigid_clips(self.mctx.ptrs, P(pca), self.P, P(rot), P(betas), B,
-                                         P(self.U_pca) if on["pca"] else None, w["loss_pca"], P(pca.grad), P(rot.grad),
-                                         P(betas.grad), P(mtr.grad), P(self.mano_state), P(self.mctx.workspace(B)),
-                                         P(self.vm), P(m.rotations_hand), P(m.int_scales_hand), tp, tw, tn, g_rig, g_frm, 8,
-                                         w["loss_inter"] / Vh, P(m.rotations_hand.grad), P(m.translations_hand.grad), CL,
-                                         sb), "mano_bwd + rigid_bwd(hand)")
+            args = (self.mctx.ptrs, P(pca), self.P, P(rot), P(betas), B,
+                    P(self.U_pca) if on["pca"] else None, w["loss_pca"], P(pca.grad), P(rot.grad),
+                    P(betas.grad), P(mtr.grad), P(self.mano_state), P(self.mctx.workspace(B)),
+                    P(self.vm), P(m.rotations_hand), P(m.int_scales_hand), tp, tw, tn, g_rig, g_frm, 8,
+                    w["loss_inter"] / Vh, P(m.rotations_hand.grad), P(m.translations_hand.grad), CL)
+            if self.adam_in_tails:
+                ck(L.hm_mano_bwd_rigid_adam_clips(*args, P(self.tail_h), sb), "mano_bwd + rigid_bwd(hand) + adam")
+            else:
+                ck(L.hm_mano_bwd_rigid_clips(*args, sb), "mano_bwd + rigid_bwd(hand)")
         else:
             ck(L.hm_rigid_bwd_clips(P(self.vm if m.optimize_mano else m.verts_hand_og), P(m.rotations_hand),
                                     P(m.int_scales_hand), 0, tp, tw, tn, g_rig, g_frm, 8, w["loss_inter"] / Vh, B, Vh,
@@ -627,20 +646,23 @@
         sc_obj = m.optimize_object_scale
         sm_in = on["smooth"] and on["sil"] and Vo <= 24576
         side_terms = on["con"] or (on["inter"] and sc_obj) or (on["smooth"] and not sm_in) or not on["sil"]
-        if side_terms:
+        if side_terms or self.adam_in_tails:
             main.wait_event(self.ev_pair)
         tp, tw, tn = _lib.terms([(self.U_smo if (on["smooth"] and not sm_in) else None, w["loss_smooth_obj"]),
                                  (self.U_cono if on["con"] else None, w["loss_contact"]),
                                  (self.G_int_o if (on["inter"] and sc_obj) else None, 1.0),
                                  (self.G_dep_o if on["depth"] else None, 1.0)])
         if on["sil"]:
-            ck(L.hm_rigid_bwd_sil_clips(P(m.verts_object_og), P(m.rotations_object), P(m.int_scales_object), 1, tp, tw, tn,
-                                        sctx.parts_ptr(), P(sctx.adj_off),
-                                        P(sctx.adj_items), P(self.vo), P(self.sil_K), 1.0, sctx.F, B, Vo,
-                                        P(m.rotations_object.grad), P(m.translations_object.grad),
-                                        P(self.g_so_part) if sc_obj else None, P(self.rigid_ws_o), CL, sctx.sum_log2q,
-                                        P(self.vo) if sm_in else None, w["loss_smooth_obj"], sa),
-               "rigid_bwd(obj) + silhouette gather")
+            args = (P(m.verts_object_og), P(m.rotations_object), P(m.int_scales_object), 1, tp, tw, tn,
+                    sctx.parts_ptr(), P(sctx.adj_off),
+                    P(sctx.adj_items), P(self.vo), P(self.sil_K), 1.0, sctx.F, B, Vo,
+                    P(m.rotations_object.grad), P(m.translations_object.grad),
+                    P(self.g_so_part) if sc_obj else None, P(self.rigid_ws_o), CL, sctx.sum_log2q,
+                    P(self.vo) if sm_in else None, w["loss_smooth_obj"])
+            if self.adam_in_tails:
+                ck(L.hm_rigid_bwd_sil_adam_clips(*args, P(self.tail_o), sa), "rigid_bwd(obj) + silhouette gather + adam")
+            else:
+                ck(L.hm_rigid_bwd_sil_clips(*args, sa), "rigid_bwd(obj) + silhouette gather")
         else:
             ck(L.hm_rigid_bwd_clips(P(m.verts_object_og), P(m.rotations_object), P(m.int_scales_object), 1, tp, tw, tn, None,
                                     None, 0, 0.0, B, Vo, None, P(m.rotations_object.grad), P(m.translations_object.grad),
@@ -697,7 +719,7 @@
             if self.shared_scale:
                 self._reduce_shared_scale_grad()
                 self._spread_shared_scale_grad()
-            self.opt.step(zero_grad=False, log=self._adam_log())
+            self._capture_step()
 
     def run(self, steps):
         if self.graph_k is not None:
diff --git a/homan_amd/loopcommon.py b/homan_amd/loopcommon.py
--- a/homan_amd/loopcommon.py
+++ b/homan_amd/loopcommon.py
@@ -75,6 +75,25 @@
         self.grads = [p.grad for p, _ in self.items]
         self.blocks = max(1, min(64, (max(p.numel() for p, _ in self.items) + 255) // 256))
 
+    def tail_block(self, params, frames, target, log=None):
+        tt = np.dtype([("p", "u8"), ("m", "u8"), ("v", "u8"), ("lr", "f4"), ("per_frame", "i4")])
+        blk = np.zeros(1, dtype=[("t", tt, 4), ("step", "u8"), ("vals", "u8"), ("weights", "u8"), ("log", "u8"),
+                                 ("beta1", "f4"), ("beta2", "f4"), ("eps", "f4"), ("target", "u4"), ("n", "i4"),
+                                 ("max_steps", "i4"), ("nclips", "i4"), ("pad", "i4")])
+        assert blk.itemsize == _lib.lib().hm_adam_tail_bytes() and len(params) <= 4
+        for k, p in enumerate(params):
+            i = [id(q) for q, _ in self.items].index(id(p))
+            (m, v), lr = self.state[i], self.items[i][1]
+            assert p.is_contiguous() and p.shape[0] == frames, "the tails update per-frame tensors"
+            blk["t"][0, k] = (p.data_ptr(), m.data_ptr(), v.data_ptr(), lr, p.numel() // frames)
+        blk["step"], blk["beta1"], blk["beta2"], blk["eps"] = self.step_t.data_ptr(), self.betas[0], self.betas[1], self.eps
+        blk["target"] = target
+        if log is not None:
+            vals, weights, n, max_steps, log_buf, nclips = log
+            blk["vals"], blk["weights"], blk["log"] = vals.data_ptr(), weights.data_ptr(), log_buf.data_ptr()
+            blk["n"], blk["max_steps"], blk["nclips"] = n, max_steps, nclips
+        return torch.from_numpy(blk.view(np.uint8).copy()).to(self.step_t.device)
+
     def step(self, zero_grad=True, log=None):
         for (p, _), g in zip(self.items, self.grads):
             assert p.grad is g, "gradient buffers must stay static (do not call zero_grad(set_to_none=True))"
diff --git a/include/homan_amd.h b/include/homan_amd.h
--- a/include/homan_amd.h
+++ b/include/homan_amd.h
@@ -54,6 +54,14 @@
                             const float* rigid_scale, const float* const* g_terms, const float* weights, int n_terms,
                             const float* g_rigid, const float* g_frame, int frame_stride, float frame_scale,
                             float* g_rigid_rot6d, float* g_rigid_trans, int clip_len, hipStream_t stream);
+
+int hm_mano_bwd_rigid_adam_clips(const void* const* model, const float* pca, int pca_dim, const float* rot, const float* betas,
+                                 int B, const float* g_pca_extra, float w_extra, float* g_pca, float* g_rot, float* g_betas,
+                                 float* g_trans, const float* state, void* workspace, const float* mesh,
+                                 const float* rigid_rot6d, const float* rigid_scale, const float* const* g_terms,
+                                 const float* weights, int n_terms, const float* g_rigid, const float* g_frame, int frame_stride,
+                                 float frame_scale, float* g_rigid_rot6d, float* g_rigid_trans, int clip_len, const void* tail,
+                                 hipStream_t stream);
 
 size_t hm_sil_workspace_bytes(int B, int V, int F, int S);
 int hm_sil_fwd(const float* verts, const int* faces, int faces_bstride, const float* K, int B, int V, int F, int S,
@@ -156,6 +164,7 @@
 int hm_adam_step_log(const void* slots, int n_tensors, int* step, float beta1, float beta2, float eps, int zero_grad,
                      int blocks_per_tensor, float* vals, const float* weights, int n, int max_steps, float* log, int nclips,
                      hipStream_t stream);
+size_t hm_adam_tail_bytes(void);
 int hm_log_scalars(const float* src, int n, const int* step, int max_steps, float* log, hipStream_t stream);
 
 int hm_rigid_fwd_clips(const float* mesh, const float* rot6d, const float* trans, const float* scale, int abs_scale, int N,
@@ -171,6 +180,12 @@
                            float orig_size, int F, int N, int V, float* g_rot6d, float* g_trans, float* g_scale_part,
                            void* workspace, int clip_len, int sum_log2q, const float* smooth_verts, float smooth_weight,
                            hipStream_t stream);
+int hm_rigid_bwd_sil_adam_clips(const float* mesh, const float* rot6d, const float* scale, int abs_scale,
+                                const float* const* g_terms, const float* weights, int n_terms, const double* sil_parts,
+                                const int* adj_off, const int* adj_items, const float* cam_verts, const float* K,
+                                float orig_size, int F, int N, int V, float* g_rot6d, float* g_trans, float* g_scale_part,
+                                void* workspace, int clip_len, int sum_log2q, const float* smooth_verts, float smooth_weight,
+                                const void* tail, hipStream_t stream);
 int hm_sum_small_clips(const float* parts, int n, float w0, const float* extra, float w1, float* out, int nclips,
                        hipStream_t stream);
 int hm_mano_fwd_clips(const void* const* model, const float* pca, int pca_dim, const float* rot, const float* betas,
```

Result: slower. 6386 (-3.3%).
